# neonnnnn/sparsepoly

Measured on AMD Instinct MI355X. Metric: pcd_epochs_per_sec, higher is better.
Workload: dtype f32; 1 GPU; BASELINE configs[1]: degree=2 n_components=30 regularizer=squaredl12 solver=pcd fit_linear=True fit_lower=explicit on 1000000x100000 CSR nnz=49987865 (~50/row); schedule=colored, parallelism=single GPU, ranks=1, launcher=external, persistent_fallbacks=0

## Files before the change

sparsepoly_amd/csrc/spfm_engine.hip.h:

```cpp
#pragma once
#include <dlfcn.h>
#include <fcntl.h>
#include <sys/mman.h>
#include <unistd.h>
#include <chrono>
#include <hip/hip_runtime.h>

#include <cerrno>
#include <cmath>
#include <cstdio>
#include <cstdlib>
#include <cstring>
#include <atomic>
#include <map>
#include <memory>
#include <mutex>
#include <string>
#include <type_traits>
#include <thread>
#include <vector>

#include "../../include/spfm.h"
#include "spfm_common.hip.h"
#include "spfm_prb.hip.h"
#include "spfm_pcdw.hip.h"
#include "spfm_psgd.hip.h"

namespace spfm {
struct IntArgs;
void schedule_exact(int64_t, int32_t, const int64_t*, const int32_t*, const int32_t*, int,
                    std::vector<int32_t>&);
void schedule_colored(int64_t, int32_t, const int64_t*, const int32_t*, const int32_t*, int,
                      std::vector<int32_t>&, std::vector<int32_t>&);
void schedule_rlf(int64_t, int32_t, const int64_t*, const int32_t*, const int32_t*, int,
                  std::vector<int32_t>&, std::vector<int32_t>&);
bool csr_to_csc(int64_t, int32_t, const int64_t*, const int32_t*, std::vector<int64_t>&,
                std::vector<int32_t>&, std::vector<int64_t>&);
int schedule_threads();
void csc_to_csr(int64_t, int32_t, const int64_t*, const int32_t*, std::vector<int64_t>&,
                std::vector<int32_t>&, std::vector<int64_t>&);
void build_wide_stream(int64_t, const int64_t*, const int32_t*, const std::vector<int32_t>&,
                       const std::vector<int32_t>&, int, std::vector<int32_t>&,
                       std::vector<int32_t>&, std::vector<int32_t>&, std::vector<uint8_t>&);
void build_pb_stream(int64_t, const int64_t*, const int32_t*, const std::vector<int32_t>&,
                     const std::vector<int32_t>&, int, int, bool, const uint8_t*,
                     std::vector<int32_t>&, std::vector<int32_t>&, std::vector<uint8_t>&,
                     std::vector<uint8_t>&);
void build_rowblock_stream(int64_t, const int64_t*, const int32_t*, const std::vector<int32_t>&,
                           const std::vector<int32_t>&, int, int, std::vector<int32_t>&,
                           std::vector<int32_t>&, std::vector<uint32_t>&, const uint8_t*);
void schedule_relax(int64_t, int32_t, const int64_t*, const int32_t*, const int32_t*, int, int,
                    std::vector<int32_t>&, std::vector<int32_t>&, std::vector<int32_t>&,
                    std::vector<int32_t>&, std::vector<int64_t>&, std::vector<int64_t>&,
                    std::vector<int16_t>&, std::vector<uint8_t>&);
template <typename T>
hipError_t device_csr_to_csc(int64_t, int32_t, int64_t, const int64_t*, const int32_t*, const T*,
                             int64_t*, int32_t*, T*, int*, hipStream_t);
extern template hipError_t device_csr_to_csc<float>(int64_t, int32_t, int64_t, const int64_t*,
                                                    const int32_t*, const float*, int64_t*,
                                                    int32_t*, float*, int*, hipStream_t);
extern template hipError_t device_csr_to_csc<double>(int64_t, int32_t, int64_t, const int64_t*,
                                                     const int32_t*, const double*, int64_t*,
                                                     int32_t*, double*, int*, hipStream_t);
hipError_t device_rowblock_stream(int64_t, int32_t, int64_t, int, int, int, const int32_t*,
                                  const int32_t*, const int64_t*, const int32_t*, const uint8_t*,
                                  int32_t*, int32_t*, uint32_t*, int*, int64_t*, hipStream_t);
hipError_t device_pb_stream(int64_t, int32_t, int64_t, int, int, int, int, const int32_t*,
                            const int32_t*, const int64_t*, const int32_t*, const int64_t*,
                            const int32_t*, int32_t*, int32_t*, uint8_t*, uint8_t*, hipStream_t);
hipError_t device_wide_stream(int64_t, int32_t, int64_t, int, int, const int32_t*, const int32_t*,
                              const int64_t*, const int32_t*, const int64_t*, const int32_t*,
                              int32_t*, int32_t*, uint8_t*, hipStream_t);
hipError_t device_first_fit(int64_t, int32_t, int64_t, const int64_t*, const int32_t*, const int64_t*,
                            const int32_t*, int, int32_t*, int*, int*, hipStream_t);
hipError_t device_rlf(int64_t, int32_t, int64_t, const int64_t*, const int32_t*, const int64_t*,
                      const int32_t*, int, std::vector<int32_t>&, std::vector<int32_t>&, int*,
                      hipStream_t);
}

using namespace spfm;
struct IntPass;

typedef struct ncclComm* ncclComm_t;

struct DevBuf {
    struct Block {
        void* p;
        std::atomic<int> refs;
    };
    Block* blk = nullptr;
    void* p = nullptr;
    size_t bytes = 0;
    DevBuf() = default;
    DevBuf(const DevBuf&) = delete;
    DevBuf& operator=(const DevBuf&) = delete;
    ~DevBuf() { release(); }
    void release() {
        if (blk && blk->refs.fetch_sub(1) == 1) {
            (void)hipFree(blk->p);
            delete blk;
        }
        blk = nullptr;
        p = nullptr;
        bytes = 0;
    }
    bool shared() const { return blk && blk->refs.load() > 1; }
    hipError_t alloc(size_t b) {
        if (b <= bytes && p && !shared()) return hipSuccess;
        release();
        if (b == 0) b = 16;
        void* q = nullptr;
        hipError_t e = hipMalloc(&q, b);
        if (e != hipSuccess) return e;
        blk = new Block{q, {1}};
        p = q;
        bytes = b;
        return e;
    }
    void share(const DevBuf& o) {
        if (o.blk == blk) return;
        release();
        if (!o.blk) return;
        o.blk->refs.fetch_add(1);
        blk = o.blk;
        p = o.p;
        bytes = o.bytes;
    }
    template <typename U>
    U* as() const {
        return reinterpret_cast<U*>(p);
    }
};

#define HIPC(expr)                                                                       \
    do {                                                                                 \
        hipError_t _e = (expr);                                                          \
        if (_e != hipSuccess) {                                                          \
            err = std::string(#expr) + ": " + hipGetErrorString(_e);                     \
            return SPFM_ERR_RUNTIME;                                                     \
        }                                                                                \
    } while (0)

#define FAIL(code, msg) \
    do {                \
        err = (msg);    \
        return (code);  \
    } while (0)

#define SPFM_TRY(call)       \
    do {                     \
        int _rc = (call);    \
        if (_rc) return _rc; \
    } while (0)

#define SPFM_GUARD(h)                              \
    if (!(h)) return SPFM_ERR_INVALID;             \
    if (hipSetDevice((h)->device) != hipSuccess) { \
        (h)->err = "hipSetDevice failed";          \
        return SPFM_ERR_RUNTIME;                   \
    }

#define SPFM_DISPATCH(dt, ...)                                    \
    ((dt) == SPFM_F32 ? [&] { using T = float; __VA_ARGS__; }()   \
                      : [&] { using T = double; __VA_ARGS__; }())

static inline unsigned cdiv(int64_t a, int64_t b) { return (unsigned)((a + b - 1) / b); }

struct StreamCache {
    std::mutex mu;
    struct Prb {
        std::string key;
        DevBuf sp, erow, eval, lmask;
        int has_long = 0;
    };
    struct Pb {
        std::string key;
        DevBuf sp, erow, eval, meta, tab;
    };
    std::vector<std::unique_ptr<Prb>> prb;
    std::vector<std::unique_ptr<Pb>> pb;
    static constexpr size_t kKeep = 2;
};

struct ProfSlot {
    std::vector<hipEvent_t> ev;
    size_t used = 0;
    double ms = 0.0;
    int64_t launches = 0, nnz = 0;
};

struct spfm_engine {
    int device = 0, dtype = SPFM_F32;
    hipStream_t stream = nullptr;
    std::string err;
    std::string devname;

    int64_t n = 0, nnz = 0;
    int d = 0;
    bool have_data = false;
    DevBuf cptr, cidx, cval, rptr, ridx, rval, yy, A, col_norm;
    std::vector<int64_t> h_cptr;
    std::vector<int32_t> h_cidx;
    bool col_norm_reduced = false;
    std::shared_ptr<StreamCache> scache;
    uint64_t sched_hash = 0;
    int share_data_from(spfm_engine* src, const double* y);

    int n_orders = 0, k = 0;
    bool have_params = false;
    DevBuf P, Pt, w, lams;
    bool p_valid = true, pt_valid = false;
    std::vector<double> h_lams;

    int solver = -1, loss = 0, reg = 0, top_degree = 0;
    bool configured = false;
    DevBuf norms, cache, dcache;

    std::vector<int32_t> order, batch_ptr;
    DevBuf d_order, d_desc;
    int max_batch_cols = 0;
    bool have_schedule = false;
    int64_t sched_version = 0;

    DevBuf part, delta, pold, viol_col, scalar, ctl, comp_order, pred_tmp, partial, pb_scal,
        pb_ticket;
    bool pbcd_fuse = true;
    double* h_scalar = nullptr;

    DevBuf sg_gradP, sg_gradw, sg_samples, sg_part, sg_cond, sg_thr, sg_theta, sg_done,
        sg_norms, sg_conv, sg_sched, sg_idx, sg_snapP, sg_snapw, sg_snapc;
    bool psgd_force_eager = false;
    int psgd_graph_sweeps = 4;
    bool psgd_warm = false;
    int psgd_redone = 0;
    std::vector<PsgdBatch> h_sched;

    bool use_graph = true;
    bool fuse_chain = true;
    int max_batch_opt = 4096;

    bool pers_failed = false;
    int pers_fallbacks = 0;
    std::string pers_reason;
    int spin_max = 1 << 21;
    int debug_drop = 0;
    bool keep_last_error = false;
    bool have_pred_args = false;
    int pa_degree = 0, pa_lin = 0, pa_lower = 0;
    DevBuf snapP, snapW, snapC;
    std::map<const void*, int> resident_cache;
    std::map<std::string, bool> resident_agreed;

    bool persistent = true;
    int prb_G = 64;
    bool prb_lds = true;
    int prb_lds_active = 0;
    bool y_pm1 = false;
    bool prb_ready = false;
    int prb_has_long = 0;
    int prb_long = kPrbLong;
    DevBuf prb_sp, prb_erow, prb_eval, prb_slab, prb_abort, prow_old, d_bptr, prb_stamps,
        prb_viol, prb_cn, prb_lmask, prb_rec;
    bool prb_pack = true;
    int prb_pack_active = 0;
    bool prb_stamp_on = false;
    int wide_min_cols = 110;
    bool wide_stamp_on = false;
    DevBuf wide_stamps;
    DevBuf w_rec;
    static constexpr size_t kPrbLds = 84 * 1024;
    bool relax_on = true;
    int relax_state = 0;
    std::vector<int32_t> r_batch_ptr;
    int relax_has_long = 0;
    DevBuf r_bptr, r_sp, r_erow, r_eval, r_lmask, r_cfptr, r_cf, r_clist, r_cslab;
    bool wide_on = true;
    int pcdw_G = 0;
    bool wide_ready = false;
    int wide_G = 0, wide_tot = 0;
    int wide_lr_active = 0;
    int wide_lds_cap = -1;
    bool wide_ep = true;
    int wide_ep_active = 0;
    bool wide_rec8 = true;
    DevBuf w_wbase, w_wsp, w_erow, w_eval, w_slabA, w_slabB;
    bool pb_persistent = true;
    int pbprb_G = 256;
    int probe_xcd = 0, probe_lds = 60 * 1024;
    bool pb_stream_ready = false;
    int pb_stream_G = 0, pb_stream_NG = 0;
    DevBuf pb_tab;
    int pbr_state = 0;
    int pbr_G = 0, pb_relax_active = 0;
    std::vector<int32_t> pbr_batch_ptr;
    DevBuf pbr_bptr, pbr_sp, pbr_erow, pbr_eval, pbr_meta, pbr_tab, pbr_cfptr, pbr_cf, pbr_clist,
        pbr_slabR;
    bool pb_balance = true;
    DevBuf pb_sp, pb_erow, pb_eval, pb_meta, pb_slabA, pb_slabB, pb_slabC, pb_stamps, pb_rec;
    bool pb_stamp_on = false;
    int pbprb_active = 0;
    int pb_dbg = 0;
    DevBuf pb_dbgbuf;
    std::map<std::string, hipGraphExec_t> graphs;

    ncclComm_t comm = nullptr;
    struct ShmComm {
        static constexpr size_t kMaxDoubles = 1 << 16;
        struct Hdr {
            volatile int arrive;
            volatile int sense;
            int pad[14];
        };
        Hdr* hdr = nullptr;
        double* slots = nullptr;
        size_t bytes = 0;
        int local_sense = 0;
    } shm;
    std::vector<double> shm_host;
    bool dist() const { return comm != nullptr || shm.hdr != nullptr; }
    int n_ranks = 1, rank = 0;
    static constexpr size_t kPeerPcdOff = 0, kPeerPbOff = 16 * 1024;
    static constexpr size_t kPeerProbeOff = kPeerPbOff + (size_t)2 * 64 * 8 * 64;
    static constexpr size_t kPeerDoubles = kPeerProbeOff + 64;
    int peer_generation = 0;
    void* peer_own = nullptr;
    std::vector<void*> peer_ptr;
    DevBuf peer_tab_pcd, peer_tab_pb;
    bool peer_ready = false;

    bool prof_on = false;
    ProfSlot prof[5];

    ~spfm_engine();

    void clear_graphs() {
        for (auto& kv : graphs) (void)hipGraphExecDestroy(kv.second);
        graphs.clear();
    }

    enum : unsigned {
        kInvPrbStream = 1,
        kInvPbStream = 2,
        kInvWideStream = 4,
        kInvRelax = 8,
        kInvPbRelax = 16,
        kInvSchedule = 32,
        kInvGraphs = 64,
        kInvStreams = kInvPrbStream | kInvPbStream | kInvWideStream,
    };
    void invalidate(unsigned mask) {
        if (mask & kInvPrbStream) prb_ready = false;
        if (mask & kInvPbStream) pb_stream_ready = false;
        if (mask & kInvWideStream) wide_ready = false;
        if (mask & kInvRelax) relax_state = 0;
        if (mask & kInvPbRelax) pbr_state = 0;
        if (mask & kInvSchedule) have_schedule = false;
        if (mask & kInvGraphs) clear_graphs();
    }

    RegState regstate() {
        RegState rs;
        rs.norms = norms.as<double>();
        rs.cache = cache.as<double>();
        rs.dcache = dcache.as<double>();
        return rs;
    }

    size_t tsize() const { return dtype == SPFM_F32 ? 4 : 8; }

    int sync() {
        HIPC(hipStreamSynchronize(stream));
        return SPFM_OK;
    }

    template <typename U>
    int upload_to(void* dst, const U* src, size_t count) {
        if (count) HIPC(hipMemcpyAsync(dst, src, sizeof(U) * count, hipMemcpyHostToDevice, stream));
        return SPFM_OK;
    }
    template <typename U>
    int upload(DevBuf& b, const U* src, size_t count, size_t min_count = 0) {
        HIPC(b.alloc(sizeof(U) * std::max(count, min_count)));
        return upload_to(b.p, src, count);
    }
    template <typename U>
    int download(U* dst, const void* src, size_t count) {
        if (count) HIPC(hipMemcpyAsync(dst, src, sizeof(U) * count, hipMemcpyDeviceToHost, stream));
        return SPFM_OK;
    }

    template <typename T>
    int stage_csr_rows(DevBuf& rp, DevBuf& ri, DevBuf& rv, std::vector<T>& hv,
                       const int64_t* indptr, const int32_t* indices, const double* data,
                       int64_t r0, int64_t r1, size_t min_entries = 0) {
        const int64_t e0 = r0 ? indptr[r0] : 0, ne = indptr[r1] - e0;
        const T* vals;
        if constexpr (std::is_same<T, double>::value) {
            vals = data + e0;
        } else {
            hv.resize((size_t)ne);
            const int nt = (ne >= (1 << 20)) ? schedule_threads() : 1;
            const int64_t per = (ne + nt - 1) / nt;
            auto work = [&](int tid) {
                const int64_t lo = per * tid, hi = std::min<int64_t>(ne, lo + per);
                for (int64_t ii = lo; ii < hi; ++ii) hv[(size_t)ii] = (T)data[e0 + ii];
            };
            std::vector<std::thread> pool;
            for (int t = 1; t < nt; ++t) pool.emplace_back(work, t);
            work(0);
            for (auto& th : pool) th.join();
            vals = hv.data();
        }
        SPFM_TRY(upload(rp, indptr + r0, (size_t)(r1 - r0 + 1)));
        SPFM_TRY(upload(ri, indices + e0, (size_t)ne, min_entries));
        return upload(rv, vals, (size_t)ne, min_entries);
    }

    template <typename T>
    int upload_targets(const double* y, std::vector<T>& hy) {
        hy.resize((size_t)n * 2);
        for (int64_t i = 0; i < n; ++i) {
            hy[(size_t)2 * i] = (T)0;
            hy[(size_t)2 * i + 1] = (T)y[i];
        }
        return upload_to(yy.p, hy.data(), hy.size());
    }

    struct BlockView {
        const double* base;
        int64_t ss, sj;
    };
    BlockView live_block(int order_idx) const {
        const double* img = p_valid ? P.as<double>() : Pt.as<double>();
        return {img + (size_t)order_idx * k * d, p_valid ? (int64_t)d : 1, p_valid ? 1 : (int64_t)k};
    }

    static constexpr size_t kProfPool = 32768;
    bool prof_armed = false;
    void prof_begin(int which, int64_t nnz_launch) {
        prof_armed = false;
        if (!prof_on) return;
        ProfSlot& ps = prof[which];
        if (ps.used + 2 > kProfPool) return;
        if (ps.used + 2 > ps.ev.size()) {
            hipEvent_t a, b;
            if (hipEventCreate(&a) != hipSuccess) return;
            if (hipEventCreate(&b) != hipSuccess) {
                (void)hipEventDestroy(a);
                return;
            }
            ps.ev.push_back(a);
            ps.ev.push_back(b);
        }
        ps.launches++;
        ps.nnz += nnz_launch;
        (void)hipEventRecord(ps.ev[ps.used], stream);
        prof_armed = true;
    }
    void prof_cancel(int which, int64_t nnz_launch) {
        if (!prof_armed) return;
        prof[which].launches--;
        prof[which].nnz -= nnz_launch;
        prof_armed = false;
    }
    void prof_end(int which) {
        if (!prof_armed) return;
        ProfSlot& ps = prof[which];
        (void)hipEventRecord(ps.ev[ps.used + 1], stream);
        ps.used += 2;
        prof_armed = false;
    }
    void prof_collect() {
        if (!prof_on) return;
        (void)hipStreamSynchronize(stream);
        for (auto& ps : prof) {
            for (size_t i = 0; i + 1 < ps.used; i += 2) {
                float ms = 0.f;
                if (hipEventElapsedTime(&ms, ps.ev[i], ps.ev[i + 1]) == hipSuccess) ps.ms += ms;
            }
            ps.used = 0;
        }
    }

    int64_t batch_nnz(int b) const {
        int64_t s = 0;
        for (int q = batch_ptr[b]; q < batch_ptr[b + 1]; ++q)
            s += h_cptr[order[q] + 1] - h_cptr[order[q]];
        return s;
    }

    int shm_barrier();

    int allreduce_shm(double* buf, size_t count);
    int allreduce_shm_piece(double* buf, size_t count);

    int allreduce(double* buf, size_t count);

    int ensure_col_norm();

    int ensure_p();
    int ensure_pt();

    template <typename F>
    int run_cached(const std::string& key, F&& body) {
        const bool graph_ok = use_graph && !prof_on && !dist();
        if (!graph_ok) return body();
        auto it = graphs.find(key);
        if (it == graphs.end()) {
            hipGraph_t g = nullptr;
            HIPC(hipStreamBeginCapture(stream, hipStreamCaptureModeThreadLocal));
            int rc = body();
            hipError_t e = hipStreamEndCapture(stream, &g);
            if (rc != SPFM_OK) {
                if (g) (void)hipGraphDestroy(g);
                return rc;
            }
            if (e != hipSuccess) {
                err = std::string("hipStreamEndCapture: ") + hipGetErrorString(e);
                return SPFM_ERR_RUNTIME;
            }
            hipGraphExec_t ge = nullptr;
            e = hipGraphInstantiate(&ge, g, nullptr, nullptr, 0);
            (void)hipGraphDestroy(g);
            if (e != hipSuccess) {
                err = std::string("hipGraphInstantiate: ") + hipGetErrorString(e);
                return SPFM_ERR_RUNTIME;
            }
            it = graphs.emplace(key, ge).first;
        }
        HIPC(hipGraphLaunch(it->second, stream));
        return SPFM_OK;
    }

    template <typename T>
    int upload_images(const int64_t* h_cp, const int32_t* h_ci, const int64_t* h_rp,
                      const int32_t* h_ri, const double* data_csc, const double* data_csr,
                      const int64_t* perm, const double* y);

    template <typename T>
    int set_data_t(const int64_t* indptr, const int32_t* indices, const double* data,
                   const double* y);

    int data_installed(const double* y);

    bool ingest_device = true;
    int ingest_device_used = 0;
    int co_tenants = 1;
    static constexpr int kIngestFallback = 2;
    template <typename T>
    int set_data_csr_device(const int64_t* indptr, const int32_t* indices, const double* data,
                            const double* y);

    int set_data_csr(int64_t n_, int32_t d_, const int64_t* indptr, const int32_t* indices,
                     const double* data, const double* y);

    int set_data(int64_t n_, int32_t d_, const int64_t* indptr, const int32_t* indices,
                 const double* data, const double* y);

    int set_params(int n_orders_, int k_, int32_t d_, const double* P_, const double* w_,
                   const double* lams_);

    int get_params(double* P_, double* w_);

    int configure(int solver_, int loss_, int reg_, int top_degree_);

// ... 359 lines not shown
```

sparsepoly_amd/csrc/spfm_engine_pcd.hip:

```cpp
#include "spfm_engine.hip.h"
#include "spfm_pcd.hip.h"
#include "spfm_linear.hip.h"

using namespace spfm;

template <typename T>
int spfm_engine::lin_body(double alpha) {
    const double mu = loss == SPFM_LOSS_SQUARED ? 1.0 : (loss == SPFM_LOSS_LOGISTIC ? 0.25 : 2.0);
    const int nb = n_batches();
    for (int b = 0; b < nb; ++b) {
        const int c0 = batch_ptr[b], nc = batch_ptr[b + 1] - c0;
        if (nc == 0) continue;
        const int32_t* cols = d_order.as<int32_t>() + c0;
        prof_begin(4, prof_on ? batch_nnz(b) : 0);
        if (!dist()) {
            hipLaunchKernelGGL((lin_fused_kernel<T>), dim3(nc), dim3(kBlock), 0, stream,
                               d_desc.as<ColDesc>() + c0, cidx.as<int32_t>(), cval.as<T>(),
                               yy.as<T>(), loss, w.as<double>(), col_norm.as<double>(), alpha,
                               mu, viol_col.as<double>());
        } else {
            hipLaunchKernelGGL((lin_grad_kernel<T>), dim3(nc), dim3(kBlock), 0, stream, cols,
                               cptr.as<int64_t>(), cidx.as<int32_t>(), cval.as<T>(),
                               yy.as<typename Vec2<T>::type>(), loss, part.as<double>());
            int rc = allreduce(part.as<double>(), (size_t)nc);
            if (rc) return rc;
            hipLaunchKernelGGL((lin_sync_kernel<T>), dim3(nc), dim3(kBlock), 0, stream, cols,
                               cptr.as<int64_t>(), cidx.as<int32_t>(), cval.as<T>(),
                               yy.as<T>(), part.as<double>(), w.as<double>(),
                               col_norm.as<double>(), alpha, mu, viol_col.as<double>());
        }
        prof_end(4);
    }
    HIPC(hipGetLastError());
    return SPFM_OK;
}

int spfm_engine::cd_linear_epoch(double alpha, double* viol) {
    int rc = epoch_prologue();
    if (rc) return rc;
    const bool wide = wide_usable();
    if (wide || prb_usable()) {
        const char* what = wide ? "wide persistent cd_linear pass" : "persistent cd_linear pass";
        rc = snapshot_state(w.as<double>(), (size_t)d, snapW);
        if (rc) return rc;
        if (wide) rc = SPFM_DISPATCH(dtype, return lin_wide<T>(alpha));
        else rc = SPFM_DISPATCH(dtype, return lin_prb_loss<T>(alpha));
        if (rc == kNotResident) {
            mark_not_resident(what);
            return cd_linear_epoch(alpha, viol);
        }
        if (rc) return rc;
        rc = epoch_epilogue(viol);
        if (rc) return rc;
        bool aborted = false;
        rc = persistent_aborted(&aborted);
        if (rc) return rc;
        if (aborted) {
            rc = recover_from_abort(w.as<double>(), (size_t)d, snapW, what);
            if (rc) return rc;
            return cd_linear_epoch(alpha, viol);
        }
        return SPFM_OK;
    }
    const std::string key = fkey("lin", {alpha}, {loss, sched_version});
    rc = run_cached(key, [&]() {
        return SPFM_DISPATCH(dtype, return lin_body<T>(alpha));
    });
    if (rc) return rc;
    return epoch_epilogue(viol);
}

template <typename T, int M>
int spfm_engine::pcd_pass_body(int order_idx, double beta, double gamma, double eta) {
    const double mu = loss == SPFM_LOSS_SQUARED ? 1.0 : (loss == SPFM_LOSS_LOGISTIC ? 0.25 : 2.0);
    double* Po = P.as<double>() + (size_t)order_idx * k * d;
    Ctl* c = ctl.as<Ctl>();
    double* cbuf[2] = {cache.as<double>(), cache.as<double>() + (kMaxDegree + 2)};
    hipLaunchKernelGGL(begin_pass_kernel, dim3(1), dim3(64), 0, stream, c,
                       comp_order.as<int32_t>(), lams.as<double>());
    const size_t a_stride = (size_t)n * Kind<M>::AS;
    if (reg != SPFM_REG_L1) {
        hipLaunchKernelGGL((pcd_compute_cache_kernel<M>), dim3(kCacheBlocks), dim3(kBlock), 0,
                           stream, c, Po, d, reg, partial.as<double>());
        hipLaunchKernelGGL((pcd_cache_combine_kernel<M>), dim3(1), dim3(64), 0, stream, reg,
                           kCacheBlocks, partial.as<double>(), cbuf[0]);
    }
    const int nb = n_batches();
    int par = 0;
    for (int b = 0; b < nb; ++b) {
        const int c0 = batch_ptr[b], nc = batch_ptr[b + 1] - c0;
        if (nc == 0) continue;
        const ColDesc* desc = d_desc.as<ColDesc>() + c0;
        const int64_t bn = prof_on ? batch_nnz(b) : 0;
        prof_begin(0, bn);
        hipLaunchKernelGGL((pcd_grad_kernel<T, M>), dim3(nc), dim3(kBlock), 0, stream, c, desc,
                           cidx.as<int32_t>(), cval.as<T>(), A.as<T>(), a_stride,
                           yy.as<typename Vec2<T>::type>(), Po, d, loss, part.as<double>(),
                           pold.as<double>());
        prof_end(0);
        int rc = allreduce(part.as<double>(), (size_t)2 * nc);
        if (rc) return rc;
        if (nc <= kWave && fuse_chain) {
            prof_begin(1, bn);
            hipLaunchKernelGGL((pcd_chain_sync_kernel<T, M>), dim3(nc), dim3(kBlock), 0, stream,
                               c, desc, nc, Po, d, part.as<double>(), pold.as<double>(), reg,
                               cbuf[par], cbuf[par ^ 1], mu, beta, gamma, eta,
                               cidx.as<int32_t>(), cval.as<T>(), A.as<T>(), a_stride,
                               yy.as<T>(), viol_col.as<double>());
            prof_end(1);
        } else {
            hipLaunchKernelGGL((pcd_chain_kernel<M>), dim3(1), dim3(kWave), 0, stream, c, desc,
                               nc, Po, d, part.as<double>(), pold.as<double>(), reg, cbuf[par],
                               cbuf[par ^ 1], mu, beta, gamma, eta, delta.as<double>(),
                               viol_col.as<double>());
            prof_begin(1, bn);
            hipLaunchKernelGGL((pcd_sync_kernel<T, M>), dim3(nc), dim3(kBlock), 0, stream, c,
                               desc, cidx.as<int32_t>(), cval.as<T>(), A.as<T>(), a_stride,
                               yy.as<T>(), delta.as<double>(), pold.as<double>());
            prof_end(1);
        }
        par ^= 1;
    }
    HIPC(hipGetLastError());
    return SPFM_OK;
}

PrbArgs spfm_engine::prb_args() {
    PrbArgs a;
    a.G = prb_G;
    a.nb = n_batches();
    a.bptr = d_bptr.as<int32_t>();
    a.desc = d_desc.as<ColDesc>();
    a.sp = prb_sp.as<int32_t>();
    a.lmask = prb_lmask.as<uint32_t>();
    a.has_long = prb_has_long;
    a.erow = prb_erow.as<int32_t>();
    a.slab = prb_slab.as<double>();
    a.rows_per = (int)std::max<int64_t>((n + prb_G - 1) / prb_G, 1);
    a.n_rows = (int)n;
    a.abort_flag = prb_abort.as<unsigned>();
    a.spin_max = spin_max;
    a.stamps = prb_stamp_on ? prb_stamps.as<long long>() : nullptr;
    a.n_ranks = peer_ready ? n_ranks : 1;
    a.rank = rank;
    a.xslab = peer_ready ? peer_tab_pcd.as<double*>() : nullptr;
    a.cf_ptr = nullptr;
    a.cf = nullptr;
    a.clist = nullptr;
    a.cslab = nullptr;
    a.rec = nullptr;
    return a;
}

PrbArgs spfm_engine::relax_args() {
    PrbArgs a = prb_args();
    a.nb = (int)r_batch_ptr.size() - 1;
    a.bptr = r_bptr.as<int32_t>();
    a.sp = r_sp.as<int32_t>();
    a.lmask = r_lmask.as<uint32_t>();
    a.has_long = relax_has_long;
    a.erow = r_erow.as<int32_t>();
    a.stamps = nullptr;
    a.cf_ptr = r_cfptr.as<int32_t>();
    a.cf = r_cf.p;
    a.clist = r_clist.as<int16_t>();
    a.cslab = r_cslab.as<double>();
    return a;
}

template <typename T, int M>
int spfm_engine::pcd_precompute_all(int order_idx) {
    if (n == 0) return SPFM_OK;
    pt_valid = false;
    int rc = ensure_pt();
    if (rc) return rc;
    const size_t lds = sizeof(T) * (size_t)Kind<M>::AS * kWave * 33;
    HIPC(hipFuncSetAttribute((const void*)pcd_precompute_all_kernel<T, M>,
                             hipFuncAttributeMaxDynamicSharedMemorySize, (int)lds));
    const int64_t tiles = (n + 31) / 32;
    const unsigned grid = (unsigned)std::min<int64_t>(tiles, 256 * 8);
    hipLaunchKernelGGL((pcd_precompute_all_kernel<T, M>), dim3(grid), dim3(kBlock), lds,
                       stream, n, k, rptr.as<int64_t>(), ridx.as<int32_t>(), rval.as<T>(),
                       Pt.as<double>() + (size_t)order_idx * k * d, A.as<T>());
    HIPC(hipGetLastError());
    return SPFM_OK;
}

template <typename T>
int spfm_engine::pcd_precompute_all_dispatch(int M, int order_idx) {
    switch (M) {
        case 0: return pcd_precompute_all<T, 0>(order_idx);
        case 2: return pcd_precompute_all<T, 2>(order_idx);
        case 3: return pcd_precompute_all<T, 3>(order_idx);
        case 4: return pcd_precompute_all<T, 4>(order_idx);
        case 5: return pcd_precompute_all<T, 5>(order_idx);
        case 6: return pcd_precompute_all<T, 6>(order_idx);
    }
    FAIL(SPFM_ERR_UNSUPPORTED, "degree outside 2..6");
}

template <typename T>
int spfm_engine::pcd_pass_dispatch(int M, int order_idx, double beta, double gamma, double eta) {
    switch (M) {
        case 0: return pcd_pass_body<T, 0>(order_idx, beta, gamma, eta);
        case 2: return pcd_pass_body<T, 2>(order_idx, beta, gamma, eta);
        case 3: return pcd_pass_body<T, 3>(order_idx, beta, gamma, eta);
        case 4: return pcd_pass_body<T, 4>(order_idx, beta, gamma, eta);
        case 5: return pcd_pass_body<T, 5>(order_idx, beta, gamma, eta);
        case 6: return pcd_pass_body<T, 6>(order_idx, beta, gamma, eta);
    }
    FAIL(SPFM_ERR_UNSUPPORTED, "degree outside 2..6");
}

int spfm_engine::pcd_epoch(int order_idx, int degree, double beta, double gamma, double eta,
              const int32_t* ic, int n_comp, double* viol) {
    int rc = epoch_prologue();
    if (rc) return rc;
    if (solver != SPFM_SOLVER_PCD) FAIL(SPFM_ERR_INVALID, "engine is not configured for pcd");
    if (order_idx < 0 || order_idx >= n_orders) FAIL(SPFM_ERR_INVALID, "bad order index");
    if (!degree_ok(degree)) FAIL(SPFM_ERR_INVALID, "bad degree");
    if (!ic || n_comp < 0 || n_comp > k) FAIL(SPFM_ERR_INVALID, "bad indices_component");
    for (int q = 0; q < n_comp; ++q)
        if (ic[q] < 0 || ic[q] >= k) FAIL(SPFM_ERR_INVALID, "indices_component out of range");
    rc = ensure_p();
    if (rc) return rc;
    pt_valid = false;
    if (n_comp > 0)
        SPFM_TRY(upload_to(comp_order.p, ic, (size_t)n_comp));
    HIPC(hipMemsetAsync(ctl.p, 0, sizeof(Ctl), stream));
    const std::string key = fkey("pcd", {beta, gamma, eta},
                                 {order_idx, degree, loss, reg, sched_version});
    const int M = kind_of(degree);
    rc = SPFM_DISPATCH(dtype, return pcd_precompute_all_dispatch<T>(M, order_idx));
    if (rc) return rc;
    bool use_prb = prb_usable();
    bool use_wide = wide_usable() && M == 2;
    const bool pers_epoch = use_prb || use_wide;
    double* Po_epoch = P.as<double>() + (size_t)order_idx * k * d;
    if (pers_epoch) {
        rc = snapshot_state(Po_epoch, (size_t)k * d, snapP);
        if (rc) return rc;
    }
    for (int pass = 0; pass < n_comp; ++pass) {
        rc = SPFM_OK;
        if (use_wide) {
            rc = SPFM_DISPATCH(dtype, return pcd_pass_wide<T>(order_idx, beta, gamma, eta));
        } else if (use_prb) {
            rc = SPFM_DISPATCH(dtype, return pcd_prb_dispatch<T>(M, order_idx, beta, gamma, eta));
        }
        if (rc == kNotResident) {
            mark_not_resident(use_wide ? "wide persistent pcd pass" : "persistent pcd pass");
            use_prb = use_wide = false;
            hipLaunchKernelGGL(unbegin_pass_kernel, dim3(1), dim3(1), 0, stream, ctl.as<Ctl>());
            HIPC(hipGetLastError());
        }
        if (!use_wide && !use_prb) {
            rc = run_cached(key, [&]() {
                return SPFM_DISPATCH(dtype, return pcd_pass_dispatch<T>(M, order_idx, beta, gamma,
                                     eta));
            });
        }
        if (rc) return rc;
    }
    pt_valid = false;
    rc = epoch_epilogue(viol);
    if (rc) return rc;
    if (pers_epoch) {
        bool aborted = false;
        rc = persistent_aborted(&aborted);
        if (rc) return rc;
        if (aborted) {
            rc = recover_from_abort(Po_epoch, (size_t)k * d, snapP,
                                    use_wide ? "wide persistent pcd pass" : "persistent pcd pass");
            if (rc) return rc;
            return pcd_epoch(order_idx, degree, beta, gamma, eta, ic, n_comp, viol);
        }
    }
    return SPFM_OK;
}

int spfm_engine::host_epoch_begin(int order_idx, int degree) {
    int rc = epoch_prologue();
    if (rc) return rc;
    if (solver != SPFM_SOLVER_PCD && solver != SPFM_SOLVER_PBCD)
        FAIL(SPFM_ERR_INVALID, "host-stepped epochs: configure for pcd or pbcd");
    if (order_idx < 0 || order_idx >= n_orders) FAIL(SPFM_ERR_INVALID, "bad order index");
    if (!degree_ok(degree)) FAIL(SPFM_ERR_INVALID, "bad degree");
    const int M = kind_of(degree);
    if (solver == SPFM_SOLVER_PCD) {
        rc = ensure_p();
        if (rc) return rc;
        pt_valid = false;
        HIPC(hipMemsetAsync(ctl.p, 0, sizeof(Ctl), stream));
        rc = SPFM_DISPATCH(dtype, return pcd_precompute_all_dispatch<T>(M, order_idx));
        if (rc) return rc;
        pt_valid = false;
    } else {
        rc = ensure_pt();
        if (rc) return rc;
        p_valid = false;
        rc = SPFM_DISPATCH(dtype, return host_pbcd_precompute<T>(M, order_idx));
        if (rc) return rc;
    }
    host_order = order_idx;
    host_degree = degree;
    return sync();
}

int spfm_engine::host_pass_begin(int s) {
    if (host_order < 0 || solver != SPFM_SOLVER_PCD)
        FAIL(SPFM_ERR_INVALID, "host_pass_begin: call spfm_host_epoch_begin (pcd) first");
    if (s < 0 || s >= k) FAIL(SPFM_ERR_INVALID, "component out of range");
    Ctl hc;
    std::memset(&hc, 0, sizeof hc);
    hc.s = s;
    hc.lam = h_lams[(size_t)s];
    SPFM_TRY(upload_to(ctl.p, &hc, 1));
    return sync();
}

template <typename T, int M>
int spfm_engine::host_sums_pcd(int b, double* out) {
    const int c0 = batch_ptr[b], nc = batch_ptr[b + 1] - c0;
    if (nc == 0) return SPFM_OK;
    double* Po = P.as<double>() + (size_t)host_order * k * d;
    hipLaunchKernelGGL((pcd_grad_kernel<T, M>), dim3(nc), dim3(kBlock), 0, stream, ctl.as<Ctl>(),
                       d_desc.as<ColDesc>() + c0, cidx.as<int32_t>(), cval.as<T>(), A.as<T>(),
                       (size_t)n * Kind<M>::AS, yy.as<typename Vec2<T>::type>(), Po, d, loss,
                       part.as<double>(), pold.as<double>());
    HIPC(hipGetLastError());
    int rc = allreduce(part.as<double>(), (size_t)2 * nc);
    if (rc) return rc;
    SPFM_TRY(download(out, part.p, 2 * (size_t)nc));
    return sync();
}

template <typename T, int M>
int spfm_engine::host_apply_pcd(int b, const double* p_new) {
    const int c0 = batch_ptr[b], nc = batch_ptr[b + 1] - c0;
    if (nc == 0) return SPFM_OK;
    double* Po = P.as<double>() + (size_t)host_order * k * d;
    SPFM_TRY(upload_to(delta.p, p_new, (size_t)nc));
    hipLaunchKernelGGL(host_apply_pcd_kernel, dim3(cdiv(nc, 64)), dim3(64), 0, stream,
                       ctl.as<Ctl>(), d_desc.as<ColDesc>() + c0, nc, Po, d, pold.as<double>(),
                       delta.as<double>(), viol_col.as<double>());
    hipLaunchKernelGGL((pcd_sync_kernel<T, M>), dim3(nc), dim3(kBlock), 0, stream, ctl.as<Ctl>(),
                       d_desc.as<ColDesc>() + c0, cidx.as<int32_t>(), cval.as<T>(), A.as<T>(),
                       (size_t)n * Kind<M>::AS, yy.as<T>(), delta.as<double>(),
                       pold.as<double>());
    HIPC(hipGetLastError());
    return sync();
}

int spfm_engine::host_step(bool sums, int b, double* out, const double* p_new, const double* p_old) {
    int rc = host_step_check(b);
    if (rc) return rc;
    if ((sums && !out) || (!sums && !p_new)) FAIL(SPFM_ERR_INVALID, "host step: NULL buffer");
    if (solver == SPFM_SOLVER_PCD)
        return SPFM_DISPATCH(dtype, return host_step_pcd_t<T>(sums, b, out, p_new));
    return SPFM_DISPATCH(dtype, return host_step_pbcd_t<T>(sums, b, out, p_new, p_old));
}

template <typename T>
int spfm_engine::host_step_pcd_t(bool sums, int b, double* out, const double* p_new) {
#define SPFM_HPC(MM) return sums ? host_sums_pcd<T, MM>(b, out) : host_apply_pcd<T, MM>(b, p_new)
    switch (kind_of(host_degree)) {
        case 0: SPFM_HPC(0);
        case 2: SPFM_HPC(2);
        case 3: SPFM_HPC(3);
        case 4: SPFM_HPC(4);
        case 5: SPFM_HPC(5);
        case 6: SPFM_HPC(6);
    }
#undef SPFM_HPC
    FAIL(SPFM_ERR_UNSUPPORTED, "degree outside 2..6");
}

int spfm_engine::host_epoch_end(double* viol) {
    if (host_order < 0) FAIL(SPFM_ERR_INVALID, "host_epoch_end: no host-stepped epoch open");
    host_order = -1;
    if (solver == SPFM_SOLVER_PCD) pt_valid = false;
    return epoch_epilogue(viol);
}


int spfm_engine::debug_stream_probe(int64_t* bytes_out) {
    if (!have_schedule || !prb_usable())
        FAIL(SPFM_ERR_INVALID, "stream probe: needs a schedule the 64-column persistent pass can run");
    int rc = SPFM_DISPATCH(dtype, return ensure_prb<T>());
    if (rc) return rc;
    DevBuf sink;
    if (sink.alloc(sizeof(double) * (size_t)prb_G * kPrbThreads) != hipSuccess)
        FAIL(SPFM_ERR_RUNTIME, "stream probe: allocation failed");
    const PrbArgs a = prb_args();
    SPFM_DISPATCH(dtype, hipLaunchKernelGGL((prb_stream_probe_kernel<T>), dim3(prb_G),
                                            dim3(kPrbThreads), 0, stream, a, prb_eval.as<T>(),
                                            sink.as<double>()));
    if (hipStreamSynchronize(stream) != hipSuccess)
        FAIL(SPFM_ERR_RUNTIME, "stream probe kernel failed");
    if (bytes_out)
        *bytes_out = nnz * (int64_t)(4 + tsize()) + (int64_t)prb_G * ((int64_t)d + n_batches()) * 4;
    return SPFM_OK;
}

int spfm_engine::debug_write_probe(int bytes, int64_t* bytes_out) {
    if (!have_schedule || !prb_usable())
        FAIL(SPFM_ERR_INVALID, "write probe: needs a schedule the 64-column persistent pass can run");
    if (bytes != 4 && bytes != 8 && bytes != 16) FAIL(SPFM_ERR_INVALID, "write probe: 4, 8 or 16 bytes");
    int rc = SPFM_DISPATCH(dtype, return ensure_prb<T>());
    if (rc) return rc;
    DevBuf recs;
    if (recs.alloc((size_t)16 * (size_t)(n > 0 ? n : 1)) != hipSuccess)
        FAIL(SPFM_ERR_RUNTIME, "write probe: allocation failed");
    const PrbArgs a = prb_args();
    if (bytes == 4)
        hipLaunchKernelGGL((prb_write_probe_kernel<4>), dim3(prb_G), dim3(kPrbThreads), 0, stream, a,
                           recs.as<float>());
    else if (bytes == 8)
        hipLaunchKernelGGL((prb_write_probe_kernel<8>), dim3(prb_G), dim3(kPrbThreads), 0, stream, a,
                           recs.as<float>());
    else
        hipLaunchKernelGGL((prb_write_probe_kernel<16>), dim3(prb_G), dim3(kPrbThreads), 0, stream,
                           a, recs.as<float>());
    if (hipStreamSynchronize(stream) != hipSuccess) FAIL(SPFM_ERR_RUNTIME, "write probe kernel failed");
    if (bytes_out) *bytes_out = nnz * (int64_t)bytes;
    return SPFM_OK;
}

SPFM_DEFINE_BRANCH_COUNTS(spfm_branch_counts_pcd)

template int spfm_engine::pcd_precompute_all_dispatch<float>(int, int);
template int spfm_engine::pcd_precompute_all_dispatch<double>(int, int);
```

sparsepoly_amd/csrc/spfm_engine_prb.inc.h:

```cpp
#include "spfm_engine.hip.h"
#include "spfm_pcd.hip.h"

using namespace spfm;

template <typename T, int LOSS>
int spfm_engine::lin_prb(double alpha) {
    const double mu = loss == SPFM_LOSS_SQUARED ? 1.0 : (loss == SPFM_LOSS_LOGISTIC ? 0.25 : 2.0);
    int rc = ensure_prb<T>();
    if (rc) return rc;
    constexpr bool can_lr = std::is_same<T, float>::value;
    constexpr int LRV = (LOSS == LOSS_SQUARED) ? 1 : 2;
    bool relaxed = false;
    if (relax_candidate()) {
        rc = ensure_relax<T>();
        if (rc) return rc;
        relaxed = relax_state == 1;
    }
    const PrbArgs pa = relaxed ? relax_args() : prb_args();
    int lds_max = 0;
    HIPC(hipDeviceGetAttribute(&lds_max, hipDeviceAttributeMaxSharedMemoryPerBlock, device));
    const size_t lds_lr = sizeof(double) * (kPrbLdsFixed + (relaxed ? kPrbLdsCR : 0)) +
                          (size_t)pa.rows_per * 5 + 16;
    const bool use_lr = can_lr && prb_lds && lds_lr <= (size_t)lds_max && (LRV == 1 || y_pm1);
    const size_t lds_bytes = use_lr ? std::max(lds_lr, kPrbLds) : kPrbLds;
    if constexpr (can_lr) {
        if (use_lr)
            HIPC(hipFuncSetAttribute((const void*)lin_prb_kernel<T, LOSS, LRV>,
                                     hipFuncAttributeMaxDynamicSharedMemorySize,
                                     (int)lds_bytes));
    }
    HIPC(hipFuncSetAttribute((const void*)lin_prb_kernel<T, LOSS, 0>,
                             hipFuncAttributeMaxDynamicSharedMemorySize, (int)kPrbLds));
    hipLaunchKernelGGL(gather_sched_kernel, dim3(cdiv(d, 256)), dim3(256), 0, stream, d,
                       d_desc.as<ColDesc>(), w.as<double>(), prow_old.as<double>());
    HIPC(hipMemsetAsync(prb_slab.p, 0, prb_slab.bytes, stream));
    if (relaxed) HIPC(hipMemsetAsync(r_cslab.p, 0, r_cslab.bytes, stream));
    {
        int prc = peer_clear(kPeerPcdOff, kPeerPbOff);
        if (prc) return prc;
    }
    prof_begin(4, nnz);
    bool launched = false;
    auto launch_cr = [&](auto lr_tag, size_t lds) -> int {
        constexpr int LRc = decltype(lr_tag)::value;
        auto* fn = lin_prb_kernel<T, LOSS, LRc, false, true>;
        HIPC(hipFuncSetAttribute((const void*)fn, hipFuncAttributeMaxDynamicSharedMemorySize,
                                 (int)lds));
        if (!resident_ok((const void*)fn, kPrbThreads, lds, prb_G)) return kNotResident;
        hipLaunchKernelGGL(fn, dim3(launch_groups(prb_G)), dim3(kPrbThreads), lds, stream, pa,
                           r_eval.as<T>(), yy.as<T>(), prow_old.as<double>(),
                           prb_cn.as<double>(), w.as<double>(), alpha, mu,
                           prb_viol.as<double>());
        return SPFM_OK;
    };
    auto launch = [&](auto lr_tag, auto mg_tag, size_t lds) -> int {
        constexpr int LRc = decltype(lr_tag)::value;
        constexpr bool MGc = decltype(mg_tag)::value;
        HIPC(hipFuncSetAttribute((const void*)lin_prb_kernel<T, LOSS, LRc, MGc>,
                                 hipFuncAttributeMaxDynamicSharedMemorySize, (int)lds));
        if (!resident_ok((const void*)lin_prb_kernel<T, LOSS, LRc, MGc>, kPrbThreads, lds, prb_G))
            return kNotResident;
        hipLaunchKernelGGL((lin_prb_kernel<T, LOSS, LRc, MGc>), dim3(launch_groups(prb_G)),
                           dim3(kPrbThreads),
                           lds, stream, pa, prb_eval.as<T>(), yy.as<T>(),
                           prow_old.as<double>(), prb_cn.as<double>(), w.as<double>(), alpha,
                           mu, prb_viol.as<double>());
        return SPFM_OK;
    };
    int lrc = SPFM_OK;
    if (relaxed) {
        launched = true;
        bool done = false;
        if constexpr (can_lr) {
            if (use_lr) {
                lrc = launch_cr(std::integral_constant<int, LRV>{}, lds_bytes);
                done = true;
            }
        }
        if (!done) lrc = launch_cr(std::integral_constant<int, 0>{}, kPrbLds);
    }
    if constexpr (can_lr) {
        if (use_lr && !launched) {
            lrc = pa.n_ranks > 1
                      ? launch(std::integral_constant<int, LRV>{}, std::true_type{}, lds_bytes)
                      : launch(std::integral_constant<int, LRV>{}, std::false_type{}, lds_bytes);
            launched = true;
        }
    }
    if (!launched)
        lrc = pa.n_ranks > 1
                  ? launch(std::integral_constant<int, 0>{}, std::true_type{}, kPrbLds)
                  : launch(std::integral_constant<int, 0>{}, std::false_type{}, kPrbLds);
    if (lrc == kNotResident) prof_cancel(4, nnz);
    if (lrc) return lrc;
    prof_end(4);
    hipLaunchKernelGGL(fold_viol_kernel, dim3(cdiv(d, 256)), dim3(256), 0, stream, d,
                       d_desc.as<ColDesc>(), prb_viol.as<double>(), viol_col.as<double>());
    HIPC(hipGetLastError());
    return SPFM_OK;
}

template <typename T>
int spfm_engine::lin_prb_loss(double alpha) {
    switch (loss) {
        case SPFM_LOSS_SQUARED: return lin_prb<T, LOSS_SQUARED>(alpha);
        case SPFM_LOSS_SQUARED_HINGE: return lin_prb<T, LOSS_SQUARED_HINGE>(alpha);
        default: return lin_prb<T, LOSS_LOGISTIC>(alpha);
    }
}

template <typename T>
int spfm_engine::ensure_prb() {
    if (prb_ready) return SPFM_OK;
    int ncu = 0;
    HIPC(hipDeviceGetAttribute(&ncu, hipDeviceAttributeMultiprocessorCount, device));
    if (prb_G > ncu) prb_G = ncu;
    if (prb_G < 1) prb_G = 1;
    const int nb_ = n_batches();
    std::unique_lock<std::mutex> cache_lock;
    std::string ckey;
    bool hit = false;
    if (scache) {
        ckey = fkey("prb", {}, {(int64_t)sched_hash, prb_G, prb_long, (int64_t)sizeof(T), nb_});
        cache_lock = std::unique_lock<std::mutex>(scache->mu);
        for (auto& e : scache->prb)
            if (e->key == ckey) {
                prb_sp.share(e->sp);
                prb_erow.share(e->erow);
                prb_eval.share(e->eval);
                prb_lmask.share(e->lmask);
                prb_has_long = e->has_long;
                stream_device_used = 2;
                hit = true;
                break;
            }
    }
    if (!hit) {
        int rc = build_prb_stream<T>(nb_);
        if (rc) return rc;
        if (scache) {
            auto e = std::make_unique<StreamCache::Prb>();
            e->key = ckey;
            e->sp.share(prb_sp);
            e->erow.share(prb_erow);
            e->eval.share(prb_eval);
            e->lmask.share(prb_lmask);
            e->has_long = prb_has_long;
            scache->prb.insert(scache->prb.begin(), std::move(e));
            if (scache->prb.size() > StreamCache::kKeep) scache->prb.pop_back();
        }
    }
    if (cache_lock.owns_lock()) cache_lock.unlock();
    HIPC(prb_slab.alloc(sizeof(double) * 2 * ((size_t)prb_G + 1) * 64 * 2));
    HIPC(prb_abort.alloc(sizeof(unsigned) * 4));
    HIPC(prow_old.alloc(sizeof(double) * (size_t)d));
    HIPC(prb_viol.alloc(sizeof(double) * (size_t)d));
    HIPC(prb_cn.alloc(sizeof(double) * (size_t)d));
    HIPC(prb_stamps.alloc(sizeof(long long) * 16 * (size_t)prb_G));
    HIPC(hipMemsetAsync(prb_stamps.p, 0, prb_stamps.bytes, stream));
    HIPC(hipMemsetAsync(prb_abort.p, 0, sizeof(unsigned) * 4, stream));
    HIPC(hipMemsetAsync(prb_slab.p, 0, prb_slab.bytes, stream));
    hipLaunchKernelGGL(gather_sched_kernel, dim3(cdiv(d, 256)), dim3(256), 0, stream, d,
                       d_desc.as<ColDesc>(), col_norm.as<double>(), prb_cn.as<double>());
    HIPC(hipGetLastError());
    HIPC(hipStreamSynchronize(stream));
    prb_ready = true;
    return SPFM_OK;
}

template <typename T>
int spfm_engine::build_prb_stream(int nb_) {
    const size_t nsp = (size_t)prb_G * nb_ * 65 + 1;
    DevBuf d_src;
    HIPC(d_src.alloc(sizeof(int32_t) * (size_t)(nnz > 0 ? nnz : 1)));
    HIPC(prb_sp.alloc(sizeof(int32_t) * nsp));
    HIPC(prb_lmask.alloc(sizeof(uint32_t) * (size_t)prb_G * nb_ * 2));
    stream_device_used = 0;
    if (stream_device && nnz >= (1 << 20)) {
        int hl = 0;
        const hipError_t e = device_rowblock_stream(
            n, d, nnz, prb_G, nb_, prb_long, d_order.as<int32_t>(), d_bptr.as<int32_t>(),
            cptr.as<int64_t>(), cidx.as<int32_t>(), nullptr, prb_sp.as<int32_t>(),
            d_src.as<int32_t>(), prb_lmask.as<uint32_t>(), &hl, nullptr, stream);
        if (e == hipSuccess) {
            prb_has_long = hl;
            stream_device_used = 1;
        } else {
            (void)hipGetLastError();
        }
    }
    std::vector<int32_t> sp, src;
    std::vector<uint32_t> lmask;
    if (!stream_device_used) {
        build_rowblock_stream(n, h_cptr.data(), h_cidx.data(), order, batch_ptr, prb_G,
                              prb_long, sp, src, lmask, nullptr);
        prb_has_long = 0;
        for (uint32_t m : lmask) prb_has_long |= (m != 0u);
        SPFM_TRY(upload_to(prb_lmask.p, lmask.data(), lmask.size()));
    }
    HIPC(prb_erow.alloc(sizeof(int32_t) * (size_t)(nnz > 0 ? nnz : 1)));
    HIPC(prb_eval.alloc(sizeof(T) * (size_t)(nnz > 0 ? nnz : 1)));
    if (!stream_device_used)
        SPFM_TRY(upload_to(prb_sp.p, sp.data(), sp.size()));
    if (nnz > 0) {
        if (!stream_device_used)
            SPFM_TRY(upload_to(d_src.p, src.data(), (size_t)nnz));
        hipLaunchKernelGGL((prb_gather_kernel<T>), dim3(cdiv(nnz, 256)), dim3(256), 0, stream,
                           nnz, d_src.as<int32_t>(), cidx.as<int32_t>(), cval.as<T>(),
                           prb_erow.as<int32_t>(), prb_eval.as<T>());
        HIPC(hipGetLastError());
    }
    HIPC(hipStreamSynchronize(stream));
    return SPFM_OK;
}

template <typename T>
int spfm_engine::ensure_relax() {
    if (relax_state != 0) return SPFM_OK;
    relax_state = -1;
    int rc = ensure_prb<T>();
    if (rc) return rc;
    std::vector<int32_t> cf_ptr, cf_row, cf_qq, sp, src;
    std::vector<int64_t> cf_ia, cf_ib;
    std::vector<int16_t> clist;
    std::vector<uint8_t> skip;
    std::vector<uint32_t> lmask;
    schedule_relax(n, d, h_cptr.data(), h_cidx.data(), order.data(), 64, 64, r_batch_ptr, cf_ptr,
                   cf_row, cf_qq, cf_ia, cf_ib, clist, skip);
    const int nbr = (int)r_batch_ptr.size() - 1;
    if ((double)nbr > 0.6 * (double)n_batches()) return SPFM_OK;
    DevBuf d_src;
    HIPC(r_bptr.alloc(sizeof(int32_t) * r_batch_ptr.size()));
    SPFM_TRY(upload_to(r_bptr.p, r_batch_ptr.data(), r_batch_ptr.size()));
    const size_t nsp_r = (size_t)prb_G * nbr * 65 + 1;
    bool dev_stream = false;
    size_t ne = 0;
    if (stream_device && nnz >= (1 << 20)) {
        DevBuf d_skip;
        HIPC(d_skip.alloc((size_t)nnz));
        SPFM_TRY(upload_to(d_skip.p, skip.data(), (size_t)nnz));
        HIPC(d_src.alloc(sizeof(int32_t) * (size_t)nnz));
        HIPC(r_sp.alloc(sizeof(int32_t) * nsp_r));
        HIPC(r_lmask.alloc(sizeof(uint32_t) * (size_t)prb_G * nbr * 2));
        int hl = 0;
        int64_t tot = 0;
        const hipError_t e = device_rowblock_stream(
            n, d, nnz, prb_G, nbr, prb_long, d_order.as<int32_t>(), r_bptr.as<int32_t>(),
            cptr.as<int64_t>(), cidx.as<int32_t>(), d_skip.as<uint8_t>(), r_sp.as<int32_t>(),
            d_src.as<int32_t>(), r_lmask.as<uint32_t>(), &hl, &tot, stream);
        if (e == hipSuccess) {
            relax_has_long = hl;
            ne = (size_t)tot;
            dev_stream = true;
        } else {
            (void)hipGetLastError();
        }
    }
    if (!dev_stream) {
        build_rowblock_stream(n, h_cptr.data(), h_cidx.data(), order, r_batch_ptr, prb_G,
                              prb_long, sp, src, lmask, skip.data());
        relax_has_long = 0;
        for (uint32_t m : lmask) relax_has_long |= (m != 0u);
        ne = src.size();
    }
    const size_t ncf = cf_row.size();
    std::vector<PrbConf<T>> hcf(ncf ? ncf : 1);
    {
        std::vector<T> hv((size_t)(nnz > 0 ? nnz : 1));
        SPFM_TRY(download(hv.data(), cval.p, (size_t)nnz));
        HIPC(hipStreamSynchronize(stream));
        for (size_t c = 0; c < ncf; ++c) {
            hcf[c].row = cf_row[c];
            hcf[c].qq = cf_qq[c];
            hcf[c].xa = hv[(size_t)cf_ia[c]];
            hcf[c].xb = hv[(size_t)cf_ib[c]];
        }
    }
    if (!dev_stream) {
        HIPC(d_src.alloc(sizeof(int32_t) * (ne ? ne : 1)));
        HIPC(r_sp.alloc(sizeof(int32_t) * sp.size()));
        HIPC(r_lmask.alloc(sizeof(uint32_t) * lmask.size()));
    }
    HIPC(r_erow.alloc(sizeof(int32_t) * (ne ? ne : 1)));
    HIPC(r_eval.alloc(sizeof(T) * (ne ? ne : 1)));
    HIPC(r_cfptr.alloc(sizeof(int32_t) * cf_ptr.size()));
    HIPC(r_cf.alloc(sizeof(PrbConf<T>) * hcf.size()));
    HIPC(r_clist.alloc(sizeof(int16_t) * clist.size() + 16));
    HIPC(r_cslab.alloc(sizeof(double) * 2 * 64 * 8));
    if (!dev_stream) {
        SPFM_TRY(upload_to(r_sp.p, sp.data(), sp.size()));
        SPFM_TRY(upload_to(r_lmask.p, lmask.data(), lmask.size()));
    }
    SPFM_TRY(upload_to(r_cfptr.p, cf_ptr.data(), cf_ptr.size()));
    SPFM_TRY(upload_to(r_cf.p, hcf.data(), hcf.size()));
    SPFM_TRY(upload_to(r_clist.p, clist.data(), clist.size()));
    if (ne > 0) {
        if (!dev_stream)
            SPFM_TRY(upload_to(d_src.p, src.data(), ne));
        hipLaunchKernelGGL((prb_gather_kernel<T>), dim3(cdiv((int64_t)ne, 256)), dim3(256), 0,
                           stream, (int64_t)ne, d_src.as<int32_t>(), cidx.as<int32_t>(),
                           cval.as<T>(), r_erow.as<int32_t>(), r_eval.as<T>());
        HIPC(hipGetLastError());
    }
    HIPC(hipStreamSynchronize(stream));
    relax_state = 1;
    return SPFM_OK;
}

template <typename T, int M, int LOSS>
int spfm_engine::pcd_pass_prb(int order_idx, double beta, double gamma, double eta) {
    const double mu = loss == SPFM_LOSS_SQUARED ? 1.0 : (loss == SPFM_LOSS_LOGISTIC ? 0.25 : 2.0);
    int rc = ensure_prb<T>();
    if (rc) return rc;
    double* Po = P.as<double>() + (size_t)order_idx * k * d;
    Ctl* c = ctl.as<Ctl>();
    double* cb = cache.as<double>();
    constexpr bool can_lr = std::is_same<T, float>::value && Kind<M>::AS <= 2;
    constexpr int LRV = (LOSS == LOSS_SQUARED) ? 1 : 2;
    constexpr bool can_stamp = std::is_same<T, float>::value && M == 2 && LOSS == LOSS_SQUARED;
    constexpr bool can_stamp3 = std::is_same<T, float>::value && M == 3 && LOSS == LOSS_SQUARED;
    if (prb_stamp_on && !((can_stamp && prb_lds) || (can_stamp3 && !prb_lds)))
        FAIL(SPFM_ERR_UNSUPPORTED,
             "prb_stamps: built for float storage, squared loss and degree 2 with prb_lds=1 "
             "or degree 3 with prb_lds=0 only");
    bool relaxed = false;
    if constexpr (M == 2 || M == 3) {
        if (relax_candidate() && !prb_stamp_on) {
            rc = ensure_relax<T>();
            if (rc) return rc;
            relaxed = relax_state == 1;
        }
    }
    PrbArgs pa = relaxed ? relax_args() : prb_args();
    constexpr bool can_pk = std::is_same<T, float>::value && M == 3;
    bool packed = false;
    if (prb_stamp_on && pa.n_ranks > 1)
        FAIL(SPFM_ERR_UNSUPPORTED,
             "prb_stamps: the timer instantiation has no cross-GPU stage (single rank only)");
    int lds_max = 0;
    HIPC(hipDeviceGetAttribute(&lds_max, hipDeviceAttributeMaxSharedMemoryPerBlock, device));
    const size_t lds_lr = sizeof(double) * (kPrbLdsFixed + (relaxed ? kPrbLdsCR : 0)) +
                          (size_t)pa.rows_per * (4 * Kind<M>::AS + (LRV == 1 ? 4 : 5)) + 16;
    const bool use_lr = can_lr && prb_lds && lds_lr <= (size_t)lds_max &&
                        (LRV == 1 || y_pm1);
    const size_t lds_bytes = use_lr ? std::max(lds_lr, kPrbLds) : kPrbLds;
    prb_lds_active = use_lr ? LRV : 0;
    hipLaunchKernelGGL(begin_pass_kernel, dim3(1), dim3(64), 0, stream, c,
                       comp_order.as<int32_t>(), lams.as<double>());
    if (reg != SPFM_REG_L1) {
        hipLaunchKernelGGL((pcd_compute_cache_kernel<M>), dim3(kCacheBlocks), dim3(kBlock), 0,
                           stream, c, Po, d, reg, partial.as<double>());
        hipLaunchKernelGGL((pcd_cache_combine_kernel<M>), dim3(1), dim3(64), 0, stream, reg,
                           kCacheBlocks, partial.as<double>(), cb);
    }
    hipLaunchKernelGGL(snapshot_row_kernel, dim3(cdiv(d, 256)), dim3(256), 0, stream, c, Po, d,
                       d_desc.as<ColDesc>(), prow_old.as<double>());
    HIPC(hipMemsetAsync(prb_slab.p, 0, prb_slab.bytes, stream));
    if (relaxed) HIPC(hipMemsetAsync(r_cslab.p, 0, r_cslab.bytes, stream));
    if constexpr (can_pk) {
        if (!use_lr && !prb_stamp_on && prb_pack) {
            HIPC(prb_rec.alloc(sizeof(float) * 4 * (size_t)n));
            pa.rec = prb_rec.p;
            hipLaunchKernelGGL(prb_pack3_kernel, dim3(cdiv(n, 256)), dim3(256), 0, stream, c, n,
                               (size_t)n * 2, yy.as<float>(), A.as<float>(),
                               prb_rec.as<float4>());
            packed = true;
        }
    }
    {
        int prc = peer_clear(kPeerPcdOff, kPeerPbOff);
        if (prc) return prc;
    }
    prof_begin(0, nnz);
    auto go = [&](auto lr_tag, auto stamp_tag, auto reg_tag) -> int {
        constexpr int LRc = decltype(lr_tag)::value;
        constexpr bool STc = decltype(stamp_tag)::value;
        constexpr int RGc = decltype(reg_tag)::value;
        const size_t lds = (LRc == 1 || LRc == 2) ? lds_bytes : kPrbLds;
        auto launch = [&](auto mg_tag) -> int {
            constexpr bool MGc = decltype(mg_tag)::value;
            HIPC(hipFuncSetAttribute(
                (const void*)pcd_prb_kernel<T, M, LOSS, LRc, STc, RGc, MGc>,
                hipFuncAttributeMaxDynamicSharedMemorySize, (int)lds));
            if (!resident_ok((const void*)pcd_prb_kernel<T, M, LOSS, LRc, STc, RGc, MGc>,
                             kPrbThreads, lds, prb_G))
                return kNotResident;
            hipLaunchKernelGGL((pcd_prb_kernel<T, M, LOSS, LRc, STc, RGc, MGc>),
                               dim3(launch_groups(prb_G)), dim3(kPrbThreads), lds, stream, c, pa, prb_eval.as<T>(),
                               A.as<T>(), (size_t)n * Kind<M>::AS, yy.as<T>(),
                               prow_old.as<double>(), Po, d, reg, cb, mu, beta, gamma, eta,
                               prb_viol.as<double>());
            return SPFM_OK;
        };
        if constexpr (STc) {
            return launch(std::false_type{});
        } else {
            return pa.n_ranks > 1 ? launch(std::true_type{}) : launch(std::false_type{});
        }
    };
    using std::integral_constant;
    int lrc = SPFM_OK;
    bool launched = false;
    if constexpr (M == 2 || M == 3) {
        if (relaxed) {
            auto launch_cr = [&](auto lr_tag) -> int {
                constexpr int LRc = decltype(lr_tag)::value;
                const size_t lds = (LRc == 1 || LRc == 2) ? lds_bytes : kPrbLds;
                auto* fn = pcd_prb_kernel<T, M, LOSS, LRc, false, -1, false, true>;
                HIPC(hipFuncSetAttribute((const void*)fn,
                                         hipFuncAttributeMaxDynamicSharedMemorySize, (int)lds));
                if (!resident_ok((const void*)fn, kPrbThreads, lds, prb_G)) return kNotResident;
                hipLaunchKernelGGL(fn, dim3(launch_groups(prb_G)), dim3(kPrbThreads), lds, stream,
                                   c, pa, r_eval.as<T>(), A.as<T>(), (size_t)n * Kind<M>::AS,
                                   yy.as<T>(), prow_old.as<double>(), Po, d, reg, cb, mu, beta,
                                   gamma, eta, prb_viol.as<double>());
                return SPFM_OK;
            };
            launched = true;
            bool done = false;
            if constexpr (can_lr) {
                if (use_lr) {
                    lrc = launch_cr(integral_constant<int, LRV>{});
                    done = true;
                }
            }
            if constexpr (can_pk) {
                if (!done && packed) {
                    lrc = launch_cr(integral_constant<int, 3>{});
                    done = true;
                }
            }
            if (!done) lrc = launch_cr(integral_constant<int, 0>{});
        }
    }
    if constexpr (can_lr) {
        if (use_lr && !launched) {
            launched = true;
            if constexpr (can_stamp) {
                if (prb_stamp_on)
                    lrc = go(integral_constant<int, LRV>{}, std::true_type{},
                             integral_constant<int, -1>{});
            }
            if (!prb_stamp_on) {
                if (reg == SPFM_REG_L1)
                    lrc = go(integral_constant<int, LRV>{}, std::false_type{},
                             integral_constant<int, REG_L1>{});
                else if (reg == SPFM_REG_OMEGATI)
                    lrc = go(integral_constant<int, LRV>{}, std::false_type{},
                             integral_constant<int, REG_OMEGATI>{});
                else if constexpr (M == 2)
                    lrc = go(integral_constant<int, LRV>{}, std::false_type{},
                             integral_constant<int, REG_SQL12>{});
                else
                    lrc = go(integral_constant<int, LRV>{}, std::false_type{},
                             integral_constant<int, -1>{});
            }
        }
    }
    if constexpr (can_pk) {
        if (!launched && packed) {
            launched = true;
            lrc = go(integral_constant<int, 3>{}, std::false_type{}, integral_constant<int, -1>{});
        }
    }
    if constexpr (can_stamp3) {
        if (!launched && prb_stamp_on) {
            launched = true;
            lrc = go(integral_constant<int, 0>{}, std::true_type{}, integral_constant<int, -1>{});
        }
    }
    if (!launched)
        lrc = go(integral_constant<int, 0>{}, std::false_type{}, integral_constant<int, -1>{});
    prb_pack_active = packed ? 1 : 0;
    if (lrc == kNotResident) prof_cancel(0, nnz);
    if (lrc) return lrc;
    prof_end(0);
    if constexpr (can_pk) {
        if (packed)
            hipLaunchKernelGGL(prb_unpack3_kernel, dim3(cdiv(n, 256)), dim3(256), 0, stream, c, n,
                               (size_t)n * 2, prb_rec.as<float4>(), yy.as<float>(),
                               A.as<float>());
    }
    hipLaunchKernelGGL(fold_viol_kernel, dim3(cdiv(d, 256)), dim3(256), 0, stream, d,
                       d_desc.as<ColDesc>(), prb_viol.as<double>(), viol_col.as<double>());
    HIPC(hipGetLastError());
    return SPFM_OK;
}

template <typename T, int M>
int spfm_engine::pcd_prb_loss(int order_idx, double beta, double gamma, double eta) {
    switch (loss) {
        case SPFM_LOSS_SQUARED:
            return pcd_pass_prb<T, M, LOSS_SQUARED>(order_idx, beta, gamma, eta);
        case SPFM_LOSS_SQUARED_HINGE:
            return pcd_pass_prb<T, M, LOSS_SQUARED_HINGE>(order_idx, beta, gamma, eta);
        default:
            return pcd_pass_prb<T, M, LOSS_LOGISTIC>(order_idx, beta, gamma, eta);
    }
}

template <typename T>
int spfm_engine::pcd_prb_dispatch(int M, int order_idx, double beta, double gamma, double eta) {
    switch (M) {
        case 0: return pcd_prb_loss<T, 0>(order_idx, beta, gamma, eta);
        case 2: return pcd_prb_loss<T, 2>(order_idx, beta, gamma, eta);
        case 3: return pcd_prb_loss<T, 3>(order_idx, beta, gamma, eta);
        case 4: return pcd_prb_loss<T, 4>(order_idx, beta, gamma, eta);
        case 5: return pcd_prb_loss<T, 5>(order_idx, beta, gamma, eta);
        case 6: return pcd_prb_loss<T, 6>(order_idx, beta, gamma, eta);
    }
    FAIL(SPFM_ERR_UNSUPPORTED, "degree outside 2..6");
}


#define SPFM_CAT_(a, b) a##b
#define SPFM_CAT(a, b) SPFM_CAT_(a, b)
SPFM_DEFINE_BRANCH_COUNTS(SPFM_CAT(spfm_branch_counts_prb_, SPFM_TU_TAG))

template int spfm_engine::ensure_prb<SPFM_TU_T>();
template int spfm_engine::lin_prb_loss<SPFM_TU_T>(double);
template int spfm_engine::pcd_prb_dispatch<SPFM_TU_T>(int, int, double, double, double);
```

sparsepoly_amd/csrc/spfm_ingest.hip:

```cpp
#include <hip/hip_runtime.h>

#include <cstdint>
#include <cstring>

#include <rocprim/device/device_radix_sort.hpp>

namespace spfm {

__global__ void ingest_check_kernel(int64_t n, int32_t d, const int64_t* __restrict__ rptr,
                                    const int32_t* __restrict__ ridx, int* __restrict__ flag) {
    const int64_t i = (int64_t)blockIdx.x * blockDim.x + threadIdx.x;
    if (i >= n) return;
    int bad = 0;
    int32_t prev = -1;
    for (int64_t ii = rptr[i]; ii < rptr[i + 1]; ++ii) {
        const int32_t j = ridx[ii];
        bad |= (j <= prev) | (j >= d);
        prev = j;
    }
    if (bad) atomicOr(flag, 1);
}

__global__ void ingest_rows_kernel(int64_t n, int64_t nnz, const int64_t* __restrict__ rptr,
                                   int32_t* __restrict__ pos, int32_t* __restrict__ row) {
    const int64_t ii = (int64_t)blockIdx.x * blockDim.x + threadIdx.x;
    if (ii >= nnz) return;
    int64_t lo = 0, hi = n;
    while (hi - lo > 1) {
        const int64_t mid = (lo + hi) >> 1;
        if (rptr[mid] <= ii) lo = mid;
        else hi = mid;
    }
    pos[ii] = (int32_t)ii;
    row[ii] = (int32_t)lo;
}

template <typename T>
__global__ void ingest_gather_kernel(int64_t nnz, const int32_t* __restrict__ perm,
                                     const int32_t* __restrict__ row, const T* __restrict__ rval,
                                     int32_t* __restrict__ cidx, T* __restrict__ cval) {
    const int64_t e = (int64_t)blockIdx.x * blockDim.x + threadIdx.x;
    if (e >= nnz) return;
    const int32_t p = perm[e];
    cidx[e] = row[p];
    cval[e] = rval[p];
}

__global__ void ingest_cptr_kernel(int32_t d, int64_t nnz, const int32_t* __restrict__ keys,
                                   int64_t* __restrict__ cptr) {
    const int32_t j = blockIdx.x * blockDim.x + threadIdx.x;
    if (j > d) return;
    int64_t lo = 0, hi = nnz;
    while (lo < hi) {
        const int64_t mid = (lo + hi) >> 1;
        if (keys[mid] < j) lo = mid + 1;
        else hi = mid;
    }
    cptr[j] = lo;
}

template <typename T>
hipError_t device_csr_to_csc(int64_t n, int32_t d, int64_t nnz, const int64_t* rptr,
                             const int32_t* ridx, const T* rval, int64_t* cptr, int32_t* cidx,
                             T* cval, int* invalid, hipStream_t stream) {
    *invalid = 0;
    hipError_t e;
    int* d_flag = nullptr;
    int32_t *pos = nullptr, *row = nullptr, *keys_out = nullptr, *perm = nullptr;
    void* temp = nullptr;
    auto done = [&](hipError_t rc) {
        (void)hipFree(d_flag);
        (void)hipFree(pos);
        (void)hipFree(row);
        (void)hipFree(keys_out);
        (void)hipFree(perm);
        (void)hipFree(temp);
        return rc;
    };
    if ((e = hipMalloc(&d_flag, sizeof(int))) != hipSuccess) return done(e);
    if ((e = hipMemsetAsync(d_flag, 0, sizeof(int), stream)) != hipSuccess) return done(e);
    if (n > 0)
        hipLaunchKernelGGL(ingest_check_kernel, dim3((unsigned)((n + 255) / 256)), dim3(256), 0,
                           stream, n, d, rptr, ridx, d_flag);
    int h_flag = 0;
    if ((e = hipMemcpyAsync(&h_flag, d_flag, sizeof(int), hipMemcpyDeviceToHost, stream)) !=
            hipSuccess ||
        (e = hipStreamSynchronize(stream)) != hipSuccess)
        return done(e);
    if (h_flag) {
        *invalid = 1;
        return done(hipSuccess);
    }
    const size_t nz = (size_t)(nnz > 0 ? nnz : 1);
    if ((e = hipMalloc(&pos, sizeof(int32_t) * nz)) != hipSuccess) return done(e);
    if ((e = hipMalloc(&row, sizeof(int32_t) * nz)) != hipSuccess) return done(e);
    if ((e = hipMalloc(&keys_out, sizeof(int32_t) * nz)) != hipSuccess) return done(e);
    if ((e = hipMalloc(&perm, sizeof(int32_t) * nz)) != hipSuccess) return done(e);
    if (nnz > 0) {
        hipLaunchKernelGGL(ingest_rows_kernel, dim3((unsigned)((nnz + 255) / 256)), dim3(256), 0,
                           stream, n, nnz, rptr, pos, row);
        int end_bit = 1;
        while (end_bit < 31 && (1 << end_bit) < d) ++end_bit;
        size_t temp_bytes = 0;
        if ((e = rocprim::radix_sort_pairs(nullptr, temp_bytes, ridx, keys_out, pos, perm,
                                           (size_t)nnz, 0, end_bit, stream)) != hipSuccess)
            return done(e);
        if ((e = hipMalloc(&temp, temp_bytes ? temp_bytes : 16)) != hipSuccess) return done(e);
        if ((e = rocprim::radix_sort_pairs(temp, temp_bytes, ridx, keys_out, pos, perm, (size_t)nnz,
                                           0, end_bit, stream)) != hipSuccess)
            return done(e);
        hipLaunchKernelGGL((ingest_gather_kernel<T>), dim3((unsigned)((nnz + 255) / 256)), dim3(256),
                           0, stream, nnz, perm, row, rval, cidx, cval);
    }
    hipLaunchKernelGGL(ingest_cptr_kernel, dim3((unsigned)((d + 1 + 255) / 256)), dim3(256), 0, stream,
                       d, nnz, keys_out, cptr);
    if ((e = hipGetLastError()) != hipSuccess) return done(e);
    if ((e = hipStreamSynchronize(stream)) != hipSuccess) return done(e);
    return done(hipSuccess);
}

template hipError_t device_csr_to_csc<float>(int64_t, int32_t, int64_t, const int64_t*,
                                             const int32_t*, const float*, int64_t*, int32_t*,
                                             float*, int*, hipStream_t);
template hipError_t device_csr_to_csc<double>(int64_t, int32_t, int64_t, const int64_t*,
                                              const int32_t*, const double*, int64_t*, int32_t*,
                                              double*, int*, hipStream_t);

}

#include <rocprim/device/device_scan.hpp>

namespace spfm {

__device__ __forceinline__ int64_t rbs_lower_bound(const int32_t* __restrict__ a, int64_t lo,
                                                   int64_t hi, int64_t key) {
    while (lo < hi) {
        const int64_t mid = (lo + hi) >> 1;
        if ((int64_t)a[mid] < key) lo = mid + 1;
        else hi = mid;
    }
    return lo;
}

__global__ void rbs_count_kernel(int32_t d, int G, int nb, int64_t rows_per,
                                 const int32_t* __restrict__ order, const int32_t* __restrict__ bptr,
                                 const int64_t* __restrict__ cptr, const int32_t* __restrict__ cidx,
                                 const uint8_t* __restrict__ skip, int32_t* __restrict__ cnt,
                                 int32_t* __restrict__ first) {
    const int64_t t = (int64_t)blockIdx.x * blockDim.x + threadIdx.x;
    if (t >= (int64_t)d * G) return;
    const int pos = (int)(t / G), g = (int)(t % G);
    int blo = 0, bhi = nb;
    while (bhi - blo > 1) {
        const int mid = (blo + bhi) >> 1;
        if (bptr[mid] <= pos) blo = mid;
        else bhi = mid;
    }
    const int b = blo, q = pos - bptr[b];
    const int32_t j = order[pos];
    const int64_t cb = cptr[j], ce = cptr[j + 1];
    const int64_t lo = rbs_lower_bound(cidx, cb, ce, (int64_t)g * rows_per);
    const int64_t hi = rbs_lower_bound(cidx, lo, ce, (int64_t)(g + 1) * rows_per);
    first[t] = (int32_t)lo;
    int32_t m = (int32_t)(hi - lo);
    if (skip)
        for (int64_t ii = lo; ii < hi; ++ii) m -= skip[ii] ? 1 : 0;
    cnt[((size_t)g * nb + b) * 65 + q] = m;
}

__global__ void rbs_fill_kernel(int32_t d, int G, int nb, const int32_t* __restrict__ bptr,
                                const int64_t* __restrict__ cptr, const int32_t* __restrict__ cidx,
                                const int32_t* __restrict__ order, int64_t rows_per,
                                const uint8_t* __restrict__ skip,
                                const int32_t* __restrict__ cnt, const int32_t* __restrict__ sp,
                                const int32_t* __restrict__ first, int32_t* __restrict__ src) {
    const int64_t t = (int64_t)blockIdx.x * blockDim.x + threadIdx.x;
    if (t >= (int64_t)d * G) return;
    const int pos = (int)(t / G), g = (int)(t % G);
    int blo = 0, bhi = nb;
    while (bhi - blo > 1) {
        const int mid = (blo + bhi) >> 1;
        if (bptr[mid] <= pos) blo = mid;
        else bhi = mid;
    }
    const size_t at = ((size_t)g * nb + blo) * 65 + (size_t)(pos - bptr[blo]);
    const int32_t m = cnt[at], dst = sp[at], lo = first[t];
    if (!skip) {
        for (int32_t u = 0; u < m; ++u) src[(size_t)dst + u] = lo + u;
    } else {
        const int32_t j = order[pos];
        const int64_t hi = rbs_lower_bound(cidx, lo, cptr[j + 1], (int64_t)(g + 1) * rows_per);
        int32_t u = 0;
        for (int64_t ii = lo; ii < hi; ++ii)
            if (!skip[ii]) src[(size_t)dst + u++] = (int32_t)ii;
    }
}

__global__ void rbs_lmask_kernel(int G, int nb, int long_thresh, const int32_t* __restrict__ bptr,
                                 const int32_t* __restrict__ cnt, uint32_t* __restrict__ lmask,
                                 int* __restrict__ any_long) {
    const int64_t t = (int64_t)blockIdx.x * blockDim.x + threadIdx.x;
    if (t >= (int64_t)G * nb) return;
    const int b = (int)(t % nb);
    const int ncols = bptr[b + 1] - bptr[b];
    uint32_t m0 = 0u, m1 = 0u;
    for (int q = 0; q < ncols && q < 64; ++q)
        if (cnt[(size_t)t * 65 + q] > long_thresh) {
            if (q < 32) m0 |= 1u << q;
            else m1 |= 1u << (q - 32);
        }
    lmask[(size_t)t * 2] = m0;
    lmask[(size_t)t * 2 + 1] = m1;
    if (m0 | m1) atomicOr(any_long, 1);
}

hipError_t device_rowblock_stream(int64_t n, int32_t d, int64_t nnz, int G, int nb, int long_thresh,
                                  const int32_t* order, const int32_t* bptr, const int64_t* cptr,
                                  const int32_t* cidx, const uint8_t* skip, int32_t* sp, int32_t* src,
                                  uint32_t* lmask, int* has_long, int64_t* n_entries,
                                  hipStream_t stream) {
    *has_long = 0;
    hipError_t e;
    int32_t *cnt = nullptr, *first = nullptr;
    int* flag = nullptr;
    void* temp = nullptr;
    auto done = [&](hipError_t rc) {
        (void)hipFree(cnt);
        (void)hipFree(first);
        (void)hipFree(flag);
        (void)hipFree(temp);
        return rc;
    };
    const int64_t rows_per = (n + G - 1) / G > 0 ? (n + G - 1) / G : 1;
    const size_t nsp = (size_t)G * nb * 65 + 1;
    const int64_t pairs = (int64_t)d * G;
    if ((e = hipMalloc(&cnt, sizeof(int32_t) * nsp)) != hipSuccess) return done(e);
    if ((e = hipMalloc(&first, sizeof(int32_t) * (size_t)(pairs > 0 ? pairs : 1))) != hipSuccess)
        return done(e);
    if ((e = hipMalloc(&flag, sizeof(int))) != hipSuccess) return done(e);
    if ((e = hipMemsetAsync(cnt, 0, sizeof(int32_t) * nsp, stream)) != hipSuccess) return done(e);
    if ((e = hipMemsetAsync(flag, 0, sizeof(int), stream)) != hipSuccess) return done(e);
    const unsigned blocks = (unsigned)((pairs + 255) / 256);
    hipLaunchKernelGGL(rbs_count_kernel, dim3(blocks), dim3(256), 0, stream, d, G, nb, rows_per,
                       order, bptr, cptr, cidx, skip, cnt, first);
    size_t temp_bytes = 0;
    if ((e = rocprim::exclusive_scan(nullptr, temp_bytes, cnt, sp, (int32_t)0, nsp,
                                     rocprim::plus<int32_t>(), stream)) != hipSuccess)
        return done(e);
    if ((e = hipMalloc(&temp, temp_bytes ? temp_bytes : 16)) != hipSuccess) return done(e);
    if ((e = rocprim::exclusive_scan(temp, temp_bytes, cnt, sp, (int32_t)0, nsp,
                                     rocprim::plus<int32_t>(), stream)) != hipSuccess)
        return done(e);
    hipLaunchKernelGGL(rbs_fill_kernel, dim3(blocks), dim3(256), 0, stream, d, G, nb, bptr, cptr, cidx,
                       order, rows_per, skip, cnt, sp, first, src);
    hipLaunchKernelGGL(rbs_lmask_kernel, dim3((unsigned)(((int64_t)G * nb + 255) / 256)), dim3(256),
                       0, stream, G, nb, long_thresh, bptr, cnt, lmask, flag);
    if ((e = hipGetLastError()) != hipSuccess) return done(e);
    int32_t total = 0;
    if ((e = hipMemcpyAsync(has_long, flag, sizeof(int), hipMemcpyDeviceToHost, stream)) !=
            hipSuccess ||
        (e = hipMemcpyAsync(&total, sp + (nsp - 1), sizeof(int32_t), hipMemcpyDeviceToHost,
                            stream)) != hipSuccess ||
        (e = hipStreamSynchronize(stream)) != hipSuccess)
        return done(e);
    if (n_entries) *n_entries = total;
    (void)nnz;
    return done(hipSuccess);
}



__global__ void sb_step_of_kernel(int32_t d, int nb, const int32_t* __restrict__ order,
                                  const int32_t* __restrict__ bptr, int32_t* __restrict__ step_of) {
    const int pos = blockIdx.x * blockDim.x + threadIdx.x;
    if (pos >= d) return;
    int blo = 0, bhi = nb;
    while (bhi - blo > 1) {
        const int mid = (blo + bhi) >> 1;
        if (bptr[mid] <= pos) blo = mid;
        else bhi = mid;
    }
    step_of[order[pos]] = blo;
}

__device__ __forceinline__ int sb_row_in_step(const int64_t* __restrict__ rptr,
                                              const int32_t* __restrict__ ridx,
                                              const int32_t* __restrict__ step_of, int32_t row,
                                              int step) {
    if (step < 0) return 0;
    int hit = 0;
    for (int64_t c = rptr[row]; c < rptr[row + 1]; ++c) hit |= (step_of[ridx[c]] == step);
    return hit;
}

__global__ void pbs_count_kernel(int32_t d, int G, int nb, int64_t rows_per,
                                 const int32_t* __restrict__ order, const int32_t* __restrict__ bptr,
                                 const int64_t* __restrict__ cptr, const int32_t* __restrict__ cidx,
                                 int32_t* __restrict__ cnt ,
                                 int32_t* __restrict__ first) {
    const int64_t t = (int64_t)blockIdx.x * blockDim.x + threadIdx.x;
    if (t >= (int64_t)d * G) return;
    const int pos = (int)(t / G), g = (int)(t % G);
    int blo = 0, bhi = nb;
    while (bhi - blo > 1) {
        const int mid = (blo + bhi) >> 1;
        if (bptr[mid] <= pos) blo = mid;
        else bhi = mid;
    }
    const int b = blo, q = pos - bptr[b];
    const int32_t j = order[pos];
    const int64_t cb = cptr[j], ce = cptr[j + 1];
    const int64_t lo = rbs_lower_bound(cidx, cb, ce, (int64_t)g * rows_per);
    const int64_t hi = rbs_lower_bound(cidx, lo, ce, (int64_t)(g + 1) * rows_per);
    first[t] = (int32_t)lo;
    cnt[((size_t)g * nb + b) * 64 + q] = (int32_t)(hi - lo);
}

__global__ void pbs_assign_kernel(int G, int nb, int NG, int balance,
                                  const int32_t* __restrict__ bptr, const int32_t* __restrict__ cnt,
                                  uint8_t* __restrict__ tab ,
                                  int32_t* __restrict__ gcnt ,
                                  int32_t* __restrict__ soff ,
                                  uint8_t* __restrict__ where ) {
    const int64_t t = (int64_t)blockIdx.x * blockDim.x + threadIdx.x;
    if (t >= (int64_t)G * nb) return;
    const int b = (int)(t % nb);
    const int QM = 64 / NG;
    const int nc = bptr[b + 1] - bptr[b];
    const int nc2 = b + 2 < nb ? bptr[b + 3] - bptr[b + 2] : 0;
    const int nw = min(64, max(nc, nc2));
    const int32_t* c = cnt + (size_t)t * 64;
    uint8_t* tb = tab + (size_t)t * 64;
    int32_t* gc = gcnt + (size_t)t * (NG + 1);
    int32_t* so = soff + (size_t)t * 64;
    uint8_t* wh = where + (size_t)t * 64;
    int load[16], used[16];
    for (int r = 0; r < NG; ++r) load[r] = used[r] = 0;
    for (int z = 0; z < 64; ++z) tb[z] = 0xFF;
    if (!balance) {
        for (int q = 0; q < nw; ++q) {
            const int r = q % NG, tt = q / NG;
            tb[r * QM + tt] = (uint8_t)q;
            wh[q] = (uint8_t)((r << 3) | tt);
            load[r] += q < nc ? c[q] : 0;
        }
    } else {
        uint8_t idx[64];
        for (int q = 0; q < nw; ++q) {
            const int cq = q < nc ? c[q] : 0;
            int z = q;
            while (z > 0) {
                const int pz = idx[z - 1];
                if ((pz < nc ? c[pz] : 0) >= cq) break;
                idx[z] = idx[z - 1];
                --z;
            }
            idx[z] = (uint8_t)q;
        }
        for (int z = 0; z < nw; ++z) {
            const int q = idx[z];
            int best = -1;
            for (int r = 0; r < NG; ++r)
                if (used[r] < QM && (best < 0 || load[r] < load[best])) best = r;
            tb[best * QM + used[best]] = (uint8_t)q;
            wh[q] = (uint8_t)((best << 3) | used[best]);
            used[best]++;
            load[best] += q < nc ? c[q] : 0;
        }
    }
    for (int r = 0; r < NG; ++r) {
        gc[r] = load[r];
        int at = 0;
        for (int tt = 0; tt < QM; ++tt) {
            const int q = tb[r * QM + tt];
            if (q == 0xFF) continue;
            so[q] = at;
            at += q < nc ? c[q] : 0;
        }
    }
    gc[NG] = 0;
}

__global__ void pbs_fill_kernel(int32_t d, int G, int nb, int NG, const int32_t* __restrict__ bptr,
                                const int32_t* __restrict__ cidx, const int32_t* __restrict__ cnt,
                                const int32_t* __restrict__ gsp, const int32_t* __restrict__ soff,
                                const uint8_t* __restrict__ where,
                                const int32_t* __restrict__ first, const int64_t* __restrict__ rptr,
                                const int32_t* __restrict__ ridx,
                                const int32_t* __restrict__ step_of, int32_t* __restrict__ src,
                                uint8_t* __restrict__ meta) {
    const int64_t t = (int64_t)blockIdx.x * blockDim.x + threadIdx.x;
    if (t >= (int64_t)d * G) return;
    const int pos = (int)(t / G), g = (int)(t % G);
    int blo = 0, bhi = nb;
    while (bhi - blo > 1) {
        const int mid = (blo + bhi) >> 1;
        if (bptr[mid] <= pos) blo = mid;
        else bhi = mid;
    }
    const int b = blo, q = pos - bptr[b];
    const size_t gb = (size_t)g * nb + b;
    const int32_t m = cnt[gb * 64 + q], lo = first[t];
    const int w = where[gb * 64 + q];
    const int32_t dst = gsp[gb * (NG + 1) + (w >> 3)] + soff[gb * 64 + q];
    for (int32_t u = 0; u < m; ++u) {
        src[(size_t)dst + u] = lo + u;
        const int hz = sb_row_in_step(rptr, ridx, step_of, cidx[lo + u], b - 1);
        meta[(size_t)dst + u] = (uint8_t)((w & 7) | (hz ? 0x80 : 0));
    }
}

hipError_t device_pb_stream(int64_t n, int32_t d, int64_t nnz, int G, int nb, int NG, int balance,
                            const int32_t* order, const int32_t* bptr, const int64_t* cptr,
                            const int32_t* cidx, const int64_t* rptr, const int32_t* ridx,
                            int32_t* gsp, int32_t* src, uint8_t* meta, uint8_t* tab,
                            hipStream_t stream) {
    hipError_t e;
    int32_t *cnt = nullptr, *first = nullptr, *gcnt = nullptr, *soff = nullptr, *step_of = nullptr;
    uint8_t* where = nullptr;
    void* temp = nullptr;
    auto done = [&](hipError_t rc) {
        (void)hipFree(cnt);
        (void)hipFree(first);
        (void)hipFree(gcnt);
        (void)hipFree(soff);
        (void)hipFree(step_of);
        (void)hipFree(where);
        (void)hipFree(temp);
        return rc;
    };
    if (NG > 16 || NG < 1 || nb < 1) return hipErrorInvalidValue;
    const int64_t rows_per = (n + G - 1) / G > 0 ? (n + G - 1) / G : 1;
    const size_t gbn = (size_t)G * nb;
    const size_t ngsp = gbn * (size_t)(NG + 1) + 1;
    const int64_t pairs = (int64_t)d * G;
    if ((e = hipMalloc(&cnt, sizeof(int32_t) * gbn * 64)) != hipSuccess) return done(e);
    if ((e = hipMalloc(&first, sizeof(int32_t) * (size_t)(pairs > 0 ? pairs : 1))) != hipSuccess)
        return done(e);
    if ((e = hipMalloc(&gcnt, sizeof(int32_t) * ngsp)) != hipSuccess) return done(e);
    if ((e = hipMalloc(&soff, sizeof(int32_t) * gbn * 64)) != hipSuccess) return done(e);
    if ((e = hipMalloc(&where, gbn * 64)) != hipSuccess) return done(e);
    if ((e = hipMalloc(&step_of, sizeof(int32_t) * (size_t)d)) != hipSuccess) return done(e);
    if ((e = hipMemsetAsync(cnt, 0, sizeof(int32_t) * gbn * 64, stream)) != hipSuccess) return done(e);
    if ((e = hipMemsetAsync(gcnt, 0, sizeof(int32_t) * ngsp, stream)) != hipSuccess) return done(e);
    hipLaunchKernelGGL(sb_step_of_kernel, dim3((unsigned)((d + 255) / 256)), dim3(256), 0, stream, d,
                       nb, order, bptr, step_of);
    const unsigned blocks = (unsigned)((pairs + 255) / 256);
    hipLaunchKernelGGL(pbs_count_kernel, dim3(blocks), dim3(256), 0, stream, d, G, nb, rows_per, order,
                       bptr, cptr, cidx, cnt, first);
    hipLaunchKernelGGL(pbs_assign_kernel, dim3((unsigned)((gbn + 127) / 128)), dim3(128), 0, stream, G,
                       nb, NG, balance, bptr, cnt, tab, gcnt, soff, where);
    size_t temp_bytes = 0;
    if ((e = rocprim::exclusive_scan(nullptr, temp_bytes, gcnt, gsp, (int32_t)0, ngsp,
                                     rocprim::plus<int32_t>(), stream)) != hipSuccess)
        return done(e);
    if ((e = hipMalloc(&temp, temp_bytes ? temp_bytes : 16)) != hipSuccess) return done(e);
    if ((e = rocprim::exclusive_scan(temp, temp_bytes, gcnt, gsp, (int32_t)0, ngsp,
                                     rocprim::plus<int32_t>(), stream)) != hipSuccess)
        return done(e);
    hipLaunchKernelGGL(pbs_fill_kernel, dim3(blocks), dim3(256), 0, stream, d, G, nb, NG, bptr, cidx,
                       cnt, gsp, soff, where, first, rptr, ridx, step_of, src, meta);
    if ((e = hipGetLastError()) != hipSuccess) return done(e);
    if ((e = hipStreamSynchronize(stream)) != hipSuccess) return done(e);
    (void)nnz;
    return done(hipSuccess);
}

__global__ void wds_count_kernel(int32_t d, int G, int nb, int64_t rows_per, int tot,
                                 const int32_t* __restrict__ order, const int32_t* __restrict__ bptr,
                                 const int64_t* __restrict__ cptr, const int32_t* __restrict__ cidx,
                                 int32_t* __restrict__ cnt, int32_t* __restrict__ first) {
    const int64_t t = (int64_t)blockIdx.x * blockDim.x + threadIdx.x;
    if (t >= (int64_t)d * G) return;
    const int pos = (int)(t / G), g = (int)(t % G);
    int blo = 0, bhi = nb;
    while (bhi - blo > 1) {
        const int mid = (blo + bhi) >> 1;
        if (bptr[mid] <= pos) blo = mid;
        else bhi = mid;
    }
    const int32_t j = order[pos];
    const int64_t cb = cptr[j], ce = cptr[j + 1];
    const int64_t lo = rbs_lower_bound(cidx, cb, ce, (int64_t)g * rows_per);
    const int64_t hi = rbs_lower_bound(cidx, lo, ce, (int64_t)(g + 1) * rows_per);
    first[t] = (int32_t)lo;
    cnt[(size_t)g * tot + (size_t)pos + (size_t)blo] = (int32_t)(hi - lo);
}

__global__ void wds_fill_kernel(int32_t d, int G, int nb, int tot, const int32_t* __restrict__ bptr,
                                const int32_t* __restrict__ cidx, const int32_t* __restrict__ cnt,
                                const int32_t* __restrict__ wsp, const int32_t* __restrict__ first,
                                const int64_t* __restrict__ rptr, const int32_t* __restrict__ ridx,
                                const int32_t* __restrict__ step_of, int32_t* __restrict__ src,
                                uint8_t* __restrict__ hz) {
    const int64_t t = (int64_t)blockIdx.x * blockDim.x + threadIdx.x;
    if (t >= (int64_t)d * G) return;
    const int pos = (int)(t / G), g = (int)(t % G);
    int blo = 0, bhi = nb;
    while (bhi - blo > 1) {
        const int mid = (blo + bhi) >> 1;
        if (bptr[mid] <= pos) blo = mid;
        else bhi = mid;
    }
    const size_t at = (size_t)g * tot + (size_t)pos + (size_t)blo;
    const int32_t m = cnt[at], dst = wsp[at], lo = first[t];
    for (int32_t u = 0; u < m; ++u) {
        src[(size_t)dst + u] = lo + u;
        hz[(size_t)dst + u] = (uint8_t)sb_row_in_step(rptr, ridx, step_of, cidx[lo + u], blo - 1);
    }
}

hipError_t device_wide_stream(int64_t n, int32_t d, int64_t nnz, int G, int nb,
                              const int32_t* order, const int32_t* bptr, const int64_t* cptr,
                              const int32_t* cidx, const int64_t* rptr, const int32_t* ridx,
                              int32_t* wsp, int32_t* src, uint8_t* hz, hipStream_t stream) {
    hipError_t e;
    int32_t *cnt = nullptr, *first = nullptr, *step_of = nullptr;
    void* temp = nullptr;
    auto done = [&](hipError_t rc) {
        (void)hipFree(cnt);
        (void)hipFree(first);
        (void)hipFree(step_of);
        (void)hipFree(temp);
        return rc;
    };
    const int64_t rows_per = (n + G - 1) / G > 0 ? (n + G - 1) / G : 1;
    const int tot = d + nb;
    const size_t nw = (size_t)G * (size_t)tot + 1;
    const int64_t pairs = (int64_t)d * G;
    if ((e = hipMalloc(&cnt, sizeof(int32_t) * nw)) != hipSuccess) return done(e);
    if ((e = hipMalloc(&first, sizeof(int32_t) * (size_t)(pairs > 0 ? pairs : 1))) != hipSuccess)
        return done(e);
    if ((e = hipMalloc(&step_of, sizeof(int32_t) * (size_t)d)) != hipSuccess) return done(e);
    if ((e = hipMemsetAsync(cnt, 0, sizeof(int32_t) * nw, stream)) != hipSuccess) return done(e);
    hipLaunchKernelGGL(sb_step_of_kernel, dim3((unsigned)((d + 255) / 256)), dim3(256), 0, stream, d,
                       nb, order, bptr, step_of);
    const unsigned blocks = (unsigned)((pairs + 255) / 256);
    hipLaunchKernelGGL(wds_count_kernel, dim3(blocks), dim3(256), 0, stream, d, G, nb, rows_per, tot,
                       order, bptr, cptr, cidx, cnt, first);
    size_t temp_bytes = 0;
    if ((e = rocprim::exclusive_scan(nullptr, temp_bytes, cnt, wsp, (int32_t)0, nw,
                                     rocprim::plus<int32_t>(), stream)) != hipSuccess)
        return done(e);
    if ((e = hipMalloc(&temp, temp_bytes ? temp_bytes : 16)) != hipSuccess) return done(e);
    if ((e = rocprim::exclusive_scan(temp, temp_bytes, cnt, wsp, (int32_t)0, nw,
                                     rocprim::plus<int32_t>(), stream)) != hipSuccess)
        return done(e);
    hipLaunchKernelGGL(wds_fill_kernel, dim3(blocks), dim3(256), 0, stream, d, G, nb, tot, bptr, cidx,
                       cnt, wsp, first, rptr, ridx, step_of, src, hz);
    if ((e = hipGetLastError()) != hipSuccess) return done(e);
    if ((e = hipStreamSynchronize(stream)) != hipSuccess) return done(e);
    (void)nnz;
    return done(hipSuccess);
}

}
```

sparsepoly_amd/csrc/spfm_options.inc.h:

```cpp
#include <climits>
#include <cstring>

namespace {

enum OptClass { TUNING, DIAGNOSTIC, TEST_HOOK, READOUT };
enum OptKind { OPT_FLAG, OPT_INT, OPT_READONLY, OPT_CUSTOM };

struct OptAccess {
    OptKind kind;
    bool spfm_engine::*b;
    int spfm_engine::*i;
    int lo, hi;
    int (*set)(spfm_engine*, int);
    int (*get)(spfm_engine*, int*);
};
struct OptRow {
    const char* key;
    OptClass cls;
    OptAccess a;
    unsigned inv;
    const char* doc;
};

constexpr int kMax = INT_MAX, kMin = INT_MIN;
constexpr OptAccess flag(bool spfm_engine::*m) { return {OPT_FLAG, m, nullptr, 0, 1, nullptr, nullptr}; }
constexpr OptAccess integer(int spfm_engine::*m, int lo, int hi) { return {OPT_INT, nullptr, m, lo, hi, nullptr, nullptr}; }
constexpr OptAccess readout(bool spfm_engine::*m) { return {OPT_READONLY, m, nullptr, 0, 0, nullptr, nullptr}; }
constexpr OptAccess readout(int spfm_engine::*m) { return {OPT_READONLY, nullptr, m, 0, 0, nullptr, nullptr}; }
constexpr OptAccess custom(int (*set)(spfm_engine*, int), int (*get)(spfm_engine*, int*)) { return {OPT_CUSTOM, nullptr, nullptr, 0, 0, set, get}; }
constexpr OptAccess with_set(OptAccess a, int (*set)(spfm_engine*, int)) { return a.set = set, a; }
constexpr OptAccess with_get(OptAccess a, int (*get)(spfm_engine*, int*)) { return a.get = get, a; }

constexpr unsigned G = spfm_engine::kInvGraphs, PRB = spfm_engine::kInvPrbStream | G,
                   PB = spfm_engine::kInvPbStream | G, WIDE = spfm_engine::kInvWideStream | G,
                   RELAX = spfm_engine::kInvRelax | G, PBRELAX = spfm_engine::kInvPbRelax | G,
                   SCHED = spfm_engine::kInvSchedule | G;

int set_co_tenants(spfm_engine* h, int value) {
    if (value < 1 || value > 64) {
        h->err = "co_tenants must be in [1, 64]";
        return SPFM_ERR_INVALID;
    }
    h->co_tenants = value;
    int ncu = 256;
    (void)hipDeviceGetAttribute(&ncu, hipDeviceAttributeMultiprocessorCount, h->device);
    const int share = std::max(1, ncu / value);
    if (h->prb_G > share) {
        h->prb_G = share;
        h->invalidate(spfm_engine::kInvPrbStream | spfm_engine::kInvRelax);
    }
    if (h->pbprb_G > share) {
        h->pbprb_G = share;
        h->invalidate(spfm_engine::kInvPbStream);
    }
    return SPFM_OK;
}
int set_peer_exchange(spfm_engine* h, int value) {
    if (value != 0) {
        h->err = "peer_exchange: only 0 can be set; connect with spfm_peer_connect";
        return SPFM_ERR_INVALID;
    }
    h->peer_ready = false;
    return SPFM_OK;
}
int set_pbprb_owners(spfm_engine* h, int value) {
    if (value != 0) {
        h->err = "pbprb_owners: dedicated owner workgroups were removed (only 0 is accepted)";
        return SPFM_ERR_UNSUPPORTED;
    }
    return SPFM_OK;
}
int get_pbprb_owners(spfm_engine*, int* v) { return *v = 0, SPFM_OK; }
int do_interaction_release(spfm_engine* h, int) { return h->interaction_release(), SPFM_OK; }
int get_persistent_active(spfm_engine* h, int* v) {
    return *v = h->have_schedule && (h->prb_usable() || h->wide_usable()), SPFM_OK;
}
int get_wide_active(spfm_engine* h, int* v) { return *v = h->have_schedule && h->wide_usable(), SPFM_OK; }
int get_relax_steps(spfm_engine* h, int* v) {
    *v = h->relax_state == 1 ? (int)h->r_batch_ptr.size() - 1
                             : (h->pbr_state == 1 ? (int)h->pbr_batch_ptr.size() - 1 : 0);
    return SPFM_OK;
}
int get_n_ranks(spfm_engine* h, int* v) { return *v = h->dist() ? h->n_ranks : 1, SPFM_OK; }
int get_pcdw_groups(spfm_engine* h, int* v) {
    return *v = h->wide_ready ? h->wide_G : h->pcdw_G, SPFM_OK;
}
int get_interaction_scratch_kib(spfm_engine* h, int* v) {
    return *v = (int)((h->interaction_scratch_bytes() + 1023) / 1024), SPFM_OK;
}
int get_free_mem_mib(spfm_engine* h, int* v) {
    size_t fr = 0, tot = 0;
    if (hipSetDevice(h->device) != hipSuccess || hipMemGetInfo(&fr, &tot) != hipSuccess) {
        h->err = "hipMemGetInfo failed";
        return SPFM_ERR_RUNTIME;
    }
    return *v = (int)(fr >> 20), SPFM_OK;
}

#define M(name) &spfm_engine::name
const OptRow kOptions[] = {
    {"use_graph", TUNING, flag(M(use_graph)), G, "hipGraph replay of the per-pass launch sequences"},
    {"fuse_chain", TUNING, flag(M(fuse_chain)), G, "fused chain+sync kernel for steps of <= 64 columns"},
    {"max_batch", TUNING, integer(M(max_batch_opt), 1, kMax), G, "columns per dependent step of the next coloured schedule"},
    {"persistent", TUNING, flag(M(persistent)), PRB, "one persistent launch per pcd component pass"},
    {"prb_groups", TUNING, integer(M(prb_G), 1, kMax), PRB | RELAX, "workgroups of the 64-column persistent pass"},
    {"prb_long", TUNING, integer(M(prb_long), 16, kMax), PRB | RELAX, "entries per (workgroup, step, slot) above which a slot is long"},
    {"prb_lds", TUNING, flag(M(prb_lds)), G, "keep the row block in LDS when it fits"},
    {"prb_pack", TUNING, flag(M(prb_pack)), G, "packed row records for degree-3 passes with rows in global memory"},
    {"relax", TUNING, flag(M(relax_on)), RELAX | PBRELAX, "merged steps for schedules of tiny steps"},
    {"pbcd_persistent", TUNING, flag(M(pb_persistent)), G, "the persistent pbcd pass"},
    {"pbprb_groups", TUNING, integer(M(pbprb_G), 1, kMax), PB | PBRELAX, "workgroups of the persistent pbcd pass"},
    {"pbprb_balance", TUNING, flag(M(pb_balance)), PB, "balanced slot groups of the persistent pbcd pass"},
    {"pbprb_owners", TUNING, custom(set_pbprb_owners, get_pbprb_owners), G, "dedicated owner workgroups: removed, only 0 is accepted"},
    {"pbcd_fuse", TUNING, flag(M(pbcd_fuse)), G, "multi-kernel pbcd: prep + chain in one launch"},
    {"wide", TUNING, flag(M(wide_on)), G, "the wide passes (steps of up to 512 columns)"},
    {"wide_min_cols", TUNING, integer(M(wide_min_cols), kMin, kMax), G, "mean class width below which 64-column steps are used"},
    {"pcdw_groups", TUNING, with_get(integer(M(pcdw_G), 1, kMax), get_pcdw_groups), WIDE, "workgroups of the wide pass (reads the count in use once its stream exists)"},
    {"wide_lds_rows", TUNING, integer(M(wide_lds_cap), kMin, kMax), G, "wide pass, block too large for LDS: rows of it kept there"},
    {"wide_ep", TUNING, flag(M(wide_ep)), G, "wide pass, rows in global memory: entry-parallel form"},
    {"wide_rec8", TUNING, flag(M(wide_rec8)), G, "wide pass: 8-byte (A, residual) row records where they apply"},
    {"ingest_device", TUNING, flag(M(ingest_device)), G, "CSR -> CSC on the device, else by host threads"},
    {"colour_device", TUNING, flag(M(colour_device)), G, "first-fit colouring on the device, else by host threads"},
    {"stream_device", TUNING, flag(M(stream_device)), PRB | PB | WIDE, "entry streams built on the device, else by host threads"},
    {"co_tenants", TUNING, with_set(integer(M(co_tenants), 1, 64), set_co_tenants), WIDE, "handles whose persistent passes share the device: caps prb_groups and pbprb_groups"},
    {"peer_exchange", TUNING, with_set(flag(M(peer_ready)), set_peer_exchange), SCHED | PRB | PB | WIDE, "0: give the in-kernel cross-GPU exchange up"},
    {"persistent_failed", TUNING, flag(M(pers_failed)), G, "0: try the persistent passes again after a fall-back"},
    {"psgd_eager", TUNING, flag(M(psgd_force_eager)), G, "launch every psgd minibatch eagerly"},
    {"psgd_graph_sweeps", TUNING, integer(M(psgd_graph_sweeps), 0, 64), G, "support-search sweeps recorded per psgd minibatch"},
    {"interaction_tile_budget", TUNING, integer(M(int_tile_budget), 0, kMax), 0, "tiles per launch of an interaction pass (0 = default)"},
    {"interaction_features", TUNING, integer(M(int_dlim), 0, kMax), 0, "interaction passes see only features below this (0 = all)"},
    {"interaction_release", TUNING, custom(do_interaction_release, nullptr), 0, "action: free the interaction passes' scratch"},
    {"prb_stamps", DIAGNOSTIC, flag(M(prb_stamp_on)), G, "phase timers of the 64-column pass"},
    {"pcdw_stamps", DIAGNOSTIC, flag(M(wide_stamp_on)), G, "phase timers of the wide pass"},
    {"pbprb_stamps", DIAGNOSTIC, flag(M(pb_stamp_on)), G, "phase timers of the persistent pbcd pass"},
    {"pbprb_dbg", DIAGNOSTIC, integer(M(pb_dbg), kMin, kMax), G, "bit mask of the persistent pbcd pass's diagnostic counters"},
    {"probe_xcd", DIAGNOSTIC, integer(M(probe_xcd), kMin, kMax), G, "spfm_debug_exchange_cost on one XCD"},
    {"probe_lds", DIAGNOSTIC, integer(M(probe_lds), kMin, kMax), G, "LDS bytes per workgroup of spfm_debug_exchange_cost"},
    {"debug_spin_max", TEST_HOOK, integer(M(spin_max), 64, kMax), G, "polls of one in-kernel wait before a persistent pass gives up"},
    {"debug_drop_group", TEST_HOOK, integer(M(debug_drop), kMin, kMax), G, "the next N persistent launches lack their last workgroup"},
    {"debug_keep_last_error", TEST_HOOK, flag(M(keep_last_error)), G, "spfm_comm_init keeps the thread's stale HIP error"},
    {"persistent_active", READOUT, custom(nullptr, get_persistent_active), 0, "the next pcd epoch uses a persistent pass"},
    {"wide_active", READOUT, custom(nullptr, get_wide_active), 0, "the next pcd epoch uses the wide pass"},
    {"pbprb_active", READOUT, readout(M(pbprb_active)), 0, "what the last pbcd epoch used"},
    {"prb_lds_active", READOUT, readout(M(prb_lds_active)), 0, "last pcd pass: 0 global rows, 1 LDS residual, 2 LDS prediction + sign"},
    {"prb_pack_active", READOUT, readout(M(prb_pack_active)), 0, "the last pcd pass used packed row records"},
    {"wide_lds_active", READOUT, readout(M(wide_lr_active)), 0, "last wide pass: 0 global rows, 1 all rows in LDS, 2 first rows of a block"},
    {"wide_ep_active", READOUT, readout(M(wide_ep_active)), 0, "the last wide pass used the entry-parallel form"},
    {"relax_steps", READOUT, custom(nullptr, get_relax_steps), 0, "merged steps per sweep (0 = strict steps)"},
    {"pb_relax_active", READOUT, readout(M(pb_relax_active)), 0, "the last pbcd epoch ran relaxed runs"},
    {"persistent_fallbacks", READOUT, readout(M(pers_fallbacks)), 0, "epochs redone on the multi-kernel engine"},
    {"psgd_redone", READOUT, readout(M(psgd_redone)), 0, "psgd epochs redone eagerly from a snapshot"},
    {"n_ranks", READOUT, custom(nullptr, get_n_ranks), 0, "ranks of the attached communicator"},
    {"peer_ready", READOUT, readout(M(peer_ready)), 0, "in-kernel cross-GPU exchange connected and verified"},
    {"ingest_device_used", READOUT, readout(M(ingest_device_used)), 0, "the last spfm_set_data_csr transposed on the device"},
    {"colour_device_used", READOUT, readout(M(colour_device_used)), 0, "the last coloured schedule was coloured on the device"},
    {"stream_device_used", READOUT, readout(M(stream_device_used)), 0, "64-column entry stream: 0 host, 1 device, 2 taken from a co-tenant"},
    {"pb_stream_device_used", READOUT, readout(M(pb_stream_device_used)), 0, "the pbcd entry stream was built on the device"},
    {"wide_stream_device_used", READOUT, readout(M(wide_stream_device_used)), 0, "the wide entry stream was built on the device"},
    {"interaction_launches", READOUT, readout(M(int_launches)), 0, "tile launches of the last interaction pass"},
    {"interaction_scratch_kib", READOUT, custom(nullptr, get_interaction_scratch_kib), 0, "scratch the interaction passes hold"},
    {"free_mem_mib", READOUT, custom(nullptr, get_free_mem_mib), 0, "free memory of the handle's device"},
};
#undef M

const OptRow* find_option(spfm_engine* h, const char* key) {
    for (const OptRow& r : kOptions)
        if (std::strcmp(r.key, key) == 0) return &r;
    h->err = std::string("unknown option: ") + key;
    return nullptr;
}
}

int spfm_set_option(spfm_handle h, const char* key, int value) {
    if (!h || !key) return SPFM_ERR_INVALID;
    const OptRow* r = find_option(h, key);
    if (!r) return SPFM_ERR_INVALID;
    const OptAccess& a = r->a;
    if (a.set) {
        const int rc = a.set(h, value);
        if (rc != SPFM_OK) return rc;
    } else if (a.kind == OPT_FLAG) {
        h->*a.b = value != 0;
    } else if (a.kind == OPT_INT) {
        if (value < a.lo || value > a.hi) {
            h->err = std::string(key) + " must be in [" + std::to_string(a.lo) + ", " +
                     std::to_string(a.hi) + "]";
            return SPFM_ERR_INVALID;
        }
        h->*a.i = value;
    } else {
        h->err = std::string("unknown option: ") + key;
        return SPFM_ERR_INVALID;
    }
    h->invalidate(r->inv);
    return SPFM_OK;
}

int spfm_get_option(spfm_handle h, const char* key, int* value) {
    if (!h || !key || !value) return SPFM_ERR_INVALID;
    const OptRow* r = find_option(h, key);
    if (!r) return SPFM_ERR_INVALID;
    if (r->a.get) return r->a.get(h, value);
    if (r->a.b) {
        *value = h->*r->a.b;
    } else if (r->a.i) {
        *value = h->*r->a.i;
    } else {
        h->err = std::string("unknown option: ") + key;
        return SPFM_ERR_INVALID;
    }
    return SPFM_OK;
}
```

sparsepoly_amd/csrc/spfm_prb.hip.h:

```cpp
#pragma once
#include "spfm_common.hip.h"
#include "spfm_pcd.hip.h"

namespace spfm {


struct PrbArgs {
    int G;
    int nb;
    const int32_t* bptr;
    const ColDesc* desc;
    const int32_t* sp;
    const uint32_t* lmask;
    int has_long;
    const int32_t* erow;
    double* slab;
    int rows_per;
    int n_rows;
    unsigned* abort_flag;
    unsigned spin_max;
    long long* stamps;
    int n_ranks, rank;
    double* const* xslab;
    const int32_t* cf_ptr;
    const void* cf;
    const int16_t* clist;
    double* cslab;
    void* rec;
};

template <typename T>
struct __attribute__((aligned(8))) PrbConf {
    int32_t row;
    int32_t qq;
    T xa, xb;
};


__device__ __forceinline__ void st_agent(double* p, double v) {
    __hip_atomic_store(reinterpret_cast<unsigned long long*>(p),
                       (unsigned long long)__double_as_longlong(v), __ATOMIC_RELAXED,
                       __HIP_MEMORY_SCOPE_AGENT);
}
__device__ __forceinline__ double ld_agent(const double* p) {
    const unsigned long long u =
        __hip_atomic_load(reinterpret_cast<const unsigned long long*>(p), __ATOMIC_RELAXED,
                          __HIP_MEMORY_SCOPE_AGENT);
    return __longlong_as_double((long long)u);
}

__device__ __forceinline__ unsigned long long prb_tag(int b) {
    return (unsigned long long)(((b >> 1) % 3) + 1);
}
__device__ __forceinline__ void prb_store_granule(double* p, double v, unsigned long long tag) {
    const unsigned long long u =
        ((unsigned long long)__double_as_longlong(v) & ~3ull) | tag;
    __hip_atomic_store(reinterpret_cast<unsigned long long*>(p), u, __ATOMIC_RELAXED,
                       __HIP_MEMORY_SCOPE_AGENT);
}
__device__ __forceinline__ unsigned long long prb_load_granule(const double* p) {
    return __hip_atomic_load(reinterpret_cast<const unsigned long long*>(p), __ATOMIC_RELAXED,
                             __HIP_MEMORY_SCOPE_AGENT);
}

__device__ __forceinline__ void prb_store_granule_l2(double* p, double v, unsigned long long tag) {
    const unsigned long long u =
        ((unsigned long long)__double_as_longlong(v) & ~3ull) | tag;
    asm volatile("global_store_dwordx2 %0, %1, off" ::"v"(p), "v"(u) : "memory");
}

__device__ __forceinline__ void prb_store_granule_sys(double* p, double v, unsigned long long tag) {
    const unsigned long long u =
        ((unsigned long long)__double_as_longlong(v) & ~3ull) | tag;
    __hip_atomic_store(reinterpret_cast<unsigned long long*>(p), u, __ATOMIC_RELAXED,
                       __HIP_MEMORY_SCOPE_SYSTEM);
}
__device__ __forceinline__ unsigned long long prb_load_granule_sys(const double* p) {
    return __hip_atomic_load(reinterpret_cast<const unsigned long long*>(p), __ATOMIC_RELAXED,
                             __HIP_MEMORY_SCOPE_SYSTEM);
}

template <int NV>
__device__ __forceinline__ bool prb_cross_gpu(const PrbArgs& a, int g, int b, int lane,
                                              double* tot) {
    const unsigned long long tag = prb_tag(b);
    const size_t par_off = (size_t)(b & 1) * a.n_ranks * 64 * 2;
    if (g == 0) {
        for (int rr = 0; rr < a.n_ranks; ++rr) {
            double* dst = a.xslab[rr] + par_off + ((size_t)a.rank * 64 + lane) * 2;
#pragma unroll
            for (int v = 0; v < NV; ++v) prb_store_granule_sys(dst + v, tot[v], tag);
        }
    }
    const double* mine = a.xslab[a.rank] + par_off + (size_t)lane * 2;
    double acc[NV];
#pragma unroll
    for (int v = 0; v < NV; ++v) acc[v] = 0.0;
    for (int rr = 0; rr < a.n_ranks; ++rr) {
        unsigned long long t[NV];
        unsigned spins = 0;
        for (;;) {
            bool all = true;
#pragma unroll
            for (int v = 0; v < NV; ++v) {
                t[v] = prb_load_granule_sys(mine + (size_t)rr * 64 * 2 + v);
                all = all && ((t[v] & 3ull) == tag);
            }
            if (all) break;
            if ((++spins & 63u) == 0) {
                if (__hip_atomic_load(a.abort_flag, __ATOMIC_RELAXED, __HIP_MEMORY_SCOPE_AGENT) ||
                    spins > a.spin_max) {
                    __hip_atomic_store(a.abort_flag, 1u, __ATOMIC_RELAXED,
                                       __HIP_MEMORY_SCOPE_AGENT);
                    return false;
                }
            }
        }
#pragma unroll
        for (int v = 0; v < NV; ++v) acc[v] += __longlong_as_double((long long)(t[v] & ~3ull));
    }
#pragma unroll
    for (int v = 0; v < NV; ++v) tot[v] = acc[v];
    return true;
}

typedef unsigned __attribute__((ext_vector_type(4))) prb_u4;

__device__ __forceinline__ void prb_load_pairs8(const double* const* p, prb_u4* r) {
    asm volatile(
        "global_load_dwordx4 %0, %8, off sc1\n\t"
        "global_load_dwordx4 %1, %9, off sc1\n\t"
        "global_load_dwordx4 %2, %10, off sc1\n\t"
        "global_load_dwordx4 %3, %11, off sc1\n\t"
        "global_load_dwordx4 %4, %12, off sc1\n\t"
        "global_load_dwordx4 %5, %13, off sc1\n\t"
        "global_load_dwordx4 %6, %14, off sc1\n\t"
        "global_load_dwordx4 %7, %15, off sc1\n\t"
        "s_waitcnt vmcnt(0)"
        : "=&v"(r[0]), "=&v"(r[1]), "=&v"(r[2]), "=&v"(r[3]), "=&v"(r[4]), "=&v"(r[5]),
          "=&v"(r[6]), "=&v"(r[7])
        : "v"(p[0]), "v"(p[1]), "v"(p[2]), "v"(p[3]), "v"(p[4]), "v"(p[5]), "v"(p[6]), "v"(p[7])
        : "memory");
}

template <int NV>
__device__ __forceinline__ bool prb_collect_quarter(const PrbArgs& a, int b, int w, int lane,
                                                    int ncols, double* out ,
                                                    int nparts = 4) {
    const double* slab = a.slab + (size_t)(b & 1) * a.G * 64 * 2;
    const unsigned long long tag = prb_tag(b);
    const int g0 = (a.G * w) / nparts, g1 = (a.G * (w + 1)) / nparts;
    double tot[NV];
#pragma unroll
    for (int v = 0; v < NV; ++v) tot[v] = 0.0;
    bool ok = true;
    if (lane < ncols) {
        const double* sl = slab + (size_t)lane * 2;
        constexpr int GU = 8;
        for (int gg = g0; gg < g1; gg += GU) {
            unsigned long long t[GU][NV];
            unsigned spins = 0;
            for (;;) {
                bool all = true;
                if constexpr (NV == 2) {
                    const double* ptr[GU];
                    prb_u4 r[GU];
#pragma unroll
                    for (int u = 0; u < GU; ++u)
                        ptr[u] = sl + (size_t)((gg + u < g1) ? gg + u : g1 - 1) * 128;
                    prb_load_pairs8(ptr, r);
#pragma unroll
                    for (int u = 0; u < GU; ++u) {
                        t[u][0] = ((unsigned long long)r[u].y << 32) | r[u].x;
                        t[u][1] = ((unsigned long long)r[u].w << 32) | r[u].z;
                        all = all && ((t[u][0] & 3ull) == tag) && ((t[u][1] & 3ull) == tag);
                    }
                } else {
#pragma unroll
                    for (int u = 0; u < GU; ++u)
#pragma unroll
                        for (int v = 0; v < NV; ++v) {
                            const bool in = gg + u < g1;
                            t[u][v] = in ? prb_load_granule(sl + (size_t)(gg + u) * 128 + v) : tag;
                            all = all && ((t[u][v] & 3ull) == tag);
                        }
                }
                if (all) break;
                if ((++spins & 63u) == 0) {
                    if (__hip_atomic_load(a.abort_flag, __ATOMIC_RELAXED,
                                          __HIP_MEMORY_SCOPE_AGENT) ||
                        spins > a.spin_max) {
                        __hip_atomic_store(a.abort_flag, 1u, __ATOMIC_RELAXED,
                                           __HIP_MEMORY_SCOPE_AGENT);
                        ok = false;
                        break;
                    }
                }
            }
            if (!ok) break;
#pragma unroll
            for (int u = 0; u < GU; ++u)
#pragma unroll
                for (int v = 0; v < NV; ++v)
                    if (gg + u < g1) tot[v] += __longlong_as_double((long long)(t[u][v] & ~3ull));
        }
    }
#pragma unroll
    for (int v = 0; v < NV; ++v) out[((size_t)w * 64 + lane) * 2 + v] = tot[v];
    return ok;
}

constexpr int PRB_PF = 4;
constexpr int kPrbLong = 48;
template <typename T>
struct PrbEntries {
    int e0, e1;
    int row[PRB_PF];
    T x[PRB_PF];
};

__device__ __forceinline__ void prb_load_sp(const PrbArgs& a, int g, int b, int slot, int ncols,
                                            int& e0, int& e1, unsigned long long& lmask) {
    e0 = 0;
    e1 = 0;
    lmask = 0ull;
    const int32_t* spb = a.sp + ((size_t)g * a.nb + b) * 65;
    if (a.has_long) {
        const uint32_t* lm = a.lmask + ((size_t)g * a.nb + b) * 2;
        lmask = ((unsigned long long)lm[1] << 32) | (unsigned long long)lm[0];
        if (slot < ncols && !((lmask >> slot) & 1ull)) {
            e0 = spb[slot];
            e1 = spb[slot + 1];
        }
    } else if (slot < ncols) {
        e0 = spb[slot];
        e1 = spb[slot + 1];
    }
}

__device__ __forceinline__ int nth_set_bit(unsigned long long m, int q) {
    for (int t = 0; t < q; ++t) m &= m - 1;
    return __builtin_ctzll(m);
}

template <typename T>
__device__ __forceinline__ void prb_load_entries(const PrbArgs& a, const T* __restrict__ eval,
                                                 int e0, int e1, int sub, PrbEntries<T>& en,
                                                 int pad_row = 0) {
    en.e0 = e0;
    en.e1 = e1;
#pragma unroll
    for (int u = 0; u < PRB_PF; ++u) {
        const int e = e0 + sub + 4 * u;
        const bool v = e < e1;
        en.row[u] = v ? a.erow[e] : pad_row;
        en.x[u] = v ? eval[e] : (T)0;
    }
}

constexpr int kPrbThreads = 512;
constexpr int kPrbParts = 8;
constexpr int kPrbLdsFixed = 2560;

template <int NV>
__device__ __forceinline__ bool prb_poll(const PrbArgs& a, const double* p, unsigned long long tag,
                                         double* out);

__device__ __forceinline__ void pcd_sync_entry_rec(size_t i, double x, double p_old, double upd,
                                                   double lam, float4* __restrict__ rec) {
    const float4 r = rec[i];
    const double a1 = (double)r.z, a2 = (double)r.w;
    const double d1 = x * (a1 - p_old * x);
    const double d2 = x * (a2 - p_old * d1);
    float4 o;
    o.x = (float)((double)r.x - lam * upd * d2);
    o.y = r.y;
    o.z = (float)(a1 - upd * x);
    o.w = (float)(a2 - upd * d1);
    rec[i] = o;
}

static __global__ void prb_pack3_kernel(const Ctl* __restrict__ ctl, int64_t n, size_t a_stride,
                                 const float* __restrict__ yy, const float* __restrict__ A_all,
                                 float4* __restrict__ rec) {
    const int64_t i = (int64_t)blockIdx.x * blockDim.x + threadIdx.x;
    if (i < n) {
        const float* A = A_all + (size_t)ctl->s * a_stride;
        float4 r;
        r.x = yy[2 * i];
        r.y = yy[2 * i + 1];
        r.z = A[2 * i];
        r.w = A[2 * i + 1];
        rec[i] = r;
    }
}
static __global__ void prb_unpack3_kernel(const Ctl* __restrict__ ctl, int64_t n, size_t a_stride,
                                   const float4* __restrict__ rec, float* __restrict__ yy,
                                   float* __restrict__ A_all) {
    const int64_t i = (int64_t)blockIdx.x * blockDim.x + threadIdx.x;
    if (i < n) {
        float* A = A_all + (size_t)ctl->s * a_stride;
        const float4 r = rec[i];
        yy[2 * i] = r.x;
        A[2 * i] = r.z;
        A[2 * i + 1] = r.w;
    }
}

constexpr int kPrbLdsCR = 256;
template <typename T, int M, int LOSS, int LR, bool STAMP = false, int REGC = -1, bool MG = false,
          bool CR = false>
__global__ __launch_bounds__(kPrbThreads) void pcd_prb_kernel(
    const Ctl* __restrict__ ctl, PrbArgs a, const T* __restrict__ eval, T* __restrict__ A_all,
    size_t a_stride, T* __restrict__ yy, const double* __restrict__ pold_sched,
    double* __restrict__ P, int d, int reg, const double* __restrict__ cache_in, double mu,
    double beta, double gamma, double eta, double* __restrict__ viol_pos) {
    T* __restrict__ A = A_all + (size_t)ctl->s * a_stride;
    extern __shared__ __attribute__((aligned(16))) double dyn_lds[];
    double* sh_delta = dyn_lds + 128;
    double* sh_pold = dyn_lds + 192;
    double* sh_chain = dyn_lds + 256;
    double* sh_quart = dyn_lds + 1536;
    int* sh_ok = reinterpret_cast<int*>(dyn_lds + 768);
    int* sh_go = reinterpret_cast<int*>(dyn_lds + 770);
    const typename Vec2<T>::type* yy2 = reinterpret_cast<const typename Vec2<T>::type*>(yy);
    const int g = blockIdx.x;
    const int tid = threadIdx.x, lane = tid & 63, wave = tid >> 6;
    const bool control = wave == 0;
    const bool worker = wave >= 1 && wave <= 4;
    const int part = worker ? wave - 1 : (control ? 4 : wave);
    const int wt = tid - 64;
    const int slot = worker ? (wt >> 2) : 64, sub = wt & 3;
    const int s = ctl->s;
    const double lam = ctl->lam;
    double* ps = P + (size_t)s * d;
    double cache[M + 1];
#pragma unroll
    for (int t = 0; t <= M; ++t) cache[t] = cache_in[t];

    double* sh_long = dyn_lds + 1024;
    constexpr bool LDSR = (LR == 1 || LR == 2);
    constexpr bool PK = (LR == 3);
    static_assert(!LDSR || (Kind<M>::AS <= 2 && sizeof(T) == 4 &&
                            (LR == 2 || LOSS == LOSS_SQUARED)),
                  "LDS-resident rows: float storage, one or two cache values per row");
    static_assert(!PK || (sizeof(T) == 4 && Kind<M>::AS == 2),
                  "packed row records: float storage, two cache values per row");
    float4* __restrict__ rec = reinterpret_cast<float4*>(a.rec);
    constexpr int AS = Kind<M>::AS;
    static_assert(!CR || (M >= 2 && !MG && !STAMP), "relaxed runs: degree >= 2, single GPU");
    constexpr int CSN = 2 + Kind<M>::AS;
    constexpr int CSS = 8;
    const int row0 = LDSR ? g * a.rows_per : 0;
    double* sh_ce = dyn_lds + kPrbLdsFixed;
    double* sh_cv = sh_ce + 128;
    T* lds_a = reinterpret_cast<T*>(dyn_lds + kPrbLdsFixed + (CR ? kPrbLdsCR : 0));
    T* lds_r = lds_a + (size_t)a.rows_per * AS;
    unsigned char* lds_s = reinterpret_cast<unsigned char*>(lds_r + a.rows_per);
    if constexpr (LDSR) {
        const int nr = min(a.rows_per, a.n_rows - row0);
        for (int il = tid; il < nr; il += kPrbThreads) {
            const typename Vec2<T>::type yv = yy2[(size_t)(row0 + il)];
#pragma unroll
            for (int t = 0; t < AS; ++t) lds_a[il * AS + t] = A[(size_t)(row0 + il) * AS + t];
            if constexpr (LR == 1) {
                lds_r[il] = (T)((double)yv.x - (double)yv.y);
            } else {
                lds_r[il] = yv.x;
                lds_s[il] = yv.y > (T)0 ? 1 : 0;
            }
        }
        __syncthreads();
    }
    PrbEntries<T> cur, nxt;
    int c0 = a.bptr[0], c1 = a.bptr[1];
    int c2 = (a.nb > 1) ? a.bptr[2] : c1;
    int c3 = (a.nb > 2) ? a.bptr[3] : c2;
    unsigned long long lm0 = 0ull, lm1 = 0ull;
    {
        int e0, e1;
        prb_load_sp(a, g, 0, slot, c1 - c0, e0, e1, lm0);
        prb_load_entries<T>(a, eval, e0, e1, sub, cur, row0);
    }
    int ne0 = 0, ne1 = 0;
    if (a.nb > 1) prb_load_sp(a, g, 1, slot, c2 - c1, ne0, ne1, lm1);
    double p_slot = (slot < c1 - c0) ? pold_sched[c0 + slot] : 0.0;
    if (tid == 0) {
        *sh_ok = 1;
        *sh_go = 0;
    }
    int cp0 = 0, cp1 = 0, cp2 = 0, cp3 = 0;
    PrbConf<T> cfc, cfn;
    cfc.row = cfn.row = 0;
    cfc.qq = cfn.qq = 0;
    cfc.xa = cfc.xb = cfn.xa = cfn.xb = (T)0;
    prb_u4 clq = {~0u, ~0u, ~0u, ~0u}, clqn = {~0u, ~0u, ~0u, ~0u};
    if constexpr (CR) {
        if (control) {
            const PrbConf<T>* cfa = reinterpret_cast<const PrbConf<T>*>(a.cf);
            cp0 = a.cf_ptr[0];
            cp1 = a.cf_ptr[min(1, a.nb)];
            cp2 = a.cf_ptr[min(2, a.nb)];
            cp3 = a.cf_ptr[min(3, a.nb)];
            if (lane < cp1 - cp0) cfc = cfa[cp0 + lane];
            if (lane < c1 - c0)
                clq = reinterpret_cast<const prb_u4*>(a.clist)[c0 + lane];
        }
    }
    long long acc[8] = {0, 0, 0, 0, 0, 0, 0, 0};
    long long tprev = STAMP ? clock64() : 0;
#define PRB_STAMP(k)                        \
    if constexpr (STAMP) {                  \
        if (tid == 0) {                     \
            const long long tn = clock64(); \
            acc[k] += tn - tprev;           \
            tprev = tn;                     \
        }                                   \
    }
#define PRB_HSTAMP(k)                       \
    if constexpr (STAMP) {                  \
        if (tid == 320) {                   \
            const long long tn = clock64(); \
            acc[k] += tn - tprev;           \
            tprev = tn;                     \
        }                                   \
    }
#define PRB_WSTAMP(k)                       \
    if constexpr (STAMP) {                  \
        if (tid == 64) {                    \
            const long long tn = clock64(); \
            acc[k] += tn - tprev;           \
            tprev = tn;                     \
        }                                   \
    }

    for (int b = 0; b < a.nb; ++b) {
        const int ncols = c1 - c0;
        const int c4 = (b + 4 <= a.nb) ? a.bptr[b + 4] : c3;
        __builtin_amdgcn_s_waitcnt(0x0F70);
        double av[PRB_PF][AS];
        double yh[PRB_PF], yt[PRB_PF], dlast[PRB_PF];
        double pl = 0.0;
        int jl = 0;
        double cst[CSN];
#pragma unroll
        for (int t = 0; t < CSN; ++t) cst[t] = 0.0;
        if (control) {
            if (lane < ncols) {
                pl = pold_sched[c0 + lane];
                if (g == 0) jl = a.desc[c0 + lane].j;
            }
            if constexpr (CR) {
                const int nc = cp1 - cp0, ncw = max(nc, cp3 - cp2);
                const unsigned long long ctag = prb_tag(b);
                double* cs = a.cslab + ((size_t)(b & 1) * 64 + lane) * CSS;
                if (lane < nc) {
                    const int i = cfc.row;
                    if (i / a.rows_per == g) {
                        double st[CSN];
                        if constexpr (LDSR) {
                            st[0] = (double)lds_r[i - row0];
                            st[1] = (LR == 1) ? 0.0 : (lds_s[i - row0] ? 1.0 : -1.0);
#pragma unroll
                            for (int t = 0; t < AS; ++t) st[2 + t] = (double)lds_a[(i - row0) * AS + t];
                        } else if constexpr (PK) {
                            const float4 r = rec[(size_t)i];
                            st[0] = (double)r.x;
                            st[1] = (double)r.y;
                            st[2] = (double)r.z;
                            st[2 + AS - 1] = (double)r.w;
                        } else {
                            const typename Vec2<T>::type yv = yy2[(size_t)i];
                            st[0] = (double)yv.x;
                            st[1] = (double)yv.y;
#pragma unroll
                            for (int t = 0; t < AS; ++t) st[2 + t] = (double)A[(size_t)i * AS + t];
                        }
#pragma unroll
                        for (int t = 0; t < CSN; ++t) prb_store_granule(cs + t, st[t], ctag);
                    }
                } else if (lane < ncw && (lane % a.G) == g) {
#pragma unroll
                    for (int t = 0; t < CSN; ++t) prb_store_granule(cs + t, 0.0, ctag);
                }
            }
        } else if (worker) {
#pragma unroll
            for (int u = 0; u < PRB_PF; ++u) {
                if constexpr (LDSR) {
                    const int il = cur.row[u] - row0;
                    yh[u] = (double)lds_r[il];
                    yt[u] = (LR == 1) ? 0.0 : (lds_s[il] ? 1.0 : -1.0);
#pragma unroll
                    for (int t = 0; t < AS; ++t) av[u][t] = (double)lds_a[il * AS + t];
                } else if constexpr (PK) {
                    const float4 r = rec[(size_t)cur.row[u]];
                    yh[u] = (double)r.x;
                    yt[u] = (double)r.y;
                    av[u][0] = (double)r.z;
                    av[u][AS - 1] = (double)r.w;
                } else {
                    const size_t i = (size_t)cur.row[u];
                    const typename Vec2<T>::type yv = yy2[i];
                    yh[u] = (double)yv.x;
                    yt[u] = (double)yv.y;
#pragma unroll
                    for (int t = 0; t < AS; ++t) av[u][t] = (double)A[i * AS + t];
                }
            }
            double ag = 0.0, ah = 0.0;
#pragma unroll
            for (int u = 0; u < PRB_PF; ++u) {
                const double dprev = grad_factor<M>(av[u], (double)cur.x[u], p_slot);
                dlast[u] = dprev;
                const double dl = dloss_dev(LOSS, yh[u], yt[u]);
                const bool v = cur.e0 + sub + 4 * u < cur.e1;
                ag += v ? dl * dprev : 0.0;
                ah += v ? dprev * dprev : 0.0;
            }
            for (int e = cur.e0 + sub + 4 * PRB_PF; e < cur.e1; e += 4) {
                const int i = a.erow[e];
                const double x = (double)eval[e];
                double a1[AS], y0, y1;
                if constexpr (LDSR) {
                    y0 = (double)lds_r[i - row0];
                    y1 = (LR == 1) ? 0.0 : (lds_s[i - row0] ? 1.0 : -1.0);
#pragma unroll
                    for (int t = 0; t < AS; ++t) a1[t] = (double)lds_a[(i - row0) * AS + t];
                } else if constexpr (PK) {
                    const float4 r = rec[(size_t)i];
                    y0 = (double)r.x;
                    y1 = (double)r.y;
                    a1[0] = (double)r.z;
                    a1[AS - 1] = (double)r.w;
                } else {
                    const typename Vec2<T>::type yv = yy2[i];
                    y0 = (double)yv.x;
                    y1 = (double)yv.y;
#pragma unroll
                    for (int t = 0; t < AS; ++t) a1[t] = (double)A[(size_t)i * AS + t];
                }
                const double dprev = grad_factor<M>(a1, x, p_slot);
                ag += dloss_dev(LOSS, y0, y1) * dprev;
                ah += dprev * dprev;
            }
            ag += dpp_move_d<0xB1, 0xf>(0.0, ag);
            ah += dpp_move_d<0xB1, 0xf>(0.0, ah);
            ag += dpp_move_d<0x4E, 0xf>(0.0, ag);
            ah += dpp_move_d<0x4E, 0xf>(0.0, ah);
            PRB_WSTAMP(0)
            if (sub == 0 && !((lm0 >> slot) & 1ull)) {
                double* sl = a.slab + (size_t)(b & 1) * a.G * 64 * 2 + ((size_t)g * 64 + slot) * 2;
                const unsigned long long tag = prb_tag(b);
                prb_store_granule(sl, ag, tag);
                prb_store_granule(sl + 1, ah, tag);
            }
        }
        const unsigned long long lmu =
            ((unsigned long long)__builtin_amdgcn_readfirstlane((int)(lm0 >> 32)) << 32) |
            (unsigned)__builtin_amdgcn_readfirstlane((int)lm0);
        if (lmu != 0ull) {
            const int32_t* spb = a.sp + ((size_t)g * a.nb + b) * 65;
            int qi = 0;
            for (unsigned long long mm = lmu; mm != 0ull; mm &= mm - 1, ++qi) {
                const int q = __builtin_ctzll(mm);
                if (worker) {
                    const int le0 = spb[q], le1 = spb[q + 1];
                    const double pq = pold_sched[c0 + q];
                    double lg = 0.0, lh = 0.0;
                    for (int e = le0 + wt; e < le1; e += 256) {
                        const int i = a.erow[e];
                        const double x = (double)eval[e];
                        double a1[Kind<M>::AS], y0, y1;
                        if constexpr (LDSR) {
                            y0 = (double)lds_r[i - row0];
                            y1 = (LR == 1) ? 0.0 : (lds_s[i - row0] ? 1.0 : -1.0);
#pragma unroll
                            for (int t = 0; t < Kind<M>::AS; ++t)
                                a1[t] = (double)lds_a[(i - row0) * Kind<M>::AS + t];
                        } else if constexpr (PK) {
                            const float4 r = rec[(size_t)i];
                            y0 = (double)r.x;
                            y1 = (double)r.y;
                            a1[0] = (double)r.z;
                            a1[Kind<M>::AS - 1] = (double)r.w;
                        } else {
                            const typename Vec2<T>::type yv = yy2[i];
                            y0 = (double)yv.x;
                            y1 = (double)yv.y;
#pragma unroll
                            for (int t = 0; t < Kind<M>::AS; ++t)
                                a1[t] = (double)A[(size_t)i * Kind<M>::AS + t];
                        }
                        const double dprev = grad_factor<M>(a1, x, pq);
                        lg += dloss_dev(LOSS, y0, y1) * dprev;
                        lh += dprev * dprev;
                    }
                    lg = wave_sum(lg);
                    lh = wave_sum(lh);
                    if (lane == 0) {
                        sh_long[(qi * 4 + (wave - 1)) * 2] = lg;
                        sh_long[(qi * 4 + (wave - 1)) * 2 + 1] = lh;
                    }
                }
            }
            __syncthreads();
            if (worker && wt < qi) {
                const int q = nth_set_bit(lmu, wt);
                double tg = 0.0, th = 0.0;
                for (int w4 = 0; w4 < 4; ++w4) {
                    tg += sh_long[(wt * 4 + w4) * 2];
                    th += sh_long[(wt * 4 + w4) * 2 + 1];
                }
                double* sl = a.slab + (size_t)(b & 1) * a.G * 64 * 2 + ((size_t)g * 64 + q) * 2;
                const unsigned long long tag = prb_tag(b);
                prb_store_granule(sl, tg, tag);
                prb_store_granule(sl + 1, th, tag);
            }
        }
        PRB_STAMP(0)
        double p_next = 0.0;
        int n2e0 = 0, n2e1 = 0;
        unsigned long long lm2 = 0ull;
        if (b + 2 < a.nb) prb_load_sp(a, g, b + 2, slot, c3 - c2, n2e0, n2e1, lm2);
        if (worker) {
            PRB_WSTAMP(1)
            if (tid == 64 + 255)
                __hip_atomic_store(sh_go, b + 1, __ATOMIC_RELAXED, __HIP_MEMORY_SCOPE_WORKGROUP);
            if (LDSR && b + 1 < a.nb) {
                prb_load_entries<T>(a, eval, ne0, ne1, sub, nxt, row0);
                if (slot < c2 - c1) p_next = pold_sched[c1 + slot];
            }
            {
                const bool ok =
                    prb_collect_quarter<2>(a, b, part, lane, ncols, sh_quart, kPrbParts);
                if (!ok) *sh_ok = 0;
            }
            PRB_WSTAMP(2)
            if (!LDSR && b + 1 < a.nb) {
                prb_load_entries<T>(a, eval, ne0, ne1, sub, nxt, row0);
                if (slot < c2 - c1) p_next = pold_sched[c1 + slot];
            }
        } else {
            unsigned spins = 0;
            while (__hip_atomic_load(sh_go, __ATOMIC_RELAXED, __HIP_MEMORY_SCOPE_WORKGROUP) <
                       b + 1 &&
                   ++spins < (1u << 24))
                __builtin_amdgcn_s_sleep(1);
            PRB_HSTAMP(1)
            const bool ok = prb_collect_quarter<2>(a, b, part, lane, ncols, sh_quart, kPrbParts);
            if (!ok) *sh_ok = 0;
            PRB_HSTAMP(2)
            if constexpr (CR) {
                if (control) {
                    if (lane < cp1 - cp0) {
                        if (!prb_poll<CSN>(a, a.cslab + ((size_t)(b & 1) * 64 + lane) * CSS,
                                           prb_tag(b), cst))
                            *sh_ok = 0;
                    }
                    const PrbConf<T>* cfa = reinterpret_cast<const PrbConf<T>*>(a.cf);
                    if (lane < cp2 - cp1) cfn = cfa[cp1 + lane];
                    clqn = prb_u4{~0u, ~0u, ~0u, ~0u};
                    if (lane < c2 - c1) clqn = reinterpret_cast<const prb_u4*>(a.clist)[c1 + lane];
                }
            }
        }
        PRB_WSTAMP(3)
        asm volatile("s_waitcnt lgkmcnt(0)\n\ts_barrier" ::: "memory");
        if (!*sh_ok) break;
        PRB_STAMP(3)
        PRB_HSTAMP(7)
        PRB_WSTAMP(4)
        if (control) {
            double tot[2];
#pragma unroll
            for (int v = 0; v < 2; ++v) {
                tot[v] = sh_quart[lane * 2 + v];
#pragma unroll
                for (int w = 1; w < kPrbParts; ++w) tot[v] += sh_quart[(w * 64 + lane) * 2 + v];
            }
            if constexpr (MG) {
                if (!prb_cross_gpu<2>(a, g, b, lane, tot)) *sh_ok = 0;
            }
            const bool valid = lane < ncols;
            bool serial = false;
            if constexpr (CR) serial = (cp1 - cp0) > 0;
            if (!serial) {
                const double res = pcd_chain_lanes<M>(REGC >= 0 ? REGC : reg, lane, ncols - 1, valid,
                                                      pl, tot[0], tot[1], lam, mu, beta, gamma, eta,
                                                      cache, sh_chain);
                const double dl = valid ? (pl - res) : 0.0;
                sh_delta[lane] = dl;
                sh_pold[lane] = pl;
                if (g == 0 && valid) {
                    ps[jl] = res;
                    viol_pos[c0 + lane] = fabs(dl);
                }
            }
            if constexpr (CR) {
                if (serial) {
                    const int nc = cp1 - cp0;
                    const int qa = cfc.qq & 0xff, qb = cfc.qq >> 8;
                    const double xa = (double)cfc.xa, xb = (double)cfc.xb;
                    sh_pold[lane] = pl;
                    sh_delta[lane] = 0.0;
                    asm volatile("s_waitcnt lgkmcnt(0)" ::: "memory");
                    __builtin_amdgcn_wave_barrier();
                    double da[AS + 1], pb = 0.0;
#pragma unroll
                    for (int t = 0; t <= AS; ++t) da[t] = 0.0;
                    if (lane < nc) {
                        const double pa = sh_pold[qa];
                        pb = sh_pold[qb];
                        da[0] = xa;
#pragma unroll
                        for (int t = 1; t <= AS; ++t) da[t] = xa * (cst[1 + t] - pa * da[t - 1]);
                        sh_ce[lane * 2] = dloss_dev(LOSS, cst[0], cst[1]) * da[AS];
                        sh_ce[lane * 2 + 1] = da[AS] * da[AS];
                    }
                    auto after_a = [&](double Da, double* a1, double& y0n) __attribute__((always_inline)) {
#pragma unroll
                        for (int t = 0; t < AS; ++t) a1[t] = (double)(T)(cst[2 + t] - Da * da[t]);
                        y0n = (double)(T)(cst[0] - lam * Da * da[AS]);
                    };
                    asm volatile("s_waitcnt lgkmcnt(0)" ::: "memory");
                    __builtin_amdgcn_wave_barrier();
                    int le[8];
#pragma unroll
                    for (int t = 0; t < 8; ++t) {
                        const unsigned w = clq[t >> 1];
                        le[t] = (int)(short)((t & 1) ? (w >> 16) : (w & 0xffffu));
                    }
                    double g0 = tot[0], h0 = tot[1];
#pragma unroll
                    for (int t = 0; t < 8; ++t)
                        if (le[t] >= 0 && (le[t] >> 8) == 0) {
                            g0 += sh_ce[(le[t] & 0xff) * 2];
                            h0 += sh_ce[(le[t] & 0xff) * 2 + 1];
                        }
                    double cc0[M + 1];
#pragma unroll
                    for (int t = 0; t <= M; ++t) cc0[t] = cache[t];
                    double dl = 0.0, res = pl;
                    for (int round = 0; round <= ncols + 1; ++round) {
                        if (lane < nc) {
                            double a1[AS], y0n;
                            after_a(sh_delta[qa], a1, y0n);
                            const double dAb = grad_factor<M>(a1, xb, pb);
                            sh_cv[lane * 2] = dloss_dev(LOSS, y0n, cst[1]) * dAb;
                            sh_cv[lane * 2 + 1] = dAb * dAb;
                        }
                        asm volatile("s_waitcnt lgkmcnt(0)" ::: "memory");
                        __builtin_amdgcn_wave_barrier();
                        double gq = g0, hq = h0;
#pragma unroll
                        for (int t = 0; t < 8; ++t)
                            if (le[t] >= 0 && (le[t] >> 8) != 0) {
                                gq += sh_cv[(le[t] & 0xff) * 2];
                                hq += sh_cv[(le[t] & 0xff) * 2 + 1];
                            }
#pragma unroll
                        for (int t = 0; t <= M; ++t) cache[t] = cc0[t];
                        res = pcd_chain_lanes<M>(reg, lane, ncols - 1, valid, pl, gq, hq, lam, mu,
                                                 beta, gamma, eta, cache, sh_chain);
                        const double dn = valid ? (pl - res) : 0.0;
                        const bool same = __double_as_longlong(dn) == __double_as_longlong(dl);
                        dl = dn;
                        sh_delta[lane] = dl;
                        asm volatile("s_waitcnt lgkmcnt(0)" ::: "memory");
                        __builtin_amdgcn_wave_barrier();
                        if (__ballot(!same) == 0ull) {
                            if (lane == 0 && g == a.G - 1) {
                                atomicAdd(&g_branch_count[BR_RELAX_STEPS], 1u);
                                atomicAdd(&g_branch_count[BR_RELAX_ROUNDS], (unsigned)(round + 1));
                            }
                            break;
                        }
                    }
                    if (g == 0 && valid) {
                        ps[jl] = res;
                        viol_pos[c0 + lane] = fabs(dl);
                    }
                    if (lane < nc && cfc.row / a.rows_per == g) {
                        const int i = cfc.row;
                        const double Db = sh_delta[qb];
                        double a1[AS], y0n;
                        after_a(sh_delta[qa], a1, y0n);
                        T a2[AS];
                        double db = xb;
#pragma unroll
                        for (int t = 0; t < AS; ++t) {
                            const double dn = xb * (a1[t] - pb * db);
                            a2[t] = (T)(a1[t] - Db * db);
                            db = dn;
                        }
                        const T y0f = (T)(y0n - lam * Db * db);
                        if constexpr (LDSR) {
#pragma unroll
                            for (int t = 0; t < AS; ++t) lds_a[(i - row0) * AS + t] = a2[t];
                            lds_r[i - row0] = y0f;
                        } else if constexpr (PK) {
                            float4 o;
                            o.x = (float)y0f;
                            o.y = (float)cst[1];
                            o.z = (float)a2[0];
                            o.w = (float)a2[AS - 1];
                            rec[(size_t)i] = o;
                        } else {
#pragma unroll
                            for (int t = 0; t < AS; ++t) A[(size_t)i * AS + t] = a2[t];
                            yy[2 * (size_t)i] = y0f;
                        }
                    }
                }
            }
            PRB_STAMP(4)
        }
        asm volatile("s_waitcnt lgkmcnt(0)\n\ts_barrier" ::: "memory");
        PRB_STAMP(5)
        PRB_WSTAMP(5)
        if (slot < ncols) {
            const double upd = sh_delta[slot];
            if (upd != 0.0) {
                const double p_old = sh_pold[slot];
#pragma unroll
                for (int u = 0; u < PRB_PF; ++u) {
                    if (cur.e0 + sub + 4 * u < cur.e1) {
                        const size_t i = (size_t)cur.row[u];
                        const double x = (double)cur.x[u];
                        if constexpr (M == 0) {
                            double yn = yh[u] - lam * av[u][0];
                            double an = av[u][0] / (1.0 + x * p_old);
                            an *= 1.0 + x * (p_old - upd);
                            yn += lam * an;
                            if constexpr (LDSR) {
                                lds_a[i - row0] = (T)an;
                                lds_r[i - row0] = (T)yn;
                            } else {
                                A[i] = (T)an;
                                yy[2 * i] = (T)yn;
                            }
                        } else if constexpr (LDSR) {
                            const int il = (int)i - row0;
                            double dprev = x;
#pragma unroll
                            for (int t = 0; t < AS; ++t) {
                                const double a1 = av[u][t];
                                const double dcur = x * (a1 - p_old * dprev);
                                lds_a[il * AS + t] = (T)(a1 - upd * dprev);
                                dprev = dcur;
                            }
                            lds_r[il] = (T)(yh[u] - lam * upd * dlast[u]);
                        } else if constexpr (PK) {
                            const double d1 = x * (av[u][0] - p_old * x);
                            float4 o;
                            o.x = (float)(yh[u] - lam * upd * dlast[u]);
                            o.y = (float)yt[u];
                            o.z = (float)(av[u][0] - upd * x);
                            o.w = (float)(av[u][AS - 1] - upd * d1);
                            rec[i] = o;
                        } else {
                            double dprev = x;
#pragma unroll
                            for (int t = 1; t < M; ++t) {
                                const double a1 = av[u][t - 1];
                                const double dcur = x * (a1 - p_old * dprev);
                                A[i * (M - 1) + (t - 1)] = (T)(a1 - upd * dprev);
                                dprev = dcur;
                            }
                            yy[2 * i] = (T)(yh[u] - lam * upd * dlast[u]);
                        }
                    }
                }
                for (int e = cur.e0 + sub + 4 * PRB_PF; e < cur.e1; e += 4) {
                    if constexpr (LDSR)
                        pcd_sync_entry_lds<T, M>(a.erow[e] - row0, (double)eval[e], p_old, upd,
                                                 lam, lds_a, lds_r);
                    else if constexpr (PK)
                        pcd_sync_entry_rec((size_t)a.erow[e], (double)eval[e], p_old, upd, lam, rec);
                    else
                        pcd_sync_entry<T, M>((size_t)a.erow[e], (double)eval[e], p_old, upd, lam,
                                             A, yy);
                }
            }
        }
        if (lmu != 0ull && worker) {
            const int32_t* spb = a.sp + ((size_t)g * a.nb + b) * 65;
            for (unsigned long long mm = lmu; mm != 0ull; mm &= mm - 1) {
                const int q = __builtin_ctzll(mm);
                const double upd = sh_delta[q];
                if (upd != 0.0) {
                    const double p_old = sh_pold[q];
                    const int le0 = spb[q], le1 = spb[q + 1];
                    for (int e = le0 + wt; e < le1; e += 256) {
                        if constexpr (LDSR)
                            pcd_sync_entry_lds<T, M>(a.erow[e] - row0, (double)eval[e], p_old,
                                                     upd, lam, lds_a, lds_r);
                        else if constexpr (PK)
                            pcd_sync_entry_rec((size_t)a.erow[e], (double)eval[e], p_old, upd, lam,
                                               rec);
                        else
                            pcd_sync_entry<T, M>((size_t)a.erow[e], (double)eval[e], p_old, upd,
                                                 lam, A, yy);
                    }
                }
            }
        }
        cur = nxt;
        p_slot = p_next;
        ne0 = n2e0;
        ne1 = n2e1;
        lm0 = lm1;
        lm1 = lm2;
        if constexpr (CR) {
            if (control) {
                cp0 = cp1;
                cp1 = cp2;
                cp2 = cp3;
                cp3 = a.cf_ptr[min(b + 4, a.nb)];
                cfc = cfn;
                clq = clqn;
            }
        }
        c0 = c1;
        c1 = c2;
        c2 = c3;
        c3 = c4;
        PRB_WSTAMP(6)
        if constexpr (LDSR)
            asm volatile("s_waitcnt lgkmcnt(0)\n\ts_barrier" ::: "memory");
        else
            __syncthreads();
        PRB_STAMP(6)
        if constexpr (STAMP) {
            if (tid == 320) tprev = clock64();
        }
        PRB_WSTAMP(7)
    }
#undef PRB_STAMP
#undef PRB_HSTAMP
#undef PRB_WSTAMP
    if constexpr (LDSR) {
        __syncthreads();
        const int nr = min(a.rows_per, a.n_rows - row0);
        for (int il = tid; il < nr; il += kPrbThreads) {
            const size_t i = (size_t)(row0 + il);
#pragma unroll
            for (int t = 0; t < AS; ++t) A[i * AS + t] = lds_a[il * AS + t];
            if constexpr (LR == 1)
                yy[2 * i] = (T)((double)lds_r[il] + (double)yy[2 * i + 1]);
            else
                yy[2 * i] = lds_r[il];
        }
    }
    if (STAMP && a.stamps != nullptr && (tid == 0 || tid == 64)) {
#pragma unroll
        for (int q = 0; q < 8; ++q)
            if (tid == 64 || (q != 1 && q != 2 && q != 7))
                a.stamps[(size_t)g * 16 + (tid == 64 ? 8 : 0) + q] = acc[q];
    }
    if (STAMP && a.stamps != nullptr && tid == 320) {
        a.stamps[(size_t)g * 16 + 1] = acc[1];
        a.stamps[(size_t)g * 16 + 2] = acc[2];
        a.stamps[(size_t)g * 16 + 7] = acc[7];
    }
}

template <typename T, int LOSS, int LR, bool MG = false, bool CR = false>
__global__ __launch_bounds__(kPrbThreads) void lin_prb_kernel(
    PrbArgs a, const T* __restrict__ eval, T* __restrict__ yy,
    const double* __restrict__ w_sched, const double* __restrict__ cn_sched,
    double* __restrict__ w, double alpha, double mu, double* __restrict__ viol_pos) {
    extern __shared__ __attribute__((aligned(16))) double dyn_lds[];
    double* sh_delta = dyn_lds + 128;
    double* sh_quart = dyn_lds + 1536;
    int* sh_ok = reinterpret_cast<int*>(dyn_lds + 768);
    int* sh_go = reinterpret_cast<int*>(dyn_lds + 770);
    const typename Vec2<T>::type* yy2 = reinterpret_cast<const typename Vec2<T>::type*>(yy);
    const int g = blockIdx.x;
    const int tid = threadIdx.x, lane = tid & 63, wave = tid >> 6;
    const bool control = wave == 0;
    const bool worker = wave >= 1 && wave <= 4;
    const int part = worker ? wave - 1 : (control ? 4 : wave);
    const int wt = tid - 64;
    const int slot = worker ? (wt >> 2) : 64, sub = wt & 3;
    double* sh_long = dyn_lds + 1024;
    static_assert(LR == 0 || (sizeof(T) == 4 && (LR == 2 || LOSS == LOSS_SQUARED)),
                  "LDS-resident rows: float storage");
    const int row0 = LR ? g * a.rows_per : 0;
    static_assert(!CR || !MG, "relaxed runs: single GPU");
    double* sh_ce = dyn_lds + kPrbLdsFixed;
    double* sh_cv = sh_ce + 64;
    T* lds_r = reinterpret_cast<T*>(dyn_lds + kPrbLdsFixed + (CR ? kPrbLdsCR : 0));
    unsigned char* lds_s = reinterpret_cast<unsigned char*>(lds_r + a.rows_per);
    if constexpr (LR != 0) {
        const int nr = min(a.rows_per, a.n_rows - row0);
        for (int il = tid; il < nr; il += kPrbThreads) {
            const typename Vec2<T>::type yv = yy2[(size_t)(row0 + il)];
            if constexpr (LR == 1) {
                lds_r[il] = (T)((double)yv.x - (double)yv.y);
            } else {
                lds_r[il] = yv.x;
                lds_s[il] = yv.y > (T)0 ? 1 : 0;
            }
        }
        __syncthreads();
    }
    auto row_state = [&](int i, double& y0, double& y1) {
        if constexpr (LR != 0) {
            y0 = (double)lds_r[i - row0];
            y1 = (LR == 1) ? 0.0 : (lds_s[i - row0] ? 1.0 : -1.0);
        } else {
            const typename Vec2<T>::type yv = yy2[(size_t)i];
            y0 = (double)yv.x;
            y1 = (double)yv.y;
        }
    };
    auto row_update = [&](int i, double yold, double dec) {
        if constexpr (LR != 0) lds_r[i - row0] = (T)(yold - dec);
        else yy[2 * (size_t)i] = (T)(yold - dec);
    };
    PrbEntries<T> cur, nxt;
    int c0 = a.bptr[0], c1 = a.bptr[1];
    int c2 = (a.nb > 1) ? a.bptr[2] : c1;
    int c3 = (a.nb > 2) ? a.bptr[3] : c2;
    unsigned long long lm0 = 0ull, lm1 = 0ull;
    {
        int e0, e1;
        prb_load_sp(a, g, 0, slot, c1 - c0, e0, e1, lm0);
        prb_load_entries<T>(a, eval, e0, e1, sub, cur, row0);
    }
    int ne0 = 0, ne1 = 0;
    if (a.nb > 1) prb_load_sp(a, g, 1, slot, c2 - c1, ne0, ne1, lm1);
    if (tid == 0) {
        *sh_ok = 1;
        *sh_go = 0;
    }
    int cp0 = 0, cp1 = 0, cp2 = 0, cp3 = 0;
    PrbConf<T> cfc, cfn;
    cfc.row = cfn.row = 0;
    cfc.qq = cfn.qq = 0;
    cfc.xa = cfc.xb = cfn.xa = cfn.xb = (T)0;
    prb_u4 clq = {~0u, ~0u, ~0u, ~0u}, clqn = {~0u, ~0u, ~0u, ~0u};
    if constexpr (CR) {
        if (control) {
            const PrbConf<T>* cfa = reinterpret_cast<const PrbConf<T>*>(a.cf);
            cp0 = a.cf_ptr[0];
            cp1 = a.cf_ptr[min(1, a.nb)];
            cp2 = a.cf_ptr[min(2, a.nb)];
            cp3 = a.cf_ptr[min(3, a.nb)];
            if (lane < cp1 - cp0) cfc = cfa[cp0 + lane];
            if (lane < c1 - c0) clq = reinterpret_cast<const prb_u4*>(a.clist)[c0 + lane];
        }
    }
    for (int b = 0; b < a.nb; ++b) {
        const int ncols = c1 - c0;
        const int c4 = (b + 4 <= a.nb) ? a.bptr[b + 4] : c3;
        double yh[PRB_PF];
        double wl = 0.0, cnl = 0.0;
        int jl = 0;
        double cst[2] = {0.0, 0.0};
        int n2e0 = 0, n2e1 = 0;
        unsigned long long lm2 = 0ull;
        const unsigned long long lmu =
            ((unsigned long long)__builtin_amdgcn_readfirstlane((int)(lm0 >> 32)) << 32) |
            (unsigned)__builtin_amdgcn_readfirstlane((int)lm0);
        if (lmu != 0ull) {
            const int32_t* spb = a.sp + ((size_t)g * a.nb + b) * 65;
            int qi = 0;
            for (unsigned long long mm = lmu; mm != 0ull; mm &= mm - 1, ++qi) {
                const int q = __builtin_ctzll(mm);
                if (worker) {
                    const int le0 = spb[q], le1 = spb[q + 1];
                    double lg = 0.0;
                    for (int e = le0 + wt; e < le1; e += 256) {
                        double y0, y1;
                        row_state(a.erow[e], y0, y1);
                        lg += dloss_dev(LOSS, y0, y1) * (double)eval[e];
                    }
                    lg = wave_sum(lg);
                    if (lane == 0) sh_long[(qi * 4 + (wave - 1)) * 2] = lg;
                }
            }
            __syncthreads();
            if (worker && wt < qi) {
                const int q = nth_set_bit(lmu, wt);
                double tg = 0.0;
                for (int w4 = 0; w4 < 4; ++w4) tg += sh_long[(wt * 4 + w4) * 2];
                double* sl = a.slab + (size_t)(b & 1) * a.G * 64 * 2 + ((size_t)g * 64 + q) * 2;
                prb_store_granule(sl, tg, prb_tag(b));
            }
        }
        if (control) {
            if (lane < ncols) {
                wl = w_sched[c0 + lane];
                cnl = cn_sched[c0 + lane];
                if (g == 0) jl = a.desc[c0 + lane].j;
            }
            if constexpr (CR) {
                const int nc = cp1 - cp0, ncw = max(nc, cp3 - cp2);
                const unsigned long long ctag = prb_tag(b);
                double* cs = a.cslab + ((size_t)(b & 1) * 64 + lane) * 8;
                if (lane < nc) {
                    if (cfc.row / a.rows_per == g) {
                        double y0, y1;
                        row_state(cfc.row, y0, y1);
                        prb_store_granule(cs, y0, ctag);
                        prb_store_granule(cs + 1, y1, ctag);
                    }
                } else if (lane < ncw && (lane % a.G) == g) {
                    prb_store_granule(cs, 0.0, ctag);
                    prb_store_granule(cs + 1, 0.0, ctag);
                }
            }
        } else if (worker) {
            double yt[PRB_PF];
#pragma unroll
            for (int u = 0; u < PRB_PF; ++u) row_state(cur.row[u], yh[u], yt[u]);
            double ag = 0.0;
#pragma unroll
            for (int u = 0; u < PRB_PF; ++u) {
                const bool v = cur.e0 + sub + 4 * u < cur.e1;
                ag += v ? dloss_dev(LOSS, yh[u], yt[u]) * (double)cur.x[u] : 0.0;
            }
            for (int e = cur.e0 + sub + 4 * PRB_PF; e < cur.e1; e += 4) {
                double y0, y1;
                row_state(a.erow[e], y0, y1);
// ... 441 lines not shown
```

sparsepoly_amd/csrc/spfm_schedule.cpp:

```cpp
#include <algorithm>
#include <atomic>
#include <cstdint>
#include <cstdlib>
#include <cstring>
#include <thread>
#include <vector>

namespace spfm {

void schedule_exact(int64_t n_rows, int32_t d, const int64_t* cptr, const int32_t* cidx,
                    const int32_t* order, int max_batch, std::vector<int32_t>& batch_ptr) {
    std::vector<int32_t> stamp((size_t)n_rows, -1);
    batch_ptr.clear();
    batch_ptr.push_back(0);
    int32_t cur = 0;
    int size = 0;
    for (int32_t pos = 0; pos < d; ++pos) {
        const int32_t j = order[pos];
        bool conflict = (size >= max_batch);
        if (!conflict) {
            for (int64_t ii = cptr[j]; ii < cptr[j + 1]; ++ii)
                if (stamp[cidx[ii]] == cur) {
                    conflict = true;
                    break;
// ... 199 lines not shown

void schedule_colored_parallel(int64_t n_rows, int32_t d, const int64_t* cptr, const int32_t* cidx,
                               const int32_t* order, int max_batch, int n_threads,
                               std::vector<int32_t>& out_order, std::vector<int32_t>& batch_ptr) {
    int kRoundMax = std::max(8, std::min(64, 3 * std::max(1, n_threads - 1)));
    if (const char* e = std::getenv("SPFM_SCHED_ROUND")) {
        const int v = std::atoi(e);
        if (v >= 1 && v <= 1024) kRoundMax = v;
    }
    const int64_t nnz = cptr[d];
    struct RowList {
        int64_t start;
        std::atomic<int32_t> cnt;
        int32_t pad;
    };
    std::vector<RowList> rows((size_t)n_rows + 1);
    {
        std::vector<int64_t> rstart((size_t)n_rows + 1, 0);
        for (int64_t ii = 0; ii < nnz; ++ii) rstart[(size_t)cidx[ii] + 1]++;
        for (int64_t i = 0; i < n_rows; ++i) rstart[(size_t)i + 1] += rstart[(size_t)i];
        for (int64_t i = 0; i <= n_rows; ++i) {
            rows[(size_t)i].start = rstart[(size_t)i];
            rows[(size_t)i].cnt.store(0, std::memory_order_relaxed);
            rows[(size_t)i].pad = 0;
        }
    }
    std::vector<int32_t> rcol((size_t)nnz);
    std::vector<std::vector<int32_t>> classes;
    std::vector<uint64_t> full;
    std::vector<int32_t> todo(order, order + d);
    size_t head = 0;
    std::vector<int32_t> round_cols, colour((size_t)kRoundMax);
    round_cols.reserve(kRoundMax);
    size_t n_classes = 0, words = 1;
    bool done = false;
    SpinBarrier bar(n_threads);
    std::vector<std::vector<uint64_t>> used((size_t)kRoundMax);
    const int n_work = n_threads > 1 ? n_threads - 1 : 1;

    auto snapshot_set = [&](int32_t j, std::vector<uint64_t>& u) {
        u.assign(words, 0);
        for (size_t w = 0; w < full.size() && w < words; ++w) u[w] = full[w];
        const int64_t cb = cptr[j], ce = cptr[j + 1];
        constexpr int64_t PD = 12;
        for (int64_t ii = cb; ii < ce; ++ii) {
            if (ii + 2 * PD < ce) __builtin_prefetch(&rows[(size_t)cidx[ii + 2 * PD]]);
            if (ii + PD < ce) __builtin_prefetch(&rcol[(size_t)rows[(size_t)cidx[ii + PD]].start]);
            const RowList& r = rows[(size_t)cidx[ii]];
            const int32_t* rc = &rcol[(size_t)r.start];
            const int32_t cnt = r.cnt.load(std::memory_order_relaxed);
            for (int32_t t = 0; t < cnt; ++t) u[(size_t)rc[t] >> 6] |= 1ull << (rc[t] & 63);
        }
    };
    auto commit = [&](int32_t j, int32_t c) {
        const int64_t cb = cptr[j], ce = cptr[j + 1];
        for (int64_t ii = cb; ii < ce; ++ii) {
            if (ii + 12 < ce) __builtin_prefetch(&rows[(size_t)cidx[ii + 12]], 1);
            RowList& r = rows[(size_t)cidx[ii]];
            const int32_t slot = r.cnt.fetch_add(1, std::memory_order_relaxed);
            rcol[(size_t)r.start + slot] = c;
        }
    };
    auto phase1 = [&](int wid) {
        for (size_t q = (size_t)wid; q < round_cols.size(); q += (size_t)n_work)
            snapshot_set(round_cols[q], used[q]);
    };
    auto phase3 = [&](int wid) {
        for (size_t q = (size_t)wid; q < round_cols.size(); q += (size_t)n_work)
            commit(round_cols[q], colour[q]);
    };

    auto worker = [&](int tid) {
        for (;;) {
            bar.wait();
            if (done) return;
            phase1(tid - 1);
            bar.wait();
            bar.wait();
            phase3(tid - 1);
            bar.wait();
        }
    };
    std::vector<std::thread> pool;
    for (int t = 1; t < n_threads; ++t) pool.emplace_back(worker, t);
    for (;;) {
        round_cols.clear();
        while ((int)round_cols.size() < kRoundMax && head < todo.size())
            round_cols.push_back(todo[head++]);
        n_classes = classes.size();
        words = n_classes / 64 + 1;
        if (round_cols.empty()) {
            done = true;
            bar.wait();
            break;
        }
        bar.wait();
        if (n_threads == 1) phase1(0);
        bar.wait();
        for (size_t q = 0; q < round_cols.size(); ++q) {
            const std::vector<uint64_t>& u = used[q];
            int32_t c = 0;
            for (;; ++c) {
                if ((size_t)c >= classes.size()) break;
                if ((size_t)c < n_classes && ((u[(size_t)c >> 6] >> (c & 63)) & 1ull)) {
                    size_t w = (size_t)c >> 6;
                    uint64_t free_bits = ~u[w] & (~0ull << (c & 63));
                    while (free_bits == 0 && ++w < words) free_bits = ~u[w];
                    c = (free_bits == 0) ? (int32_t)(words * 64)
                                         : (int32_t)(w * 64 + (size_t)__builtin_ctzll(free_bits));
                    if ((size_t)c >= classes.size()) break;
                }
                if ((int)classes[(size_t)c].size() >= max_batch) continue;
                bool clash = false;
                for (size_t a = 0; a < q && !clash; ++a)
                    if (colour[a] == c &&
                        columns_share_row(cptr, cidx, round_cols[a], round_cols[q]))
                        clash = true;
                if (!clash) break;
            }
            if ((size_t)c >= classes.size()) {
                c = (int32_t)classes.size();
                classes.emplace_back();
            }
            colour[q] = c;
            classes[(size_t)c].push_back(round_cols[q]);
            if ((int)classes[(size_t)c].size() >= max_batch) {
                if (full.size() <= ((size_t)c >> 6)) full.resize(((size_t)c >> 6) + 1, 0);
                full[(size_t)c >> 6] |= 1ull << (c & 63);
            }
        }
        bar.wait();
        if (n_threads == 1) phase3(0);
        bar.wait();
    }
    for (auto& t : pool) t.join();
    out_order.clear();
    out_order.reserve((size_t)d);
    batch_ptr.clear();
    batch_ptr.push_back(0);
    for (auto& cl : classes) {
        if (cl.empty()) continue;
        out_order.insert(out_order.end(), cl.begin(), cl.end());
        batch_ptr.push_back((int32_t)out_order.size());
    }
    if (batch_ptr.size() == 1) batch_ptr.push_back(0);
}

void schedule_rlf(int64_t n_rows, int32_t d, const int64_t* cptr, const int32_t* cidx,
                  const int32_t* order, int max_batch, std::vector<int32_t>& out_order,
                  std::vector<int32_t>& batch_ptr) {
    std::vector<int32_t> urow((size_t)n_rows, 0), wrow((size_t)n_rows, 0), mark((size_t)n_rows, 0);
    for (int64_t ii = 0; ii < cptr[d]; ++ii) urow[(size_t)cidx[ii]]++;
    std::vector<char> coloured((size_t)d, 0);
    std::vector<int32_t> cand, members;
    cand.reserve((size_t)d);
    out_order.clear();
    out_order.reserve((size_t)d);
    batch_ptr.assign(1, 0);
    int32_t n_done = 0, stamp = 0;
    while (n_done < d) {
        cand.clear();
        for (int32_t pos = 0; pos < d; ++pos)
            if (!coloured[(size_t)pos]) cand.push_back(pos);
        std::fill(wrow.begin(), wrow.end(), 0);
        members.clear();
        while (!cand.empty() && (int)members.size() < max_batch) {
            const int32_t* cnt = members.empty() ? urow.data() : wrow.data();
            int64_t best_key = -1;
            int32_t best = -1;
            for (const int32_t pos : cand) {
                const int32_t j = order[pos];
                int64_t key = 0;
                for (int64_t ii = cptr[j]; ii < cptr[j + 1]; ++ii) key += cnt[(size_t)cidx[ii]];
                if (key > best_key) {
                    best_key = key;
                    best = pos;
                }
            }
            ++stamp;
            const int32_t v = order[best];
            for (int64_t ii = cptr[v]; ii < cptr[v + 1]; ++ii) {
                mark[(size_t)cidx[ii]] = stamp;
                urow[(size_t)cidx[ii]]--;
            }
            coloured[(size_t)best] = 1;
            members.push_back(best);
            size_t kept = 0;
            for (const int32_t pos : cand) {
                if (pos == best) continue;
                const int32_t u = order[pos];
                bool hit = false;
                for (int64_t ii = cptr[u]; ii < cptr[u + 1] && !hit; ++ii)
                    hit = mark[(size_t)cidx[ii]] == stamp;
                if (!hit) {
                    cand[kept++] = pos;
                    continue;
                }
                for (int64_t ii = cptr[u]; ii < cptr[u + 1]; ++ii) wrow[(size_t)cidx[ii]]++;
            }
            cand.resize(kept);
        }
        std::sort(members.begin(), members.end());
        for (const int32_t pos : members) out_order.push_back(order[pos]);
        n_done += (int32_t)members.size();
        batch_ptr.push_back(n_done);
    }
    if (batch_ptr.size() == 1) batch_ptr.push_back(0);
}

int schedule_threads() {
    if (const char* e = std::getenv("SPFM_THREADS")) {
        const int v = std::atoi(e);
        if (v >= 1) return std::min(v, 64);
    }
    const unsigned hw = std::thread::hardware_concurrency();
    return (int)std::max(1u, std::min(hw, 16u));
}

template <typename F>
static void run_threads(int n_threads, F&& fn) {
    std::vector<std::thread> pool;
    for (int t = 1; t < n_threads; ++t) pool.emplace_back([&fn, t]() { fn(t); });
    fn(0);
    for (auto& th : pool) th.join();
}


void csc_to_csr(int64_t n, int32_t d, const int64_t* cptr, const int32_t* cidx,
                std::vector<int64_t>& rptr, std::vector<int32_t>& ridx,
                std::vector<int64_t>& perm ) {
    const int64_t nnz = cptr[d];
    rptr.assign((size_t)n + 1, 0);
    ridx.resize((size_t)nnz);
    perm.resize((size_t)nnz);
    const int T = (nnz >= (1 << 20)) ? schedule_threads() : 1;
    const int64_t per = (n + T - 1) / T;
    run_threads(T, [&](int tid) {
        const int64_t lo = per * tid, hi = std::min<int64_t>(n, lo + per);
        for (int64_t ii = 0; ii < nnz; ++ii) {
            const int64_t i = cidx[ii];
            if (i >= lo && i < hi) rptr[(size_t)i + 1]++;
        }
    });
    for (int64_t i = 0; i < n; ++i) rptr[(size_t)i + 1] += rptr[(size_t)i];
    std::vector<int64_t> fill(rptr.begin(), rptr.end() - 1);
    run_threads(T, [&](int tid) {
        const int64_t lo = per * tid, hi = std::min<int64_t>(n, lo + per);
        for (int32_t j = 0; j < d; ++j)
            for (int64_t ii = cptr[j]; ii < cptr[j + 1]; ++ii) {
                const int64_t i = cidx[ii];
                if (i < lo || i >= hi) continue;
                const int64_t dst = fill[(size_t)i]++;
                ridx[(size_t)dst] = j;
                perm[(size_t)dst] = ii;
            }
    });
}

bool csr_to_csc(int64_t n, int32_t d, const int64_t* rptr, const int32_t* ridx,
                std::vector<int64_t>& cptr, std::vector<int32_t>& cidx,
                std::vector<int64_t>& perm) {
    const int64_t nnz = rptr[n];
    cptr.assign((size_t)d + 1, 0);
    cidx.resize((size_t)nnz);
    perm.resize((size_t)nnz);
    const int T = (nnz >= (1 << 20)) ? schedule_threads() : 1;
    const int32_t per = (int32_t)((d + T - 1) / T);
    std::vector<char> bad((size_t)T, 0);
    run_threads(T, [&](int tid) {
        const int32_t lo = per * tid, hi = std::min<int32_t>(d, lo + per);
        if (tid == 0)
            for (int64_t i = 0; i < n && !bad[0]; ++i)
                for (int64_t ii = rptr[i]; ii < rptr[i + 1]; ++ii)
                    if (ridx[ii] < 0 || ridx[ii] >= d || (ii > rptr[i] && ridx[ii] <= ridx[ii - 1])) {
                        bad[0] = 1;
                        break;
                    }
        for (int64_t ii = 0; ii < nnz; ++ii) {
            const int32_t j = ridx[ii];
            if (j >= lo && j < hi) cptr[(size_t)j + 1]++;
        }
    });
    if (bad[0]) return false;
    for (int32_t j = 0; j < d; ++j) cptr[(size_t)j + 1] += cptr[(size_t)j];
    std::vector<int64_t> fill(cptr.begin(), cptr.end() - 1);
    run_threads(T, [&](int tid) {
        const int32_t lo = per * tid, hi = std::min<int32_t>(d, lo + per);
        for (int64_t i = 0; i < n; ++i)
            for (int64_t ii = rptr[i]; ii < rptr[i + 1]; ++ii) {
                const int32_t j = ridx[ii];
                if (j < lo || j >= hi) continue;
                const int64_t dst = fill[(size_t)j]++;
                cidx[(size_t)dst] = (int32_t)i;
                perm[(size_t)dst] = ii;
            }
    });
    return true;
}

void build_rowblock_stream(int64_t n, const int64_t* cptr, const int32_t* cidx,
                           const std::vector<int32_t>& order,
                           const std::vector<int32_t>& batch_ptr, int G, int long_thresh,
                           std::vector<int32_t>& sp, std::vector<int32_t>& src,
                           std::vector<uint32_t>& lmask, const uint8_t* skip) {
    const int nb = (int)batch_ptr.size() - 1;
    const int64_t rows_per = (n + G - 1) / G > 0 ? (n + G - 1) / G : 1;
    sp.assign((size_t)G * nb * 65 + 1, 0);
    const int64_t nnz = cptr[order.size()];
    const int T = std::min(G, (nnz >= (1 << 20)) ? schedule_threads() : 1);
    const int gper = (G + T - 1) / T;
    run_threads(T, [&](int tid) {
        const int g0 = gper * tid, g1 = std::min(G, g0 + gper);
        const int64_t rlo = (int64_t)g0 * rows_per, rhi = (int64_t)g1 * rows_per;
        for (int b = 0; b < nb; ++b)
            for (int q = 0; q < batch_ptr[b + 1] - batch_ptr[b]; ++q) {
                const int32_t j = order[(size_t)batch_ptr[b] + q];
                for (int64_t ii = cptr[j]; ii < cptr[j + 1]; ++ii) {
                    const int64_t i = cidx[ii];
                    if (i < rlo || i >= rhi) continue;
                    if (skip && skip[(size_t)ii]) continue;
                    sp[((size_t)(i / rows_per) * nb + b) * 65 + q]++;
                }
            }
    });
    int64_t run = 0;
    for (size_t t = 0; t < sp.size(); ++t) {
        const int64_t c = sp[t];
        sp[t] = (int32_t)run;
        run += c;
    }
    lmask.assign((size_t)G * nb * 2, 0u);
    for (int g = 0; g < G; ++g)
        for (int b = 0; b < nb; ++b) {
            const size_t base = ((size_t)g * nb + b) * 65;
            for (int q = 0; q < batch_ptr[b + 1] - batch_ptr[b]; ++q)
                if (sp[base + q + 1] - sp[base + q] > long_thresh)
                    lmask[((size_t)g * nb + b) * 2 + (q >> 5)] |= (1u << (q & 31));
        }
    src.resize((size_t)run);
    std::vector<int32_t> fill(sp.begin(), sp.end());
    run_threads(T, [&](int tid) {
        const int g0 = gper * tid, g1 = std::min(G, g0 + gper);
        const int64_t rlo = (int64_t)g0 * rows_per, rhi = (int64_t)g1 * rows_per;
        for (int b = 0; b < nb; ++b)
            for (int q = 0; q < batch_ptr[b + 1] - batch_ptr[b]; ++q) {
                const int32_t j = order[(size_t)batch_ptr[b] + q];
                for (int64_t ii = cptr[j]; ii < cptr[j + 1]; ++ii) {
                    const int64_t i = cidx[ii];
                    if (i < rlo || i >= rhi) continue;
                    if (skip && skip[(size_t)ii]) continue;
                    src[(size_t)fill[((size_t)(i / rows_per) * nb + b) * 65 + q]++] = (int32_t)ii;
                }
            }
    });
}

void build_pb_stream(int64_t n, const int64_t* cptr, const int32_t* cidx,
                     const std::vector<int32_t>& order, const std::vector<int32_t>& batch_ptr,
                     int G, int NG, bool balance, const uint8_t* skip, std::vector<int32_t>& gsp,
                     std::vector<int32_t>& src, std::vector<uint8_t>& meta,
                     std::vector<uint8_t>& tab) {
    const int nb = (int)batch_ptr.size() - 1;
    const int QM = 64 / NG;
    const int64_t rows_per = (n + G - 1) / G > 0 ? (n + G - 1) / G : 1;
    const size_t stride = (size_t)NG + 1;
    gsp.assign((size_t)G * nb * stride + 1, 0);
    tab.assign((size_t)G * (size_t)std::max(nb, 1) * 64, 0xFF);
    const int64_t nnz = cptr[order.size()];
    const int T = std::min(G, (nnz >= (1 << 20)) ? schedule_threads() : 1);
    const int gper = (G + T - 1) / T;
    auto ncols_of = [&](int b) { return (b >= 0 && b < nb) ? batch_ptr[b + 1] - batch_ptr[b] : 0; };
    auto sub_range = [&](int32_t j, int64_t rlo, int64_t rhi, int64_t& lo, int64_t& hi) {
        const int32_t* first = cidx + cptr[j];
        const int32_t* last = cidx + cptr[j + 1];
        lo = cptr[j] + (std::lower_bound(first, last, (int32_t)std::min<int64_t>(rlo, INT32_MAX)) - first);
        hi = cptr[j] + (std::lower_bound(first, last, (int32_t)std::min<int64_t>(rhi, INT32_MAX)) - first);
    };
    run_threads(T, [&](int tid) {
        const int g0 = gper * tid, g1 = std::min(G, g0 + gper);
        if (g0 >= g1) return;
        const int64_t rlo = (int64_t)g0 * rows_per, rhi = std::min<int64_t>(n, (int64_t)g1 * rows_per);
        std::vector<int32_t> cnt((size_t)(g1 - g0) * 64);
        int idx[64], load[64], used[64];
        for (int b = 0; b < nb; ++b) {
            const int nc = ncols_of(b);
            const int nw = std::min(64, std::max(nc, ncols_of(b + 2)));
            std::fill(cnt.begin(), cnt.end(), 0);
            for (int q = 0; q < nc; ++q) {
                int64_t lo, hi;
                sub_range(order[(size_t)batch_ptr[b] + q], rlo, rhi, lo, hi);
                for (int64_t ii = lo; ii < hi; ++ii)
                    if (!skip || !skip[ii]) cnt[(size_t)(cidx[ii] / rows_per - g0) * 64 + (size_t)q]++;
            }
            for (int g = g0; g < g1; ++g) {
                const int32_t* c = &cnt[(size_t)(g - g0) * 64];
                uint8_t* tb = &tab[((size_t)g * nb + b) * 64];
                int32_t* gs = &gsp[((size_t)g * nb + b) * stride];
                if (!balance) {
                    for (int q = 0; q < nw; ++q) {
                        tb[(q % NG) * QM + q / NG] = (uint8_t)q;
                        gs[q % NG] += c[q];
                    }
                    continue;
                }
                for (int q = 0; q < nw; ++q) idx[q] = q;
                std::stable_sort(idx, idx + nw, [&](int x, int y) { return c[x] > c[y]; });
                for (int r = 0; r < NG; ++r) load[r] = used[r] = 0;
                for (int z = 0; z < nw; ++z) {
                    const int q = idx[z];
                    int best = -1;
                    for (int r = 0; r < NG; ++r)
                        if (used[r] < QM && (best < 0 || load[r] < load[best])) best = r;
                    tb[best * QM + used[best]] = (uint8_t)q;
                    used[best]++;
                    load[best] += c[q];
                }
                for (int r = 0; r < NG; ++r) gs[r] = load[r];
            }
        }
    });
    int64_t run = 0;
    for (size_t t = 0; t < gsp.size(); ++t) {
        const int64_t c = gsp[t];
        gsp[t] = (int32_t)run;
        run += c;
    }
    src.resize((size_t)run);
    meta.resize((size_t)run);
    std::vector<int32_t> last((size_t)n, -2);
    run_threads(T, [&](int tid) {
        const int g0 = gper * tid, g1 = std::min(G, g0 + gper);
        if (g0 >= g1) return;
        const int64_t rlo = (int64_t)g0 * rows_per, rhi = std::min<int64_t>(n, (int64_t)g1 * rows_per);
        std::vector<int32_t> pos((size_t)(g1 - g0) * 64);
        std::vector<uint8_t> where((size_t)(g1 - g0) * 64);
        std::vector<int64_t> lo_q(64), hi_q(64);
        for (int b = 0; b < nb; ++b) {
            const int nc = ncols_of(b);
            std::fill(pos.begin(), pos.end(), 0);
            for (int q = 0; q < nc; ++q) {
                sub_range(order[(size_t)batch_ptr[b] + q], rlo, rhi, lo_q[(size_t)q], hi_q[(size_t)q]);
                for (int64_t ii = lo_q[(size_t)q]; ii < hi_q[(size_t)q]; ++ii)
                    if (!skip || !skip[ii])
                        pos[(size_t)(cidx[ii] / rows_per - g0) * 64 + (size_t)q]++;
            }
            for (int g = g0; g < g1; ++g) {
                int32_t* pc = &pos[(size_t)(g - g0) * 64];
                uint8_t* wh = &where[(size_t)(g - g0) * 64];
                const uint8_t* tb = &tab[((size_t)g * nb + b) * 64];
                const int32_t* gs = &gsp[((size_t)g * nb + b) * stride];
                for (int r = 0; r < NG; ++r) {
                    int32_t at = gs[r];
                    for (int t = 0; t < QM; ++t) {
                        const int q = tb[r * QM + t];
                        if (q == 0xFF) continue;
                        wh[q] = (uint8_t)((r << 3) | t);
                        const int32_t c = q < nc ? pc[q] : 0;
                        pc[q] = at;
                        at += c;
                    }
                }
            }
            for (int q = 0; q < nc; ++q)
                for (int64_t ii = lo_q[(size_t)q]; ii < hi_q[(size_t)q]; ++ii) {
                    const int64_t i = cidx[ii];
                    if (skip && skip[ii]) {
                        last[(size_t)i] = b;
                        continue;
                    }
                    const size_t gi = (size_t)(i / rows_per);
                    const size_t lq = (gi - (size_t)g0) * 64 + (size_t)q;
                    const size_t e = (size_t)pos[lq]++;
                    src[e] = (int32_t)ii;
                    meta[e] = (uint8_t)((where[lq] & 7) | (last[(size_t)i] == b - 1 ? 0x80 : 0));
                    last[(size_t)i] = b;
                }
        }
    });
}

void build_wide_stream(int64_t n, const int64_t* cptr, const int32_t* cidx,
                       const std::vector<int32_t>& order, const std::vector<int32_t>& batch_ptr,
                       int G, std::vector<int32_t>& wbase, std::vector<int32_t>& wsp,
                       std::vector<int32_t>& src, std::vector<uint8_t>& hz) {
    const int nb = (int)batch_ptr.size() - 1;
    const int64_t rows_per = (n + G - 1) / G > 0 ? (n + G - 1) / G : 1;
    wbase.assign((size_t)nb + 1, 0);
    for (int b = 0; b < nb; ++b) wbase[(size_t)b + 1] = wbase[(size_t)b] + (batch_ptr[b + 1] - batch_ptr[b]) + 1;
    const size_t tot = (size_t)wbase[(size_t)nb];
    wsp.assign((size_t)G * tot + 1, 0);
    const int64_t nnz = cptr[order.size()];
    const int T = std::min(G, (nnz >= (1 << 20)) ? schedule_threads() : 1);
    const int gper = (G + T - 1) / T;
    run_threads(T, [&](int tid) {
        const int g0 = gper * tid, g1 = std::min(G, g0 + gper);
        const int64_t rlo = (int64_t)g0 * rows_per, rhi = (int64_t)g1 * rows_per;
        for (int b = 0; b < nb; ++b)
            for (int q = 0; q < batch_ptr[b + 1] - batch_ptr[b]; ++q) {
                const int32_t j = order[(size_t)batch_ptr[b] + q];
                for (int64_t ii = cptr[j]; ii < cptr[j + 1]; ++ii) {
                    const int64_t i = cidx[ii];
                    if (i < rlo || i >= rhi) continue;
                    wsp[(size_t)(i / rows_per) * tot + (size_t)wbase[(size_t)b] + (size_t)q]++;
                }
            }
    });
    int64_t run = 0;
    for (size_t t = 0; t < wsp.size(); ++t) {
        const int64_t c = wsp[t];
        wsp[t] = (int32_t)run;
        run += c;
    }
    src.resize((size_t)run);
    hz.resize((size_t)run);
    std::vector<int32_t> fill(wsp.begin(), wsp.end());
    std::vector<int32_t> last((size_t)n, -2);
    run_threads(T, [&](int tid) {
        const int g0 = gper * tid, g1 = std::min(G, g0 + gper);
        const int64_t rlo = (int64_t)g0 * rows_per, rhi = (int64_t)g1 * rows_per;
        for (int b = 0; b < nb; ++b)
            for (int q = 0; q < batch_ptr[b + 1] - batch_ptr[b]; ++q) {
                const int32_t j = order[(size_t)batch_ptr[b] + q];
                for (int64_t ii = cptr[j]; ii < cptr[j + 1]; ++ii) {
                    const int64_t i = cidx[ii];
                    if (i < rlo || i >= rhi) continue;
                    const size_t e = (size_t)fill[(size_t)(i / rows_per) * tot +
                                                  (size_t)wbase[(size_t)b] + (size_t)q]++;
                    src[e] = (int32_t)ii;
                    hz[e] = (uint8_t)(last[(size_t)i] == b - 1 ? 1 : 0);
                    last[(size_t)i] = b;
                }
            }
    });
}

}
```

Baseline: 3.687 epochs/s.

## Precompute next-step partial sums during exchange wait using row-hazard masks

Adds a per-(workgroup, step, slot) hazard bitmask, built on host or device at stream-build time, that marks entries whose row was touched in the previous step. In the degree-2 LDS-resident persistent PCD kernel, the next step's entries are loaded and gradient partial sums for hazard-free entries are computed while waiting on the cross-workgroup slab exchange. The first slab pairs are also issued early and reused. Only hazarded entries are recomputed after the update, which hides latency but adds registers, an extra hazard buffer and build-time work.

Result: slower. 2.967 epochs/s (-19.5%).

```diff
diff --git a/sparsepoly_amd/csrc/spfm_engine.hip.h b/sparsepoly_amd/csrc/spfm_engine.hip.h
--- a/sparsepoly_amd/csrc/spfm_engine.hip.h
+++ b/sparsepoly_amd/csrc/spfm_engine.hip.h
@@ -48,7 +48,8 @@
                      std::vector<uint8_t>&);
 void build_rowblock_stream(int64_t, const int64_t*, const int32_t*, const std::vector<int32_t>&,
                            const std::vector<int32_t>&, int, int, std::vector<int32_t>&,
-                           std::vector<int32_t>&, std::vector<uint32_t>&, const uint8_t*);
+                           std::vector<int32_t>&, std::vector<uint32_t>&, const uint8_t*,
+                           std::vector<uint16_t>* = nullptr);
 void schedule_relax(int64_t, int32_t, const int64_t*, const int32_t*, const int32_t*, int, int,
                     std::vector<int32_t>&, std::vector<int32_t>&, std::vector<int32_t>&,
                     std::vector<int32_t>&, std::vector<int64_t>&, std::vector<int64_t>&,
@@ -65,6 +66,8 @@
 hipError_t device_rowblock_stream(int64_t, int32_t, int64_t, int, int, int, const int32_t*,
                                   const int32_t*, const int64_t*, const int32_t*, const uint8_t*,
                                   int32_t*, int32_t*, uint32_t*, int*, int64_t*, hipStream_t);
+hipError_t device_rowblock_hazards(int64_t, int, int, const int32_t*, const int32_t*, uint16_t*,
+                                   hipStream_t);
 hipError_t device_pb_stream(int64_t, int32_t, int64_t, int, int, int, int, const int32_t*,
                             const int32_t*, const int64_t*, const int32_t*, const int64_t*,
                             const int32_t*, int32_t*, int32_t*, uint8_t*, uint8_t*, hipStream_t);
@@ -170,7 +173,7 @@
     std::mutex mu;
     struct Prb {
         std::string key;
-        DevBuf sp, erow, eval, lmask;
+        DevBuf sp, erow, eval, lmask, hz;
         int has_long = 0;
     };
     struct Pb {
@@ -255,12 +258,14 @@
     int prb_G = 64;
     bool prb_lds = true;
     int prb_lds_active = 0;
+    bool prb_early = true;
+    int prb_early_active = 0;
     bool y_pm1 = false;
     bool prb_ready = false;
     int prb_has_long = 0;
     int prb_long = kPrbLong;
     DevBuf prb_sp, prb_erow, prb_eval, prb_slab, prb_abort, prow_old, d_bptr, prb_stamps,
-        prb_viol, prb_cn, prb_lmask, prb_rec;
+        prb_viol, prb_cn, prb_lmask, prb_rec, prb_hz;
     bool prb_pack = true;
     int prb_pack_active = 0;
     bool prb_stamp_on = false;
diff --git a/sparsepoly_amd/csrc/spfm_engine_pcd.hip b/sparsepoly_amd/csrc/spfm_engine_pcd.hip
--- a/sparsepoly_amd/csrc/spfm_engine_pcd.hip
+++ b/sparsepoly_amd/csrc/spfm_engine_pcd.hip
@@ -135,6 +135,7 @@
     a.lmask = prb_lmask.as<uint32_t>();
     a.has_long = prb_has_long;
     a.erow = prb_erow.as<int32_t>();
+    a.hz = prb_hz.as<uint16_t>();
     a.slab = prb_slab.as<double>();
     a.rows_per = (int)std::max<int64_t>((n + prb_G - 1) / prb_G, 1);
     a.n_rows = (int)n;
@@ -160,6 +161,7 @@
     a.lmask = r_lmask.as<uint32_t>();
     a.has_long = relax_has_long;
     a.erow = r_erow.as<int32_t>();
+    a.hz = nullptr;
     a.stamps = nullptr;
     a.cf_ptr = r_cfptr.as<int32_t>();
     a.cf = r_cf.p;
diff --git a/sparsepoly_amd/csrc/spfm_engine_prb.inc.h b/sparsepoly_amd/csrc/spfm_engine_prb.inc.h
--- a/sparsepoly_amd/csrc/spfm_engine_prb.inc.h
+++ b/sparsepoly_amd/csrc/spfm_engine_prb.inc.h
@@ -129,6 +129,7 @@
                 prb_erow.share(e->erow);
                 prb_eval.share(e->eval);
                 prb_lmask.share(e->lmask);
+                prb_hz.share(e->hz);
                 prb_has_long = e->has_long;
                 stream_device_used = 2;
                 hit = true;
@@ -145,6 +146,7 @@
             e->erow.share(prb_erow);
             e->eval.share(prb_eval);
             e->lmask.share(prb_lmask);
+            e->hz.share(prb_hz);
             e->has_long = prb_has_long;
             scache->prb.insert(scache->prb.begin(), std::move(e));
             if (scache->prb.size() > StreamCache::kKeep) scache->prb.pop_back();
@@ -175,6 +177,7 @@
     HIPC(d_src.alloc(sizeof(int32_t) * (size_t)(nnz > 0 ? nnz : 1)));
     HIPC(prb_sp.alloc(sizeof(int32_t) * nsp));
     HIPC(prb_lmask.alloc(sizeof(uint32_t) * (size_t)prb_G * nb_ * 2));
+    HIPC(prb_hz.alloc(sizeof(uint16_t) * std::max<size_t>((size_t)prb_G * nb_ * 64, 1)));
     stream_device_used = 0;
     if (stream_device && nnz >= (1 << 20)) {
         int hl = 0;
@@ -191,12 +194,14 @@
     }
     std::vector<int32_t> sp, src;
     std::vector<uint32_t> lmask;
+    std::vector<uint16_t> hz;
     if (!stream_device_used) {
         build_rowblock_stream(n, h_cptr.data(), h_cidx.data(), order, batch_ptr, prb_G,
-                              prb_long, sp, src, lmask, nullptr);
+                              prb_long, sp, src, lmask, nullptr, &hz);
         prb_has_long = 0;
         for (uint32_t m : lmask) prb_has_long |= (m != 0u);
         SPFM_TRY(upload_to(prb_lmask.p, lmask.data(), lmask.size()));
+        if (!hz.empty()) SPFM_TRY(upload_to(prb_hz.p, hz.data(), hz.size()));
     }
     HIPC(prb_erow.alloc(sizeof(int32_t) * (size_t)(nnz > 0 ? nnz : 1)));
     HIPC(prb_eval.alloc(sizeof(T) * (size_t)(nnz > 0 ? nnz : 1)));
@@ -210,6 +215,9 @@
                            prb_erow.as<int32_t>(), prb_eval.as<T>());
         HIPC(hipGetLastError());
     }
+    if (stream_device_used)
+        HIPC(device_rowblock_hazards(n, prb_G, nb_, prb_sp.as<int32_t>(), prb_erow.as<int32_t>(),
+                                     prb_hz.as<uint16_t>(), stream));
     HIPC(hipStreamSynchronize(stream));
     return SPFM_OK;
 }
@@ -345,6 +353,7 @@
                         (LRV == 1 || y_pm1);
     const size_t lds_bytes = use_lr ? std::max(lds_lr, kPrbLds) : kPrbLds;
     prb_lds_active = use_lr ? LRV : 0;
+    prb_early_active = 0;
     hipLaunchKernelGGL(begin_pass_kernel, dim3(1), dim3(64), 0, stream, c,
                        comp_order.as<int32_t>(), lams.as<double>());
     if (reg != SPFM_REG_L1) {
@@ -377,25 +386,29 @@
         constexpr bool STc = decltype(stamp_tag)::value;
         constexpr int RGc = decltype(reg_tag)::value;
         const size_t lds = (LRc == 1 || LRc == 2) ? lds_bytes : kPrbLds;
-        auto launch = [&](auto mg_tag) -> int {
+        auto launch = [&](auto mg_tag, auto eg_tag) -> int {
             constexpr bool MGc = decltype(mg_tag)::value;
-            HIPC(hipFuncSetAttribute(
-                (const void*)pcd_prb_kernel<T, M, LOSS, LRc, STc, RGc, MGc>,
-                hipFuncAttributeMaxDynamicSharedMemorySize, (int)lds));
-            if (!resident_ok((const void*)pcd_prb_kernel<T, M, LOSS, LRc, STc, RGc, MGc>,
-                             kPrbThreads, lds, prb_G))
-                return kNotResident;
-            hipLaunchKernelGGL((pcd_prb_kernel<T, M, LOSS, LRc, STc, RGc, MGc>),
-                               dim3(launch_groups(prb_G)), dim3(kPrbThreads), lds, stream, c, pa, prb_eval.as<T>(),
-                               A.as<T>(), (size_t)n * Kind<M>::AS, yy.as<T>(),
-                               prow_old.as<double>(), Po, d, reg, cb, mu, beta, gamma, eta,
-                               prb_viol.as<double>());
+            constexpr bool EGc = decltype(eg_tag)::value;
+            auto* fn = pcd_prb_kernel<T, M, LOSS, LRc, STc, RGc, MGc, false, EGc>;
+            HIPC(hipFuncSetAttribute((const void*)fn, hipFuncAttributeMaxDynamicSharedMemorySize,
+                                     (int)lds));
+            if (!resident_ok((const void*)fn, kPrbThreads, lds, prb_G)) return kNotResident;
+            hipLaunchKernelGGL(fn, dim3(launch_groups(prb_G)), dim3(kPrbThreads), lds, stream, c,
+                               pa, prb_eval.as<T>(), A.as<T>(), (size_t)n * Kind<M>::AS,
+                               yy.as<T>(), prow_old.as<double>(), Po, d, reg, cb, mu, beta, gamma,
+                               eta, prb_viol.as<double>());
+            prb_early_active = EGc ? 1 : 0;
             return SPFM_OK;
         };
+        constexpr bool can_eg = M == 2 && (LRc == 1 || LRc == 2) && !STc;
         if constexpr (STc) {
-            return launch(std::false_type{});
+            return launch(std::false_type{}, std::false_type{});
         } else {
-            return pa.n_ranks > 1 ? launch(std::true_type{}) : launch(std::false_type{});
+            if (pa.n_ranks > 1) return launch(std::true_type{}, std::false_type{});
+            if constexpr (can_eg) {
+                if (prb_early) return launch(std::false_type{}, std::true_type{});
+            }
+            return launch(std::false_type{}, std::false_type{});
         }
     };
     using std::integral_constant;
diff --git a/sparsepoly_amd/csrc/spfm_ingest.hip b/sparsepoly_amd/csrc/spfm_ingest.hip
--- a/sparsepoly_amd/csrc/spfm_ingest.hip
+++ b/sparsepoly_amd/csrc/spfm_ingest.hip
@@ -268,6 +268,40 @@
     return done(hipSuccess);
 }
 
+
+__global__ __launch_bounds__(1024) void rbs_hazard_kernel(int nb, const int32_t* __restrict__ sp,
+                                                          const int32_t* __restrict__ erow,
+                                                          int32_t* __restrict__ stamp,
+                                                          uint16_t* __restrict__ hz) {
+    const int g = blockIdx.x, t = threadIdx.x, q = t >> 4, k = t & 15;
+    for (int b = 0; b < nb; ++b) {
+        const int32_t* spb = sp + ((size_t)g * nb + b) * 65;
+        const int32_t e0 = spb[q], e1 = spb[q + 1];
+        bool f = false;
+        if (b >= 1 && e0 + k < e1) f = stamp[erow[e0 + k]] == b;
+        const unsigned long long m = __ballot(f);
+        if (k == 0) hz[((size_t)g * nb + b) * 64 + q] = (uint16_t)(m >> (t & 63));
+        __syncthreads();
+        for (int32_t e = spb[0] + t; e < spb[64]; e += 1024) stamp[erow[e]] = b + 1;
+        __syncthreads();
+    }
+}
+
+hipError_t device_rowblock_hazards(int64_t n, int G, int nb, const int32_t* sp,
+                                   const int32_t* erow, uint16_t* hz, hipStream_t stream) {
+    if (nb <= 0 || G <= 0) return hipSuccess;
+    int32_t* stamp = nullptr;
+    hipError_t e = hipMalloc(&stamp, sizeof(int32_t) * (size_t)(n > 0 ? n : 1));
+    if (e != hipSuccess) return e;
+    if ((e = hipMemsetAsync(stamp, 0, sizeof(int32_t) * (size_t)(n > 0 ? n : 1), stream)) ==
+        hipSuccess) {
+        hipLaunchKernelGGL(rbs_hazard_kernel, dim3(G), dim3(1024), 0, stream, nb, sp, erow, stamp, hz);
+        e = hipGetLastError();
+        if (e == hipSuccess) e = hipStreamSynchronize(stream);
+    }
+    (void)hipFree(stamp);
+    return e;
+}
 
 
 __global__ void sb_step_of_kernel(int32_t d, int nb, const int32_t* __restrict__ order,
diff --git a/sparsepoly_amd/csrc/spfm_options.inc.h b/sparsepoly_amd/csrc/spfm_options.inc.h
--- a/sparsepoly_amd/csrc/spfm_options.inc.h
+++ b/sparsepoly_amd/csrc/spfm_options.inc.h
@@ -106,6 +106,7 @@
     {"prb_groups", TUNING, integer(M(prb_G), 1, kMax), PRB | RELAX, "workgroups of the 64-column persistent pass"},
     {"prb_long", TUNING, integer(M(prb_long), 16, kMax), PRB | RELAX, "entries per (workgroup, step, slot) above which a slot is long"},
     {"prb_lds", TUNING, flag(M(prb_lds)), G, "keep the row block in LDS when it fits"},
+    {"prb_early", TUNING, flag(M(prb_early)), G, "degree 2, rows in LDS: form the next step's partial sums inside the exchange wait"},
     {"prb_pack", TUNING, flag(M(prb_pack)), G, "packed row records for degree-3 passes with rows in global memory"},
     {"relax", TUNING, flag(M(relax_on)), RELAX | PBRELAX, "merged steps for schedules of tiny steps"},
     {"pbcd_persistent", TUNING, flag(M(pb_persistent)), G, "the persistent pbcd pass"},
@@ -143,6 +144,7 @@
     {"wide_active", READOUT, custom(nullptr, get_wide_active), 0, "the next pcd epoch uses the wide pass"},
     {"pbprb_active", READOUT, readout(M(pbprb_active)), 0, "what the last pbcd epoch used"},
     {"prb_lds_active", READOUT, readout(M(prb_lds_active)), 0, "last pcd pass: 0 global rows, 1 LDS residual, 2 LDS prediction + sign"},
+    {"prb_early_active", READOUT, readout(M(prb_early_active)), 0, "the last pcd pass formed the next step's partial sums inside the exchange wait"},
     {"prb_pack_active", READOUT, readout(M(prb_pack_active)), 0, "the last pcd pass used packed row records"},
     {"wide_lds_active", READOUT, readout(M(wide_lr_active)), 0, "last wide pass: 0 global rows, 1 all rows in LDS, 2 first rows of a block"},
     {"wide_ep_active", READOUT, readout(M(wide_ep_active)), 0, "the last wide pass used the entry-parallel form"},
diff --git a/sparsepoly_amd/csrc/spfm_prb.hip.h b/sparsepoly_amd/csrc/spfm_prb.hip.h
--- a/sparsepoly_amd/csrc/spfm_prb.hip.h
+++ b/sparsepoly_amd/csrc/spfm_prb.hip.h
@@ -14,6 +14,7 @@
     const uint32_t* lmask;
     int has_long;
     const int32_t* erow;
+    const uint16_t* hz;
     double* slab;
     int rows_per;
     int n_rows;
@@ -143,10 +144,39 @@
         : "memory");
 }
 
-template <int NV>
+__device__ __forceinline__ void prb_issue_pairs8(const double* const* p, prb_u4* r) {
+    asm volatile(
+        "global_load_dwordx4 %0, %8, off sc1\n\t"
+        "global_load_dwordx4 %1, %9, off sc1\n\t"
+        "global_load_dwordx4 %2, %10, off sc1\n\t"
+        "global_load_dwordx4 %3, %11, off sc1\n\t"
+        "global_load_dwordx4 %4, %12, off sc1\n\t"
+        "global_load_dwordx4 %5, %13, off sc1\n\t"
+        "global_load_dwordx4 %6, %14, off sc1\n\t"
+        "global_load_dwordx4 %7, %15, off sc1"
+        : "=&v"(r[0]), "=&v"(r[1]), "=&v"(r[2]), "=&v"(r[3]), "=&v"(r[4]), "=&v"(r[5]),
+          "=&v"(r[6]), "=&v"(r[7])
+        : "v"(p[0]), "v"(p[1]), "v"(p[2]), "v"(p[3]), "v"(p[4]), "v"(p[5]), "v"(p[6]), "v"(p[7])
+        : "memory");
+}
+__device__ __forceinline__ void prb_wait_pairs8(prb_u4* r) {
+    asm volatile("s_waitcnt vmcnt(0)"
+                 : "+v"(r[0]), "+v"(r[1]), "+v"(r[2]), "+v"(r[3]), "+v"(r[4]), "+v"(r[5]),
+                   "+v"(r[6]), "+v"(r[7])
+                 :
+                 : "memory");
+}
+__device__ __forceinline__ const double* prb_first_pair(const PrbArgs& a, int b, int w, int lane,
+                                                        int g, int nparts, int u) {
+    const int g0 = (a.G * w) / nparts, g1 = (a.G * (w + 1)) / nparts;
+    const int gi = (g0 + u < g1) ? g0 + u : (g1 > g0 ? g1 - 1 : g);
+    return a.slab + (size_t)(b & 1) * a.G * 64 * 2 + (size_t)lane * 2 + (size_t)gi * 128;
+}
+
+template <int NV, bool PRE = false>
 __device__ __forceinline__ bool prb_collect_quarter(const PrbArgs& a, int b, int w, int lane,
                                                     int ncols, double* out ,
-                                                    int nparts = 4) {
+                                                    int nparts = 4, const prb_u4* pre = nullptr) {
     const double* slab = a.slab + (size_t)(b & 1) * a.G * 64 * 2;
     const unsigned long long tag = prb_tag(b);
     const int g0 = (a.G * w) / nparts, g1 = (a.G * (w + 1)) / nparts;
@@ -168,7 +198,12 @@
 #pragma unroll
                     for (int u = 0; u < GU; ++u)
                         ptr[u] = sl + (size_t)((gg + u < g1) ? gg + u : g1 - 1) * 128;
-                    prb_load_pairs8(ptr, r);
+                    if (PRE && gg == g0 && spins == 0) {
+#pragma unroll
+                        for (int u = 0; u < GU; ++u) r[u] = pre[u];
+                    } else {
+                        prb_load_pairs8(ptr, r);
+                    }
 #pragma unroll
                     for (int u = 0; u < GU; ++u) {
                         t[u][0] = ((unsigned long long)r[u].y << 32) | r[u].x;
@@ -258,6 +293,34 @@
     }
 }
 
+struct PrbRaw {
+    int row[PRB_PF];
+    float x[PRB_PF];
+    double p;
+    unsigned hz;
+};
+__device__ __forceinline__ void prb_issue_entries(const PrbArgs& a, const float* __restrict__ eval,
+                                                  int e0, int e1, int sub, const double* pp,
+                                                  const uint16_t* hp, PrbRaw& raw) {
+#pragma unroll
+    for (int u = 0; u < PRB_PF; ++u) {
+        const int e = e0 + sub + 4 * u;
+        const int ec = e < e1 ? e : 0;
+        asm volatile("global_load_dword %0, %1, off" : "=v"(raw.row[u]) : "v"(a.erow + ec) : "memory");
+        asm volatile("global_load_dword %0, %1, off" : "=v"(raw.x[u]) : "v"(eval + ec) : "memory");
+    }
+    asm volatile("global_load_dwordx2 %0, %1, off" : "=v"(raw.p) : "v"(pp) : "memory");
+    asm volatile("global_load_ushort %0, %1, off" : "=v"(raw.hz) : "v"(hp) : "memory");
+}
+__device__ __forceinline__ void prb_wait_entries(PrbRaw& raw) {
+    asm volatile("s_waitcnt vmcnt(8)"
+                 : "+v"(raw.row[0]), "+v"(raw.row[1]), "+v"(raw.row[2]), "+v"(raw.row[3]),
+                   "+v"(raw.x[0]), "+v"(raw.x[1]), "+v"(raw.x[2]), "+v"(raw.x[3]), "+v"(raw.p),
+                   "+v"(raw.hz)
+                 :
+                 : "memory");
+}
+
 constexpr int kPrbThreads = 512;
 constexpr int kPrbParts = 8;
 constexpr int kPrbLdsFixed = 2560;
@@ -309,7 +372,7 @@
 
 constexpr int kPrbLdsCR = 256;
 template <typename T, int M, int LOSS, int LR, bool STAMP = false, int REGC = -1, bool MG = false,
-          bool CR = false>
+          bool CR = false, bool EG = false>
 __global__ __launch_bounds__(kPrbThreads) void pcd_prb_kernel(
     const Ctl* __restrict__ ctl, PrbArgs a, const T* __restrict__ eval, T* __restrict__ A_all,
     size_t a_stride, T* __restrict__ yy, const double* __restrict__ pold_sched,
@@ -349,6 +412,8 @@
     float4* __restrict__ rec = reinterpret_cast<float4*>(a.rec);
     constexpr int AS = Kind<M>::AS;
     static_assert(!CR || (M >= 2 && !MG && !STAMP), "relaxed runs: degree >= 2, single GPU");
+    static_assert(!EG || (LDSR && M == 2 && !MG && !CR && !STAMP),
+                  "early gather: degree 2, rows in LDS, single GPU, strict steps");
     constexpr int CSN = 2 + Kind<M>::AS;
     constexpr int CSS = 8;
     const int row0 = LDSR ? g * a.rows_per : 0;
@@ -388,6 +453,14 @@
     if (tid == 0) {
         *sh_ok = 1;
         *sh_go = 0;
+    }
+    unsigned emask = 0u;
+    float e_r[PRB_PF], e_a[PRB_PF];
+    double e_pg[PRB_PF], e_dp[PRB_PF];
+#pragma unroll
+    for (int u = 0; u < PRB_PF; ++u) {
+        e_r[u] = e_a[u] = 0.0f;
+        e_pg[u] = e_dp[u] = 0.0;
     }
     int cp0 = 0, cp1 = 0, cp2 = 0, cp3 = 0;
     PrbConf<T> cfc, cfn;
@@ -438,8 +511,21 @@
         const int ncols = c1 - c0;
         const int c4 = (b + 4 <= a.nb) ? a.bptr[b + 4] : c3;
         __builtin_amdgcn_s_waitcnt(0x0F70);
+#ifndef SPFM_PRB_EG_TOP
+#define SPFM_PRB_EG_TOP 0
+#endif
+        PrbRaw raw;
+        if constexpr (EG && SPFM_PRB_EG_TOP) {
+            if (worker) {
+                const bool more = b + 1 < a.nb;
+                prb_issue_entries(a, eval, more ? ne0 : 0, more ? ne1 : 0, sub,
+                                  pold_sched + ((more && slot < c2 - c1) ? c1 + slot : 0),
+                                  a.hz + ((size_t)g * a.nb + (more ? b + 1 : b)) * 64 + slot, raw);
+            }
+        }
         double av[PRB_PF][AS];
         double yh[PRB_PF], yt[PRB_PF], dlast[PRB_PF];
+        float c_r[PRB_PF], c_a[PRB_PF];
         double pl = 0.0;
         int jl = 0;
         double cst[CSN];
@@ -485,8 +571,53 @@
                 }
             }
         } else if (worker) {
-#pragma unroll
-            for (int u = 0; u < PRB_PF; ++u) {
+            double ag = 0.0, ah = 0.0;
+            if constexpr (EG) {
+                bool late[PRB_PF];
+                bool any_late[PRB_PF];
+                float l_r[PRB_PF], l_a[PRB_PF];
+                int l_s[PRB_PF];
+#pragma unroll
+                for (int u = 0; u < PRB_PF; ++u) {
+                    late[u] = (cur.e0 + sub + 4 * u < cur.e1) && !((emask >> u) & 1u);
+                    any_late[u] = __ballot(late[u]) != 0ull;
+                    l_r[u] = l_a[u] = 0.0f;
+                    l_s[u] = 0;
+                    if (any_late[u]) {
+                        const int il = cur.row[u] - row0;
+                        l_r[u] = lds_r[il];
+                        l_a[u] = lds_a[il];
+                        if constexpr (LR == 2) l_s[u] = lds_s[il];
+                    }
+                }
+#pragma unroll
+                for (int u = 0; u < PRB_PF; ++u) {
+                    float fr = e_r[u], fa = e_a[u];
+                    double pg = e_pg[u], dp = e_dp[u];
+                    if (any_late[u]) {
+                        double a1[AS];
+                        a1[0] = (double)l_a[u];
+                        const double y1 = (LR == 1) ? 0.0 : (l_s[u] ? 1.0 : -1.0);
+                        const double dprev = grad_factor<M>(a1, (double)cur.x[u], p_slot);
+                        const double dl = dloss_dev(LOSS, (double)l_r[u], y1);
+                        if (late[u]) {
+                            fr = l_r[u];
+                            fa = l_a[u];
+                            pg = dl * dprev;
+                            dp = dprev;
+                        }
+                    }
+                    const double ph = dp * dp;
+                    c_r[u] = fr;
+                    c_a[u] = fa;
+                    dlast[u] = dp;
+                    const bool v = cur.e0 + sub + 4 * u < cur.e1;
+                    ag += v ? pg : 0.0;
+                    ah += v ? ph : 0.0;
+                }
+            }
+#pragma unroll
+            for (int u = 0; u < (EG ? 0 : PRB_PF); ++u) {
                 if constexpr (LDSR) {
                     const int il = cur.row[u] - row0;
                     yh[u] = (double)lds_r[il];
@@ -508,9 +639,8 @@
                     for (int t = 0; t < AS; ++t) av[u][t] = (double)A[i * AS + t];
                 }
             }
-            double ag = 0.0, ah = 0.0;
-#pragma unroll
-            for (int u = 0; u < PRB_PF; ++u) {
+#pragma unroll
+            for (int u = 0; u < (EG ? 0 : PRB_PF); ++u) {
                 const double dprev = grad_factor<M>(av[u], (double)cur.x[u], p_slot);
                 dlast[u] = dprev;
                 const double dl = dloss_dev(LOSS, yh[u], yt[u]);
@@ -627,11 +757,68 @@
             PRB_WSTAMP(1)
             if (tid == 64 + 255)
                 __hip_atomic_store(sh_go, b + 1, __ATOMIC_RELAXED, __HIP_MEMORY_SCOPE_WORKGROUP);
-            if (LDSR && b + 1 < a.nb) {
+            if (!EG && LDSR && b + 1 < a.nb) {
                 prb_load_entries<T>(a, eval, ne0, ne1, sub, nxt, row0);
                 if (slot < c2 - c1) p_next = pold_sched[c1 + slot];
             }
-            {
+            if constexpr (EG) {
+                const bool more = b + 1 < a.nb;
+                if constexpr (!SPFM_PRB_EG_TOP)
+                    prb_issue_entries(a, eval, more ? ne0 : 0, more ? ne1 : 0, sub,
+                                      pold_sched + ((more && slot < c2 - c1) ? c1 + slot : 0),
+                                      a.hz + ((size_t)g * a.nb + (more ? b + 1 : b)) * 64 + slot,
+                                      raw);
+                const double* ptr[8];
+                prb_u4 r8[8];
+#pragma unroll
+                for (int u = 0; u < 8; ++u) ptr[u] = prb_first_pair(a, b, part, lane, g, kPrbParts, u);
+                prb_issue_pairs8(ptr, r8);
+                prb_wait_entries(raw);
+                emask = 0u;
+                if (more) {
+                    nxt.e0 = ne0;
+                    nxt.e1 = ne1;
+                    p_next = (slot < c2 - c1) ? raw.p : 0.0;
+                    bool early[PRB_PF];
+#pragma unroll
+                    for (int u = 0; u < PRB_PF; ++u) {
+                        const bool v = ne0 + sub + 4 * u < ne1;
+                        nxt.row[u] = v ? raw.row[u] : row0;
+                        nxt.x[u] = v ? raw.x[u] : 0.0f;
+                        early[u] = v && !((raw.hz >> (sub + 4 * u)) & 1u);
+                        emask |= early[u] ? (1u << u) : 0u;
+                    }
+                    bool any_early[PRB_PF];
+                    int e_s[PRB_PF];
+#pragma unroll
+                    for (int u = 0; u < PRB_PF; ++u) {
+                        any_early[u] = __ballot(early[u]) != 0ull;
+                        e_s[u] = 0;
+                        if (any_early[u]) {
+                            const int il = nxt.row[u] - row0;
+                            e_r[u] = lds_r[il];
+                            e_a[u] = lds_a[il];
+                            if constexpr (LR == 2) e_s[u] = lds_s[il];
+                        }
+                    }
+#pragma unroll
+                    for (int u = 0; u < PRB_PF; ++u) {
+                        if (any_early[u]) {
+                            double a1[AS];
+                            a1[0] = (double)e_a[u];
+                            const double y1 = (LR == 1) ? 0.0 : (e_s[u] ? 1.0 : -1.0);
+                            const double dprev = grad_factor<M>(a1, (double)nxt.x[u], p_next);
+                            const double dl = dloss_dev(LOSS, (double)e_r[u], y1);
+                            e_pg[u] = dl * dprev;
+                            e_dp[u] = dprev;
+                        }
+                    }
+                }
+                prb_wait_pairs8(r8);
+                const bool ok = prb_collect_quarter<2, true>(a, b, part, lane, ncols, sh_quart,
+                                                             kPrbParts, r8);
+                if (!ok) *sh_ok = 0;
+            } else {
                 const bool ok =
                     prb_collect_quarter<2>(a, b, part, lane, ncols, sh_quart, kPrbParts);
                 if (!ok) *sh_ok = 0;
@@ -823,6 +1010,13 @@
             const double upd = sh_delta[slot];
             if (upd != 0.0) {
                 const double p_old = sh_pold[slot];
+                if constexpr (EG) {
+#pragma unroll
+                    for (int u = 0; u < PRB_PF; ++u) {
+                        yh[u] = (double)c_r[u];
+                        av[u][0] = (double)c_a[u];
+                    }
+                }
 #pragma unroll
                 for (int u = 0; u < PRB_PF; ++u) {
                     if (cur.e0 + sub + 4 * u < cur.e1) {
diff --git a/sparsepoly_amd/csrc/spfm_schedule.cpp b/sparsepoly_amd/csrc/spfm_schedule.cpp
--- a/sparsepoly_amd/csrc/spfm_schedule.cpp
+++ b/sparsepoly_amd/csrc/spfm_schedule.cpp
@@ -525,7 +525,8 @@
                            const std::vector<int32_t>& order,
                            const std::vector<int32_t>& batch_ptr, int G, int long_thresh,
                            std::vector<int32_t>& sp, std::vector<int32_t>& src,
-                           std::vector<uint32_t>& lmask, const uint8_t* skip) {
+                           std::vector<uint32_t>& lmask, const uint8_t* skip,
+                           std::vector<uint16_t>* hz) {
     const int nb = (int)batch_ptr.size() - 1;
     const int64_t rows_per = (n + G - 1) / G > 0 ? (n + G - 1) / G : 1;
     sp.assign((size_t)G * nb * 65 + 1, 0);
@@ -575,6 +576,30 @@
                     src[(size_t)fill[((size_t)(i / rows_per) * nb + b) * 65 + q]++] = (int32_t)ii;
                 }
             }
+    });
+    if (!hz) return;
+    hz->assign((size_t)G * nb * 64, 0);
+    run_threads(T, [&](int tid) {
+        const int g0 = gper * tid, g1 = std::min(G, g0 + gper);
+        std::vector<int32_t> last((size_t)rows_per);
+        for (int g = g0; g < g1; ++g) {
+            std::fill(last.begin(), last.end(), 0);
+            const int64_t r0 = (int64_t)g * rows_per;
+            for (int b = 0; b < nb; ++b) {
+                const size_t base = ((size_t)g * nb + b) * 65;
+                if (b >= 1)
+                    for (int q = 0; q < 64; ++q) {
+                        const int32_t e0 = sp[base + q], e1 = sp[base + q + 1];
+                        uint16_t m = 0;
+                        for (int k = 0; k < 16 && e0 + k < e1; ++k)
+                            if (last[(size_t)(cidx[src[(size_t)(e0 + k)]] - r0)] == b)
+                                m |= (uint16_t)(1u << k);
+                        (*hz)[((size_t)g * nb + b) * 64 + q] = m;
+                    }
+                for (int32_t e = sp[base]; e < sp[base + 64]; ++e)
+                    last[(size_t)(cidx[src[(size_t)e]] - r0)] = b + 1;
+            }
+        }
     });
 }
 
```
